# addtt/ladder-vae-pytorch

Measured on AMD Instinct MI355X. Metric: training images/sec (ELBO step: fwd+bwd+Adamax), higher is better.
Workload: dtype f32; 1 GPU; CIFAR10-shaped 15-layer LVAE (BASELINE configs[2]): 32x32x3, zdims 32x15, 4 blocks/layer, 64 filters, gated+skip, DMoL-10, dropout 0.2, free bits 1.0; batch_per_gpu=256, global_batch=256, parallelism=dp1, hip_graph=True

## Files before the change

include/lvae_hip.h:

```cpp
#ifndef LVAE_HIP_H
#define LVAE_HIP_H

#include <stddef.h>
#include <stdint.h>

#ifdef __cplusplus
extern "C" {
#endif

#define LVAE_ABI_VERSION 17

#define LVAE_EINVAL (-1)
#define LVAE_EALIGN (-2)
#define LVAE_EWORKSPACE (-3)

enum { LVAE_STATS_BN_FWD = 0, LVAE_STATS_BN_BWD = 1 };
enum { LVAE_PREC_F32 = 0, LVAE_PREC_BF16 = 1 };
enum { LVAE_DT_F32 = 0, LVAE_DT_BF16 = 1 };
enum {
  LVAE_FORM_AUTO = 0,
  LVAE_FORM_F32_MFMA = 1,
  LVAE_FORM_SIX_PRODUCT = 2,
  LVAE_FORM_SIX_PRODUCT_DIRECT = 3
};
enum { LVAE_ACT_NONE = 0, LVAE_ACT_ELU = 1, LVAE_ACT_RELU = 2, LVAE_ACT_LEAKYRELU = 3, LVAE_ACT_SELU = 4 };

enum {
  LVAE_GATHER_CONV = 0,
  LVAE_GATHER_TRANSPOSED = 1
};

int lvae_abi_version(void);
const char* lvae_last_error(void);

typedef struct lvae_bn_fold {
  const float* parts;
  int32_t rows;
  int64_t M;
  const float* gamma;
  const float* beta;
  float eps, momentum;
  float* running_mean;
  float* running_var;
  float* coef_out;
} lvae_bn_fold;

typedef struct lvae_conv_desc {
  const float* x;
  const float* x2;
  int32_t C1, C2;
  const float* w;
  int64_t w_stap, w_sk, w_sn;
  const float* bias;
  const float* in_scale;
  const float* in_shift;
  int32_t in_act;
  const float* out_scale;
  int32_t out_act;
  float* y;
  int32_t N, H, W, OH, OW, Cout;
  int32_t KH, KW, stride, pad;
  int32_t gather;
  int32_t precision;
  void* workspace;
  int64_t workspace_bytes;
  int32_t workspace_ready;
  float* stats_out;
  const float* stats_pivot;
  int32_t stats_mode;
  int32_t stats_act;
  const float* stats_x;
  const struct lvae_bn_fold* in_fold;
  int32_t form;
  uint8_t x_dtype;
  uint8_t y_dtype;
  uint8_t stats_x_dtype;
  uint8_t reserved_;
} lvae_conv_desc;

size_t lvae_conv2d_workspace(const lvae_conv_desc* d);
int lvae_conv2d_f32(const lvae_conv_desc* d, void* stream);
int lvae_conv1x1_dgrad_cat_f32(const lvae_conv_desc* d, float* dx2, int32_t split, void* stream);
int32_t lvae_conv1x1_dgrad_cat_ok(const lvae_conv_desc* d, int32_t split);
enum {
  LVAE_VARIANT_DIRECT = 0,
  LVAE_VARIANT_POS = 2,
  LVAE_VARIANT_WINO_F32 = 3,
  LVAE_VARIANT_WINO_SIX = 4,
  LVAE_VARIANT_BF16_DIRECT = 5,
  LVAE_VARIANT_SIX_DIRECT = 6
};
int32_t lvae_conv2d_variant(const lvae_conv_desc* d);
int32_t lvae_conv2d_position_major(const lvae_conv_desc* d);
int32_t lvae_resblock_bf16_storage(const lvae_conv_desc* d);
int lvae_conv2d_bf16(const lvae_conv_desc* d, void* stream);
int32_t lvae_conv2d_stats_rows(const lvae_conv_desc* d);
int32_t lvae_conv2d_folds_bn_finalize(const lvae_conv_desc* d);
int32_t lvae_conv2d_stats_buffer_rows(const lvae_conv_desc* d);

size_t lvae_conv2d_prepare_entry_bytes(void);
int lvae_conv2d_prepare_entry(const lvae_conv_desc* d, void* entry);
int lvae_conv2d_prepare_weights(const void* entries, int32_t n, int32_t max_cout, void* stream);

int lvae_conv1x1_gate_f32(const lvae_conv_desc* d, const float* res, int32_t act, float* out, void* stream);
int32_t lvae_conv1x1_gate_stats_rows(const lvae_conv_desc* d);
enum {
  LVAE_GATE_PERSISTENT = 1,
  LVAE_GATE_SINGLE_SHOT = 2
};
int32_t lvae_conv1x1_gate_variant(const lvae_conv_desc* d);
int lvae_conv1x1_gate_bwd_f32(const lvae_conv_desc* d, const float* dout, const float* ab, int32_t act, float* dab,
                              void* stream);
int32_t lvae_conv1x1_gate_bwd_ok(const lvae_conv_desc* d);

typedef struct lvae_bn_apply {
  const float* parts;
  int32_t rows;
  int32_t act;
  int64_t M;
  const float* coef;
  const float* dh;
  const float* x;
  const float* add;
  float* dgamma;
  float* dbeta;
  float* out;
  int32_t dh_bf16;
  int32_t reserved_;
  const float* drop;
} lvae_bn_apply;
size_t lvae_conv1x1_gate_bwd_wgrad_workspace(const lvae_conv_desc* d);
int32_t lvae_conv1x1_gate_bwd_wgrad_apply_ok(const lvae_conv_desc* d);
int lvae_conv1x1_gate_bwd_wgrad_f32(const lvae_conv_desc* d, const float* dout, const float* ab, const float* y, int32_t act,
                                    float* dw, int64_t dw_sk, int64_t dw_sn, float* db, void* workspace, size_t workspace_bytes,
                                    const lvae_bn_apply* ap, void* stream);
int32_t lvae_conv1x1_gate_bwd_wgrad_recompute_ok(const lvae_conv_desc* d);
int lvae_conv1x1_gate_bwd_wgrad_recompute_f32(const lvae_conv_desc* d, const float* dout, const float* y, int32_t act, void* gate_ws,
                                              int64_t gate_ws_bytes, int32_t gate_ws_ready, const float* gate_w, int64_t gate_w_sk,
                                              int64_t gate_w_sn, const float* gate_bias, float* dw, int64_t dw_sk, int64_t dw_sn,
                                              float* db, void* workspace, size_t workspace_bytes, const lvae_bn_apply* ap, void* stream);

size_t lvae_conv1x1_cat_bwd_workspace(const lvae_conv_desc* d, int32_t split);
int32_t lvae_conv1x1_cat_bwd_apply_ok(const lvae_conv_desc* d, int32_t split);
int lvae_conv1x1_cat_bwd_f32(const lvae_conv_desc* d, const float* x1, const float* x2, float* dx1, float* dx2, float* dweight, float* dbias,
                             const lvae_bn_apply* ap, void* workspace, size_t workspace_bytes, int32_t max_workgroups, void* stream);

enum { LVAE_RB_PRO_AFFINE = 0, LVAE_RB_PRO_BN_APPLY = 1, LVAE_RB_PRO_GATE_BWD = 2 };
enum { LVAE_RB_EPI_PLAIN = 0, LVAE_RB_EPI_GATE = 1 };
typedef struct lvae_rb_ext {
  int32_t prologue, epilogue;
  const float* gate_w;
  int64_t gate_w_sk, gate_w_sn;
  void* gate_ws;
  int64_t gate_ws_bytes;
  int32_t gate_ws_ready;
  const float* gate_bias;
  int32_t act;
  const float* res;
  float* ab;
  float* out;
  float* out_stats;
  const float* out_stats_pivot;
  const float* dout;
  const float* ab_in;
  float* dab;
  const float* bwd_parts;
  int32_t bwd_rows;
  int32_t bwd_act;
  int64_t bwd_M;
  const float* bwd_coef;
  const float* bwd_x;
  float* dgamma;
  float* dbeta;
  const float* pro_drop;
  float* xt_out;
  const void* pf_ptr[2];
  int64_t pf_bytes[2];
  const float* ap_parts;
  int32_t ap_rows;
  int32_t ap_act;
  int64_t ap_M;
  const float* ap_coef;
  const float* ap_dh;
  const float* ap_x;
  const float* ap_add;
  float* ap_dgamma;
  float* ap_dbeta;
  float* ap_out;
} lvae_rb_ext;
size_t lvae_resblock_gate_workspace(const lvae_conv_desc* g);
int lvae_resblock_gate_prepare_entry(const lvae_conv_desc* g, void* entry);
int32_t lvae_resblock_conv_rows(const lvae_conv_desc* d);
int32_t lvae_resblock_conv_gate_rows(const lvae_conv_desc* d);
size_t lvae_resblock_conv_workspace(const lvae_conv_desc* d);
int lvae_resblock_conv_prepare_entry(const lvae_conv_desc* d, void* entry);
int lvae_resblock_conv_f32(const lvae_conv_desc* d, const lvae_rb_ext* ext, void* stream);

size_t lvae_conv2d_wgrad_workspace(const lvae_conv_desc* d);
int lvae_conv2d_wgrad_f32(const lvae_conv_desc* d, const float* dy, float* dw, float* db, void* workspace,
                          size_t workspace_bytes, void* stream);
int lvae_conv2d_wgrad_bf16(const lvae_conv_desc* d, const float* dy, float* dw, float* db, void* workspace, size_t workspace_bytes,
                           void* stream);
int32_t lvae_conv2d_wgrad_apply_ok(const lvae_conv_desc* d);
int lvae_conv2d_wgrad_apply_f32(const lvae_conv_desc* d, const lvae_bn_apply* ap, float* dw, float* db, void* workspace,
                                size_t workspace_bytes, void* stream);
int32_t lvae_conv2d_wgrad_pair_ok(const lvae_conv_desc* a, const lvae_conv_desc* b);
size_t lvae_conv2d_wgrad_pair_workspace(const lvae_conv_desc* a, const lvae_conv_desc* b);
int32_t lvae_conv2d_wgrad_pair_schedule(const lvae_conv_desc* a, const lvae_conv_desc* b, int32_t* sched);
int lvae_conv2d_wgrad_pair_f32(const lvae_conv_desc* a, const lvae_bn_apply* ap, const lvae_conv_desc* b, const float* dy_b, float* dw_a,
                               float* db_a, float* dw_b, float* db_b, void* workspace, size_t workspace_bytes, void* stream);
int32_t lvae_conv2d_wgrad_shared_ok(const lvae_conv_desc* descs, const lvae_bn_apply* const* aps, int32_t n);
size_t lvae_conv2d_wgrad_shared_workspace(const lvae_conv_desc* descs, int32_t n);
int32_t lvae_conv2d_wgrad_shared_schedule(const lvae_conv_desc* descs, const lvae_bn_apply* const* aps, int32_t n, int32_t* sched);
int lvae_conv2d_wgrad_shared_f32(const lvae_conv_desc* descs, const float* const* dy, float* const* dw, float* const* db, int32_t n,
                                 void* workspace, size_t workspace_bytes, void* stream);
enum {
  LVAE_WGRAD_VARIANT_GENERIC = 0,
  LVAE_WGRAD_VARIANT_IMG = 1,
  LVAE_WGRAD_VARIANT_BF16 = 2,
  LVAE_WGRAD_VARIANT_WINO = 3,
  LVAE_WGRAD_VARIANT_DIRECT_1X1 = 4,
  LVAE_WGRAD_VARIANT_TILE = 5,
  LVAE_WGRAD_VARIANT_THIN = 6
};
int32_t lvae_conv2d_wgrad_variant(const lvae_conv_desc* d);
size_t lvae_conv2d_wgrad_grouped_workspace(const lvae_conv_desc* descs, int32_t n);
int lvae_conv2d_wgrad_grouped_f32(const lvae_conv_desc* descs, const float* const* dy, float* const* dw, float* const* db,
                                  int32_t n, void* workspace, size_t workspace_bytes, void* stream);
int32_t lvae_conv2d_wgrad_grouped_schedule(const lvae_conv_desc* descs, int32_t n, int32_t* launch_of);

size_t lvae_bn_stats_workspace(int64_t M, int32_t C);
int lvae_bn_stats_f32(const float* x, int64_t M, int32_t C, const float* gamma, const float* beta, float eps,
                      float momentum, float* running_mean, float* running_var, float* scale, float* shift,
                      float* mean, float* rstd, void* workspace, size_t workspace_bytes, void* stream);
int lvae_bn_finalize_parts_f32(const float* parts, int32_t rows, int64_t M, int32_t C, const float* pivot, const float* gamma,
                               const float* beta, float eps, float momentum, float* running_mean, float* running_var,
                               float* scale, float* shift, float* mean, float* rstd, void* stream);
int lvae_bn_eval_coeffs_f32(int32_t C, const float* gamma, const float* beta, const float* running_mean,
                            const float* running_var, float eps, float* scale, float* shift, void* stream);

int lvae_affine_act_f32(const float* x, int64_t M, int32_t C, const float* scale, const float* shift, int32_t act,
                        const float* row_scale, int64_t rows_per_n, float* y, void* stream);

int lvae_affine_act_bwd_f32(const float* dh, const float* x, int64_t M, int32_t C, const float* scale,
                            const float* shift, int32_t act, int32_t bn_train, const float* mean, const float* rstd,
                            float* dgamma, float* dbeta, const float* drop, int64_t rows_per_n, const float* add,
                            float* dx, void* workspace, size_t workspace_bytes, void* stream);
int lvae_affine_act_bwd_parts_f32(const float* parts, int32_t rows, const float* dh, const float* x, int64_t M, int32_t C,
                                  const float* scale, const float* shift, int32_t act, const float* mean, const float* rstd,
                                  float* dgamma, float* dbeta, const float* drop, int64_t rows_per_n, const float* add,
                                  float* dx, void* workspace, size_t workspace_bytes, int32_t dtypes, void* stream);

int lvae_gate_fwd_f32(const float* ab, const float* res, int64_t M, int32_t C, int32_t act, float* out, void* stream);
int lvae_gate_bwd_f32(const float* dout, const float* ab, int64_t M, int32_t C, int32_t act, float* dab, void* stream);

int lvae_act_bwd_from_out_f32(const float* dy, const float* y, int64_t n, int32_t act, float* dx, void* stream);
int lvae_add_f32(const float* a, const float* b, int64_t n, float* out, void* stream);
int lvae_add3_f32(const float* a, const float* b, const float* c, int64_t n, float* out, void* stream);
int lvae_sum_of_row_means_f32(const float* x, int32_t L, int32_t N, float* out, void* stream);
int lvae_scale_rows_add_f32(const float* a, const float* row_scale, int64_t rows_per_n, int32_t C, const float* b,
                            int64_t M, float* out, void* stream);
int lvae_colsum_f32(const float* x, int64_t R, int64_t P, float* out, int32_t accumulate, void* stream);

int lvae_normal_stochastic_fwd_f32(const float* p, int32_t p_bcast, const float* q, const float* eps, int32_t N,
                                   int32_t HW, int32_t Z, int32_t mode, int32_t analytical_kl, float* z,
                                   float* logprob_p, float* logprob_q, float* kl_samplewise, float* kl_spatial,
                                   void* stream);
int lvae_normal_stochastic_bwd_f32(const float* p, int32_t p_bcast, const float* q, const float* eps, const float* z,
                                   const float* dz, const float* g_lp, const float* g_lq, const float* g_kl,
                                   const float* g_ks, int32_t N, int32_t HW, int32_t Z, int32_t mode,
                                   int32_t analytical_kl, float* dp, float* dq, void* stream);

typedef struct lvae_stoch_block {
  lvae_conv_desc conv_p, conv_q, conv_out;
  const float* p_given;
  int32_t p_bcast;
  int32_t mode, analytical_kl;
  const float* eps;
  float *logprob_p, *logprob_q, *kl_samplewise, *kl_spatial;
} lvae_stoch_block;
int32_t lvae_stoch_block_ok(const lvae_stoch_block* b);
size_t lvae_stoch_block_workspace(const lvae_conv_desc* d);
int lvae_stoch_block_prepare_entry(const lvae_conv_desc* d, void* entry);
int lvae_stoch_block_fwd_f32(const lvae_stoch_block* b, void* stream);
typedef struct lvae_stoch_block_bwd {
  lvae_conv_desc dgrad_out, dgrad_q, dgrad_p;
  const float* p;
  int32_t p_bcast;
  int32_t mode, analytical_kl;
  const float *q, *z, *eps, *dz, *g_lp, *g_lq, *g_kl, *g_ks;
} lvae_stoch_block_bwd;
int32_t lvae_stoch_block_bwd_ok(const lvae_stoch_block_bwd* b);
int lvae_stoch_block_bwd_f32(const lvae_stoch_block_bwd* b, void* stream);

int lvae_normal_prior_sample_f32(const float* p, int32_t p_bcast, const float* eps, float temperature,
                                 const float* row_temperature, int32_t N, int32_t HW, int32_t Z, float* z, float* logprob_p,
                                 void* stream);

size_t lvae_latent_interp_workspace(int32_t B, int32_t T);
int lvae_latent_interp_f32(const float* za, const float* zb, const float* t, int32_t B, int64_t n, int32_t T, int32_t mode, float* out,
                           void* workspace, size_t workspace_bytes, void* stream);

int lvae_kl_elementwise_fwd_f32(const float* p, int32_t p_bcast, const float* q, int32_t q_bcast, const float* z, int32_t N,
                                int32_t HW, int32_t Z, int32_t analytical_kl, float* out, void* stream);
int lvae_kl_elementwise_bwd_f32(const float* p, int32_t p_bcast, const float* q, int32_t q_bcast, const float* z, const float* g,
                                int32_t N, int32_t HW, int32_t Z, int32_t analytical_kl, float* dp, float* dq, float* dz,
                                void* stream);

int lvae_bernoulli_fwd_f32(const float* logits, const float* x, const float* u, int32_t N, int64_t P, float* mean,
                           float* mode, float* sample, float* ll, float* dll_dlogits, void* stream);
size_t lvae_dmol_workspace(int32_t N, int32_t HW);
int lvae_dmol_ll_fwd_f32(const float* l, const float* x, int32_t N, int32_t HW, int32_t nmix, float* ll, float* dll_dl,
                         void* workspace, size_t workspace_bytes, void* stream);
int lvae_dmol_sample_f32(const float* l, const float* u_mix, const float* u_log, int32_t N, int32_t HW, int32_t nmix,
                         float* sample, void* stream);
int lvae_gaussian_fwd_f32(const float* params, const float* x, const float* eps, int32_t N, int64_t P, int32_t C,
                          float* sample, float* ll, float* dll_dparams, void* stream);
int lvae_discr_logistic_fwd_f32(const float* raw, const float* x, const float* u, int32_t N, int64_t P, int32_t C, float* mean,
                                float* logscale, float* sample, float* ll, float* dll_draw, void* stream);
int lvae_bernoulli_masked_fwd_f32(const float* logits, const float* x, const float* u, int32_t N, int64_t P, int32_t C, float* mean,
                                  float* mode, float* sample, float* ll, float* dll_dlogits, const uint8_t* mask, float* filled,
                                  void* stream);
int lvae_dmol_ll_masked_fwd_f32(const float* l, const float* x, int32_t N, int32_t HW, int32_t nmix, float* ll, float* dll_dl,
                                void* workspace, size_t workspace_bytes, const uint8_t* mask, const float* sample, float* filled,
                                void* stream);
int lvae_gaussian_masked_fwd_f32(const float* params, const float* x, const float* eps, int32_t N, int64_t P, int32_t C, float* sample,
                                 float* ll, float* dll_dparams, const uint8_t* mask, float* filled, void* stream);
int lvae_discr_logistic_masked_fwd_f32(const float* raw, const float* x, const float* u, int32_t N, int64_t P, int32_t C, float* mean,
                                       float* logscale, float* sample, float* ll, float* dll_draw, const uint8_t* mask, float* filled,
                                       void* stream);
int lvae_mask_select_f32(const float* a, const float* b, float b_value, const uint8_t* mask, int32_t N, int32_t C, int64_t HW,
                         int32_t nchw, float* out, void* stream);
int lvae_scale_per_sample_f32(const float* a, const float* g, int32_t N, int64_t P, float* out, void* stream);

int lvae_upsample2x_fwd_f32(const float* x, int32_t N, int32_t H, int32_t W, int32_t C, float* y, void* stream);
int lvae_upsample2x_bwd_f32(const float* dy, int32_t N, int32_t H, int32_t W, int32_t C, float* dx, void* stream);
int lvae_pad_crop_f32(const float* x, int32_t N, int32_t C, int32_t H, int32_t W, int32_t src_nchw, float* y, int32_t OH,
                      int32_t OW, int32_t dst_nchw, void* stream);

int lvae_kl_bookkeeping_fwd_f32(const float* kl, int32_t L, int32_t N, float free_bits, float* kl_sep,
                                float* kl_avg_layerwise, float* scalars, void* stream);
int lvae_kl_bookkeeping_bwd_f32(const float* kl, int32_t L, int32_t N, float free_bits, const float* g_sep,
                                const float* g_avg, const float* g_scalars, float* dkl, void* stream);
int lvae_elbo_loss_fwd_f32(const float* ll, const float* kl_sep, const float* kl_loss, float beta, int32_t N,
                           float* elbo_sep, float* scalars, void* stream);
int lvae_elbo_loss_bwd_f32(const float* g_loss, float beta, int32_t N, float* d_ll, float* d_kl_loss, void* stream);
int lvae_elbo_loss_fwd_anneal_f32(const float* ll, const float* kl_sep, const float* kl_loss, const int64_t* step, int64_t anneal_steps,
                                  int32_t N, float* elbo_sep, float* scalars, void* stream);
int lvae_elbo_loss_bwd_anneal_f32(const float* g_loss, const int64_t* step, int64_t anneal_steps, int32_t N, float* d_ll,
                                  float* d_kl_loss, void* stream);

int lvae_iw_loss_fwd_f32(const float* ll, const float* kl_sep, float beta, int32_t K, int32_t B, float* elbo_sep, float* w, float* bound,
                         float* scalars, void* stream);
int lvae_iw_loss_bwd_f32(const float* g_loss, const float* w, float beta, int32_t K, int32_t B, float* d_ll, float* d_kl_sep,
                         void* stream);
int lvae_iw_loss_fwd_anneal_f32(const float* ll, const float* kl_sep, const int64_t* step, int64_t anneal_steps, int32_t K, int32_t B,
                                float* elbo_sep, float* w, float* bound, float* scalars, void* stream);
int lvae_iw_loss_bwd_anneal_f32(const float* g_loss, const float* w, const int64_t* step, int64_t anneal_steps, int32_t K, int32_t B,
                                float* d_ll, float* d_kl_sep, void* stream);
int lvae_repeat_samples_fwd_f32(const float* in, int64_t n, int32_t K, float* out, void* stream);
int lvae_repeat_samples_bwd_f32(const float* dout, int64_t n, int32_t K, float* din, void* stream);

int lvae_iw_logmeanexp_f32(const float* elbo, int32_t S, int32_t N, float* out, void* stream);
int lvae_iw_online_f32(const float* elbo, float* state, int32_t N, int32_t mode, int32_t S, float* iw, float* mean, void* stream);
int lvae_eval_online_f32(const float* elbo_sep, const float* ll, const float* kl_sep, const float* kl_avg_layerwise, double* state,
                         int32_t N, int32_t L, int32_t mode, void* stream);
int lvae_eval_totals_f64(const double* state, int32_t N, int32_t L, int32_t S, double* totals, void* stream);
size_t lvae_latent_stats_workspace(int32_t N, int32_t HW, int32_t Z);
int lvae_latent_stats_fold_f32(const float* p, int32_t p_bcast, const float* q, int32_t N, int32_t HW, int32_t Z, double* sums,
                               void* workspace, size_t workspace_bytes, void* stream);
int lvae_latent_stats_finalize_f64(const double* sums, int64_t U, int64_t n_images, double kl_threshold, double var_threshold,
                                   double* unit_out, double* layer_out, void* stream);
int lvae_summary_fold_f64(const float* loss, const float* elbo, const float* recons, const float* kl, const float* l2,
                          const float* grad_norm, const float* gscale, const float* kl_layers, int32_t L, double* acc, void* stream);
int lvae_summary_take_f64(double* acc, int32_t n, double* out, void* stream);
int lvae_micro_fold_f64(const float* loss, const float* elbo, const float* recons, const float* kl, const float* l2, const float* iw,
                        const float* ess, const float* kl_layers, int32_t L, int32_t M, double* acc, int64_t* count, float* out,
                        void* stream);

int lvae_image_border_count_f32(const float* a, int32_t a_nhwc, const float* b, int32_t b_nhwc, int32_t N, int32_t C, int32_t H,
                                int32_t W, float threshold, int32_t* count, void* stream);
int lvae_image_grid_u8(const float* a, int32_t a_nhwc, const float* b, int32_t b_nhwc, int32_t N, int32_t C, int32_t H, int32_t W,
                       int32_t nrow, const int32_t* border_count, float pad_value, uint8_t* grid, int64_t grid_bytes, void* stream);

#define LVAE_FEED_U8 0
#define LVAE_FEED_F32 1
int lvae_batch_gather_f32(const void* src, int32_t src_kind, int32_t src_hwc, int32_t N, int32_t C, int32_t H, int32_t W,
                          const int32_t* index, const int64_t* cursor, int32_t steps_per_epoch, int32_t B_global, int32_t lo,
                          int64_t base, int32_t n_rows, float* out, void* stream);

size_t lvae_nn_l2_workspace(int32_t Q, int64_t N, int32_t k);
int lvae_nn_l2_f32(const float* queries, int32_t Q, const void* table, int32_t table_kind, int64_t N, int64_t D, const int32_t* exclude,
                   int32_t k, int32_t* index_out, float* dist_out, void* workspace, size_t workspace_bytes, void* stream);

int lvae_adamax_step_f32(float* p, const float* g, float* exp_avg, float* exp_inf, const float* mask, int64_t n,
                         float lr, float beta1, float beta2, float eps, float weight_decay, const float* gscale,
                         const uint64_t* step_count, void* stream);
int lvae_adamax_ema_step_f32(float* p, const float* g, float* exp_avg, float* exp_inf, const float* mask, int64_t n,
                             float lr, float beta1, float beta2, float eps, float weight_decay, const float* gscale,
                             const uint64_t* step_count, float* ema, float decay, void* stream);
enum { LVAE_LR_CONSTANT = 0, LVAE_LR_COSINE = 1, LVAE_LR_LINEAR = 2, LVAE_LR_STEP = 3, LVAE_LR_EXP = 4 };
typedef struct lvae_lr_schedule {
  float base_lr;
  float min_lr;
  float gamma;
  int32_t kind;
  int64_t warmup_steps;
  int64_t decay_steps;
} lvae_lr_schedule;
int lvae_lr_schedule_at(const lvae_lr_schedule* schedule, uint64_t n, float* lr);
int lvae_adamax_sched_step_f32(float* p, const float* g, float* exp_avg, float* exp_inf, const float* mask, int64_t n,
                               const lvae_lr_schedule* schedule, float beta1, float beta2, float eps, float weight_decay,
                               const float* gscale, const uint64_t* step_count, float* ema, float decay, float* lr_out, void* stream);
typedef struct lvae_grad_guard_state {
  float norm;
  float scale;
  int32_t skip;
  int32_t reserved_;
  uint64_t clipped;
  uint64_t skipped;
} lvae_grad_guard_state;
int lvae_grad_guard_f32(const float* g, int64_t n, const float* gscale_in, float max_norm, float skip_threshold,
                        lvae_grad_guard_state* state, void* workspace, size_t workspace_bytes, void* stream);
int lvae_adamax_guarded_step_f32(float* p, const float* g, float* exp_avg, float* exp_inf, const float* mask, int64_t n, float lr,
                                 const lvae_lr_schedule* schedule, float beta1, float beta2, float eps, float weight_decay,
                                 const uint64_t* step_count, float* ema, float decay, float* lr_out,
                                 const lvae_grad_guard_state* guard, void* stream);
int lvae_adam_step_f32(float* p, const float* g, float* exp_avg, float* exp_avg_sq, const float* mask, int64_t n, float lr,
                       const lvae_lr_schedule* schedule , double beta1, double beta2, float eps, float weight_decay,
                       int32_t decoupled, const float* gscale , const uint64_t* step_count, float* ema ,
                       float decay, float* lr_out , const lvae_grad_guard_state* guard , void* stream);
typedef struct lvae_copy_entry {
  float* dst;
  const float* src;
  int64_t n;
} lvae_copy_entry;
int lvae_multi_copy_f32(const lvae_copy_entry* table, int32_t n_entries, const int32_t* flag, int32_t want, void* stream);
int lvae_swap_f32(float* a, float* b, int64_t n, void* stream);
size_t lvae_sumsq_workspace(int64_t n);
int lvae_l2norm_f32(const float* x, int64_t n, float* out, void* workspace, size_t workspace_bytes, void* stream);

int lvae_rng_fill_f32(float* out, int64_t n, int32_t kind, float lo, float hi, uint64_t seed, const uint64_t* offset,
                      uint64_t stream_id, void* stream);
int lvae_counter_advance(uint64_t* counter, uint64_t by, void* stream);
int lvae_counter_advance_unless(uint64_t* counter, uint64_t by, const int32_t* flag, void* stream);
int lvae_fill_f32(float* out, int64_t n, float value, void* stream);

int lvae_allreduce_unique_id(const char* librccl_path, void* id128);
int lvae_allreduce_init(const char* librccl_path, const void* id128, int32_t world, int32_t rank, void** handle);
int lvae_allreduce_enqueue(void* handle, float* buf, int64_t n, float* scratch, void* launch_stream, void* side_stream);
int lvae_allreduce_wait(void* handle, void* launch_stream, void* side_stream);
int lvae_allreduce_destroy(void* handle);

#ifdef __cplusplus
}
#endif
#endif
```

ladder-vae-pytorch_amd/_C.py:

```python
import ctypes as C
import os

import torch

_HERE = os.path.dirname(os.path.abspath(__file__))
LIB_PATH = os.path.join(_HERE, 'liblvae_hip.so')

ACT = {None: 0, 'none': 0, 'elu': 1, 'relu': 2, 'leakyrelu': 3, 'selu': 4}
GATHER_CONV, GATHER_TRANSPOSED = 0, 1
PREC_F32, PREC_BF16 = 0, 1
DT_F32, DT_BF16 = 0, 1
VARIANT_DIRECT, VARIANT_POS, VARIANT_WINO_F32, VARIANT_WINO_SIX, VARIANT_BF16_DIRECT, VARIANT_SIX_DIRECT = 0, 2, 3, 4, 5, 6
GATE_PERSISTENT, GATE_SINGLE_SHOT = 1, 2
WGRAD_VARIANT_GENERIC, WGRAD_VARIANT_IMG, WGRAD_VARIANT_BF16, WGRAD_VARIANT_WINO, WGRAD_VARIANT_DIRECT_1X1, WGRAD_VARIANT_TILE, WGRAD_VARIANT_THIN = range(7)
FEED_U8, FEED_F32 = 0, 1
FORM_AUTO, FORM_F32_MFMA, FORM_SIX_PRODUCT, FORM_SIX_PRODUCT_DIRECT = 0, 1, 2, 3


class LvaeHipError(RuntimeError):
    pass


class ConvDesc(C.Structure):
    _fields_ = [
        ('x', C.c_void_p), ('x2', C.c_void_p), ('C1', C.c_int32), ('C2', C.c_int32),
        ('w', C.c_void_p), ('w_stap', C.c_int64), ('w_sk', C.c_int64), ('w_sn', C.c_int64),
        ('bias', C.c_void_p), ('in_scale', C.c_void_p), ('in_shift', C.c_void_p), ('in_act', C.c_int32),
        ('out_scale', C.c_void_p), ('out_act', C.c_int32), ('y', C.c_void_p),
        ('N', C.c_int32), ('H', C.c_int32), ('W', C.c_int32), ('OH', C.c_int32), ('OW', C.c_int32),
        ('Cout', C.c_int32), ('KH', C.c_int32), ('KW', C.c_int32), ('stride', C.c_int32), ('pad', C.c_int32),
        ('gather', C.c_int32), ('precision', C.c_int32), ('workspace', C.c_void_p), ('workspace_bytes', C.c_int64), ('workspace_ready', C.c_int32), ('stats_out', C.c_void_p), ('stats_pivot', C.c_void_p), ('stats_mode', C.c_int32), ('stats_act', C.c_int32),
        ('stats_x', C.c_void_p),
        ('in_fold', C.c_void_p),
        ('form', C.c_int32), ('x_dtype', C.c_uint8), ('y_dtype', C.c_uint8), ('stats_x_dtype', C.c_uint8), ('reserved_', C.c_uint8),
    ]


class BnFold(C.Structure):
    _fields_ = [('parts', C.c_void_p), ('rows', C.c_int32), ('M', C.c_int64), ('gamma', C.c_void_p), ('beta', C.c_void_p),
                ('eps', C.c_float), ('momentum', C.c_float), ('running_mean', C.c_void_p), ('running_var', C.c_void_p),
                ('coef_out', C.c_void_p)]


class BnApply(C.Structure):
    _fields_ = [('parts', C.c_void_p), ('rows', C.c_int32), ('act', C.c_int32), ('M', C.c_int64), ('coef', C.c_void_p), ('dh', C.c_void_p),
                ('x', C.c_void_p), ('add', C.c_void_p), ('dgamma', C.c_void_p), ('dbeta', C.c_void_p), ('out', C.c_void_p),
                ('dh_bf16', C.c_int32), ('reserved_', C.c_int32), ('drop', C.c_void_p)]


class RbExt(C.Structure):
    _fields_ = [('prologue', C.c_int32), ('epilogue', C.c_int32), ('gate_w', C.c_void_p), ('gate_w_sk', C.c_int64), ('gate_w_sn', C.c_int64),
                ('gate_ws', C.c_void_p), ('gate_ws_bytes', C.c_int64), ('gate_ws_ready', C.c_int32), ('gate_bias', C.c_void_p), ('act', C.c_int32), ('res', C.c_void_p), ('ab', C.c_void_p), ('out', C.c_void_p),
                ('out_stats', C.c_void_p), ('out_stats_pivot', C.c_void_p), ('dout', C.c_void_p), ('ab_in', C.c_void_p), ('dab', C.c_void_p),
                ('bwd_parts', C.c_void_p), ('bwd_rows', C.c_int32), ('bwd_act', C.c_int32), ('bwd_M', C.c_int64), ('bwd_coef', C.c_void_p),
                ('bwd_x', C.c_void_p), ('dgamma', C.c_void_p), ('dbeta', C.c_void_p), ('pro_drop', C.c_void_p), ('xt_out', C.c_void_p),
                ('pf_ptr', C.c_void_p * 2), ('pf_bytes', C.c_int64 * 2),
                ('ap_parts', C.c_void_p), ('ap_rows', C.c_int32), ('ap_act', C.c_int32), ('ap_M', C.c_int64), ('ap_coef', C.c_void_p),
                ('ap_dh', C.c_void_p), ('ap_x', C.c_void_p), ('ap_add', C.c_void_p), ('ap_dgamma', C.c_void_p), ('ap_dbeta', C.c_void_p),
                ('ap_out', C.c_void_p)]


class StochBlock(C.Structure):
    _fields_ = [('conv_p', ConvDesc), ('conv_q', ConvDesc), ('conv_out', ConvDesc), ('p_given', C.c_void_p), ('p_bcast', C.c_int32),
                ('mode', C.c_int32), ('analytical_kl', C.c_int32), ('eps', C.c_void_p), ('logprob_p', C.c_void_p), ('logprob_q', C.c_void_p),
                ('kl_samplewise', C.c_void_p), ('kl_spatial', C.c_void_p)]


class StochBlockBwd(C.Structure):
    _fields_ = [('dgrad_out', ConvDesc), ('dgrad_q', ConvDesc), ('dgrad_p', ConvDesc), ('p', C.c_void_p), ('p_bcast', C.c_int32),
                ('mode', C.c_int32), ('analytical_kl', C.c_int32), ('q', C.c_void_p), ('z', C.c_void_p), ('eps', C.c_void_p), ('dz', C.c_void_p),
                ('g_lp', C.c_void_p), ('g_lq', C.c_void_p), ('g_kl', C.c_void_p), ('g_ks', C.c_void_p)]


class LrScheduleStruct(C.Structure):
    _fields_ = [('base_lr', C.c_float), ('min_lr', C.c_float), ('gamma', C.c_float), ('kind', C.c_int32),
                ('warmup_steps', C.c_int64), ('decay_steps', C.c_int64)]


class GradGuardState(C.Structure):
    _fields_ = [('norm', C.c_float), ('scale', C.c_float), ('skip', C.c_int32), ('reserved_', C.c_int32), ('clipped', C.c_uint64),
                ('skipped', C.c_uint64)]


class CopyEntry(C.Structure):
    _fields_ = [('dst', C.c_void_p), ('src', C.c_void_p), ('n', C.c_int64)]


LR_KINDS = {'constant': 0, 'cosine': 1, 'linear': 2, 'step': 3, 'exp': 4}

RB_PRO_AFFINE, RB_PRO_BN_APPLY, RB_PRO_GATE_BWD = 0, 1, 2
RB_EPI_PLAIN, RB_EPI_GATE = 0, 1

ABI_VERSION = 17

_P, _I, _L, _F, _Z, _U = C.c_void_p, C.c_int32, C.c_int64, C.c_float, C.c_size_t, C.c_uint64

SIGNATURES = {
    'lvae_abi_version': (C.c_int, []),
    'lvae_last_error': (C.c_char_p, []),
    'lvae_conv2d_workspace': (_Z, [C.POINTER(ConvDesc)]),
    'lvae_conv2d_f32': (C.c_int, [C.POINTER(ConvDesc), _P]),
    'lvae_conv2d_bf16': (C.c_int, [C.POINTER(ConvDesc), _P]),
    'lvae_conv1x1_dgrad_cat_f32': (C.c_int, [C.POINTER(ConvDesc), _P, _I, _P]),
    'lvae_conv1x1_dgrad_cat_ok': (_I, [C.POINTER(ConvDesc), _I]),
    'lvae_conv2d_stats_rows': (_I, [C.POINTER(ConvDesc)]),
    'lvae_conv2d_variant': (_I, [C.POINTER(ConvDesc)]),
    'lvae_conv2d_position_major': (_I, [C.POINTER(ConvDesc)]),
    'lvae_resblock_bf16_storage': (_I, [C.POINTER(ConvDesc)]),
    'lvae_conv2d_folds_bn_finalize': (_I, [C.POINTER(ConvDesc)]),
    'lvae_conv2d_stats_buffer_rows': (_I, [C.POINTER(ConvDesc)]),
    'lvae_conv2d_prepare_entry_bytes': (_Z, []),
    'lvae_conv2d_prepare_entry': (C.c_int, [C.POINTER(ConvDesc), _P]),
    'lvae_conv2d_prepare_weights': (C.c_int, [_P, _I, _I, _P]),
    'lvae_conv1x1_gate_f32': (C.c_int, [C.POINTER(ConvDesc), _P, _I, _P, _P]),
    'lvae_conv1x1_gate_stats_rows': (_I, [C.POINTER(ConvDesc)]),
    'lvae_conv1x1_gate_variant': (_I, [C.POINTER(ConvDesc)]),
    'lvae_conv1x1_gate_bwd_f32': (C.c_int, [C.POINTER(ConvDesc), _P, _P, _I, _P, _P]),
    'lvae_conv1x1_gate_bwd_ok': (_I, [C.POINTER(ConvDesc)]),
    'lvae_conv1x1_gate_bwd_wgrad_workspace': (_Z, [C.POINTER(ConvDesc)]),
    'lvae_conv1x1_gate_bwd_wgrad_apply_ok': (_I, [C.POINTER(ConvDesc)]),
    'lvae_conv1x1_gate_bwd_wgrad_f32': (C.c_int, [C.POINTER(ConvDesc), _P, _P, _P, _I, _P, _L, _L, _P, _P, _Z, C.POINTER(BnApply), _P]),
    'lvae_conv1x1_gate_bwd_wgrad_recompute_ok': (_I, [C.POINTER(ConvDesc)]),
    'lvae_conv1x1_gate_bwd_wgrad_recompute_f32': (C.c_int, [C.POINTER(ConvDesc), _P, _P, _I, _P, _L, _I, _P, _L, _L, _P, _P, _L, _L, _P, _P, _Z,
                                                            C.POINTER(BnApply), _P]),
    'lvae_conv1x1_cat_bwd_workspace': (_Z, [C.POINTER(ConvDesc), _I]),
    'lvae_conv1x1_cat_bwd_apply_ok': (_I, [C.POINTER(ConvDesc), _I]),
    'lvae_conv1x1_cat_bwd_f32': (C.c_int, [C.POINTER(ConvDesc), _P, _P, _P, _P, _P, _P, C.POINTER(BnApply), _P, _Z, _I, _P]),
    'lvae_resblock_gate_workspace': (_Z, [C.POINTER(ConvDesc)]),
    'lvae_resblock_gate_prepare_entry': (C.c_int, [C.POINTER(ConvDesc), _P]),
    'lvae_resblock_conv_rows': (_I, [C.POINTER(ConvDesc)]),
    'lvae_resblock_conv_gate_rows': (_I, [C.POINTER(ConvDesc)]),
    'lvae_resblock_conv_workspace': (_Z, [C.POINTER(ConvDesc)]),
    'lvae_resblock_conv_prepare_entry': (C.c_int, [C.POINTER(ConvDesc), _P]),
    'lvae_resblock_conv_f32': (C.c_int, [C.POINTER(ConvDesc), C.POINTER(RbExt), _P]),
    'lvae_conv2d_wgrad_workspace': (_Z, [C.POINTER(ConvDesc)]),
    'lvae_conv2d_wgrad_f32': (C.c_int, [C.POINTER(ConvDesc), _P, _P, _P, _P, _Z, _P]),
    'lvae_conv2d_wgrad_bf16': (C.c_int, [C.POINTER(ConvDesc), _P, _P, _P, _P, _Z, _P]),
    'lvae_conv2d_wgrad_variant': (_I, [C.POINTER(ConvDesc)]),
    'lvae_conv2d_wgrad_apply_ok': (_I, [C.POINTER(ConvDesc)]),
    'lvae_conv2d_wgrad_apply_f32': (C.c_int, [C.POINTER(ConvDesc), C.POINTER(BnApply), _P, _P, _P, _Z, _P]),
    'lvae_conv2d_wgrad_pair_ok': (_I, [C.POINTER(ConvDesc), C.POINTER(ConvDesc)]),
    'lvae_conv2d_wgrad_pair_workspace': (_Z, [C.POINTER(ConvDesc), C.POINTER(ConvDesc)]),
    'lvae_conv2d_wgrad_pair_schedule': (_I, [C.POINTER(ConvDesc), C.POINTER(ConvDesc), C.POINTER(_I)]),
    'lvae_conv2d_wgrad_pair_f32': (C.c_int, [C.POINTER(ConvDesc), C.POINTER(BnApply), C.POINTER(ConvDesc), _P, _P, _P, _P, _P, _P, _Z, _P]),
    'lvae_conv2d_wgrad_shared_ok': (_I, [C.POINTER(ConvDesc), _P, _I]),
    'lvae_conv2d_wgrad_shared_workspace': (_Z, [C.POINTER(ConvDesc), _I]),
    'lvae_conv2d_wgrad_shared_schedule': (_I, [C.POINTER(ConvDesc), _P, _I, C.POINTER(_I)]),
    'lvae_conv2d_wgrad_shared_f32': (C.c_int, [C.POINTER(ConvDesc), _P, _P, _P, _I, _P, _Z, _P]),
    'lvae_conv2d_wgrad_grouped_workspace': (_Z, [C.POINTER(ConvDesc), _I]),
    'lvae_conv2d_wgrad_grouped_f32': (C.c_int, [C.POINTER(ConvDesc), _P, _P, _P, _I, _P, _Z, _P]),
    'lvae_conv2d_wgrad_grouped_schedule': (_I, [C.POINTER(ConvDesc), _I, C.POINTER(_I)]),
    'lvae_bn_stats_workspace': (_Z, [_L, _I]),
    'lvae_bn_stats_f32': (C.c_int, [_P, _L, _I, _P, _P, _F, _F, _P, _P, _P, _P, _P, _P, _P, _Z, _P]),
    'lvae_bn_finalize_parts_f32': (C.c_int, [_P, _I, _L, _I, _P, _P, _P, _F, _F, _P, _P, _P, _P, _P, _P, _P]),
    'lvae_bn_eval_coeffs_f32': (C.c_int, [_I, _P, _P, _P, _P, _F, _P, _P, _P]),
    'lvae_affine_act_f32': (C.c_int, [_P, _L, _I, _P, _P, _I, _P, _L, _P, _P]),
    'lvae_affine_act_bwd_f32': (C.c_int, [_P, _P, _L, _I, _P, _P, _I, _I, _P, _P, _P, _P, _P, _L, _P, _P, _P, _Z, _P]),
    'lvae_affine_act_bwd_parts_f32': (C.c_int, [_P, _I, _P, _P, _L, _I, _P, _P, _I, _P, _P, _P, _P, _P, _L, _P, _P, _P, _Z, _I, _P]),
    'lvae_gate_fwd_f32': (C.c_int, [_P, _P, _L, _I, _I, _P, _P]),
    'lvae_gate_bwd_f32': (C.c_int, [_P, _P, _L, _I, _I, _P, _P]),
    'lvae_act_bwd_from_out_f32': (C.c_int, [_P, _P, _L, _I, _P, _P]),
    'lvae_add_f32': (C.c_int, [_P, _P, _L, _P, _P]),
    'lvae_add3_f32': (C.c_int, [_P, _P, _P, _L, _P, _P]),
    'lvae_sum_of_row_means_f32': (C.c_int, [_P, _I, _I, _P, _P]),
    'lvae_scale_rows_add_f32': (C.c_int, [_P, _P, _L, _I, _P, _L, _P, _P]),
    'lvae_colsum_f32': (C.c_int, [_P, _L, _L, _P, _I, _P]),
    'lvae_normal_stochastic_fwd_f32': (C.c_int, [_P, _I, _P, _P, _I, _I, _I, _I, _I, _P, _P, _P, _P, _P, _P]),
    'lvae_normal_stochastic_bwd_f32': (C.c_int, [_P, _I, _P, _P, _P, _P, _P, _P, _P, _P, _I, _I, _I, _I, _I, _P, _P, _P]),
    'lvae_stoch_block_ok': (_I, [C.POINTER(StochBlock)]),
    'lvae_stoch_block_workspace': (_Z, [C.POINTER(ConvDesc)]),
    'lvae_stoch_block_prepare_entry': (C.c_int, [C.POINTER(ConvDesc), _P]),
    'lvae_stoch_block_fwd_f32': (C.c_int, [C.POINTER(StochBlock), _P]),
    'lvae_stoch_block_bwd_ok': (_I, [C.POINTER(StochBlockBwd)]),
    'lvae_stoch_block_bwd_f32': (C.c_int, [C.POINTER(StochBlockBwd), _P]),
    'lvae_normal_prior_sample_f32': (C.c_int, [_P, _I, _P, _F, _P, _I, _I, _I, _P, _P, _P]),
    'lvae_latent_interp_workspace': (_Z, [_I, _I]),
    'lvae_latent_interp_f32': (C.c_int, [_P, _P, _P, _I, _L, _I, _I, _P, _P, _Z, _P]),
    'lvae_kl_elementwise_fwd_f32': (C.c_int, [_P, _I, _P, _I, _P, _I, _I, _I, _I, _P, _P]),
    'lvae_kl_elementwise_bwd_f32': (C.c_int, [_P, _I, _P, _I, _P, _P, _I, _I, _I, _I, _P, _P, _P, _P]),
    'lvae_bernoulli_fwd_f32': (C.c_int, [_P, _P, _P, _I, _L, _P, _P, _P, _P, _P, _P]),
    'lvae_dmol_workspace': (_Z, [_I, _I]),
    'lvae_dmol_ll_fwd_f32': (C.c_int, [_P, _P, _I, _I, _I, _P, _P, _P, _Z, _P]),
    'lvae_dmol_sample_f32': (C.c_int, [_P, _P, _P, _I, _I, _I, _P, _P]),
    'lvae_gaussian_fwd_f32': (C.c_int, [_P, _P, _P, _I, _L, _I, _P, _P, _P, _P]),
    'lvae_discr_logistic_fwd_f32': (C.c_int, [_P, _P, _P, _I, _L, _I, _P, _P, _P, _P, _P, _P]),
    'lvae_bernoulli_masked_fwd_f32': (C.c_int, [_P, _P, _P, _I, _L, _I, _P, _P, _P, _P, _P, _P, _P, _P]),
    'lvae_dmol_ll_masked_fwd_f32': (C.c_int, [_P, _P, _I, _I, _I, _P, _P, _P, _Z, _P, _P, _P, _P]),
    'lvae_gaussian_masked_fwd_f32': (C.c_int, [_P, _P, _P, _I, _L, _I, _P, _P, _P, _P, _P, _P]),
    'lvae_discr_logistic_masked_fwd_f32': (C.c_int, [_P, _P, _P, _I, _L, _I, _P, _P, _P, _P, _P, _P, _P, _P]),
    'lvae_mask_select_f32': (C.c_int, [_P, _P, _F, _P, _I, _I, _L, _I, _P, _P]),
    'lvae_scale_per_sample_f32': (C.c_int, [_P, _P, _I, _L, _P, _P]),
    'lvae_upsample2x_fwd_f32': (C.c_int, [_P, _I, _I, _I, _I, _P, _P]),
    'lvae_upsample2x_bwd_f32': (C.c_int, [_P, _I, _I, _I, _I, _P, _P]),
    'lvae_pad_crop_f32': (C.c_int, [_P, _I, _I, _I, _I, _I, _P, _I, _I, _I, _P]),
    'lvae_kl_bookkeeping_fwd_f32': (C.c_int, [_P, _I, _I, _F, _P, _P, _P, _P]),
    'lvae_kl_bookkeeping_bwd_f32': (C.c_int, [_P, _I, _I, _F, _P, _P, _P, _P, _P]),
    'lvae_elbo_loss_fwd_f32': (C.c_int, [_P, _P, _P, _F, _I, _P, _P, _P]),
    'lvae_elbo_loss_bwd_f32': (C.c_int, [_P, _F, _I, _P, _P, _P]),
    'lvae_elbo_loss_fwd_anneal_f32': (C.c_int, [_P, _P, _P, _P, _L, _I, _P, _P, _P]),
    'lvae_elbo_loss_bwd_anneal_f32': (C.c_int, [_P, _P, _L, _I, _P, _P, _P]),
    'lvae_iw_loss_fwd_f32': (C.c_int, [_P, _P, _F, _I, _I, _P, _P, _P, _P, _P]),
    'lvae_iw_loss_bwd_f32': (C.c_int, [_P, _P, _F, _I, _I, _P, _P, _P]),
    'lvae_iw_loss_fwd_anneal_f32': (C.c_int, [_P, _P, _P, _L, _I, _I, _P, _P, _P, _P, _P]),
    'lvae_iw_loss_bwd_anneal_f32': (C.c_int, [_P, _P, _P, _L, _I, _I, _P, _P, _P]),
    'lvae_repeat_samples_fwd_f32': (C.c_int, [_P, _L, _I, _P, _P]),
    'lvae_repeat_samples_bwd_f32': (C.c_int, [_P, _L, _I, _P, _P]),
    'lvae_iw_online_f32': (C.c_int, [_P, _P, _I, _I, _I, _P, _P, _P]),
    'lvae_eval_online_f32': (C.c_int, [_P, _P, _P, _P, _P, _I, _I, _I, _P]),
    'lvae_eval_totals_f64': (C.c_int, [_P, _I, _I, _I, _P, _P]),
    'lvae_latent_stats_workspace': (_Z, [_I, _I, _I]),
    'lvae_latent_stats_fold_f32': (C.c_int, [_P, _I, _P, _I, _I, _I, _P, _P, _Z, _P]),
    'lvae_latent_stats_finalize_f64': (C.c_int, [_P, _L, _L, C.c_double, C.c_double, _P, _P, _P]),
    'lvae_summary_fold_f64': (C.c_int, [_P, _P, _P, _P, _P, _P, _P, _P, _I, _P, _P]),
    'lvae_summary_take_f64': (C.c_int, [_P, _I, _P, _P]),
    'lvae_micro_fold_f64': (C.c_int, [_P, _P, _P, _P, _P, _P, _P, _P, _I, _I, _P, _P, _P, _P]),
    'lvae_image_border_count_f32': (C.c_int, [_P, _I, _P, _I, _I, _I, _I, _I, _F, _P, _P]),
    'lvae_image_grid_u8': (C.c_int, [_P, _I, _P, _I, _I, _I, _I, _I, _I, _P, _F, _P, _L, _P]),
    'lvae_batch_gather_f32': (C.c_int, [_P, _I, _I, _I, _I, _I, _I, _P, _P, _I, _I, _I, _L, _I, _P, _P]),
    'lvae_nn_l2_workspace': (_Z, [_I, _L, _I]),
    'lvae_nn_l2_f32': (C.c_int, [_P, _I, _P, _I, _L, _L, _P, _I, _P, _P, _P, _Z, _P]),
    'lvae_iw_logmeanexp_f32': (C.c_int, [_P, _I, _I, _P, _P]),
    'lvae_adamax_step_f32': (C.c_int, [_P, _P, _P, _P, _P, _L, _F, _F, _F, _F, _F, _P, _P, _P]),
    'lvae_adamax_ema_step_f32': (C.c_int, [_P, _P, _P, _P, _P, _L, _F, _F, _F, _F, _F, _P, _P, _P, _F, _P]),
    'lvae_lr_schedule_at': (C.c_int, [C.POINTER(LrScheduleStruct), _U, C.POINTER(C.c_float)]),
    'lvae_adamax_sched_step_f32': (C.c_int, [_P, _P, _P, _P, _P, _L, C.POINTER(LrScheduleStruct), _F, _F, _F, _F, _P, _P, _P, _F, _P, _P]),
    'lvae_grad_guard_f32': (C.c_int, [_P, _L, _P, _F, _F, _P, _P, _Z, _P]),
    'lvae_adamax_guarded_step_f32': (C.c_int, [_P, _P, _P, _P, _P, _L, _F, C.POINTER(LrScheduleStruct), _F, _F, _F, _F, _P, _P, _F, _P, _P, _P]),
    'lvae_adam_step_f32': (C.c_int, [_P, _P, _P, _P, _P, _L, _F, C.POINTER(LrScheduleStruct), C.c_double, C.c_double, _F, _F, _I, _P, _P, _P,
                                     _F, _P, _P, _P]),
    'lvae_multi_copy_f32': (C.c_int, [_P, _I, _P, _I, _P]),
    'lvae_swap_f32': (C.c_int, [_P, _P, _L, _P]),
    'lvae_sumsq_workspace': (_Z, [_L]),
    'lvae_l2norm_f32': (C.c_int, [_P, _L, _P, _P, _Z, _P]),
    'lvae_rng_fill_f32': (C.c_int, [_P, _L, _I, _F, _F, _U, _P, _U, _P]),
    'lvae_counter_advance': (C.c_int, [_P, _U, _P]),
    'lvae_counter_advance_unless': (C.c_int, [_P, _U, _P, _P]),
    'lvae_fill_f32': (C.c_int, [_P, _L, _F, _P]),
    'lvae_allreduce_unique_id': (C.c_int, [C.c_char_p, _P]),
    'lvae_allreduce_init': (C.c_int, [C.c_char_p, _P, _I, _I, C.POINTER(C.c_void_p)]),
    'lvae_allreduce_enqueue': (C.c_int, [_P, _P, _L, _P, _P, _P]),
    'lvae_allreduce_wait': (C.c_int, [_P, _P, _P]),
    'lvae_allreduce_destroy': (C.c_int, [_P]),
}

_lib = None


def load():
    global _lib
    if _lib is not None:
        return _lib
    if not os.path.exists(LIB_PATH):
        raise LvaeHipError("%s is missing: build it with `python -c 'import __graft_entry__ as g; g.build()'` or "
                           "`make -C ladder-vae-pytorch_amd/csrc`. There is no CPU / PyTorch fallback." % LIB_PATH)
    lib = C.CDLL(LIB_PATH)
    for name, (res, args) in SIGNATURES.items():
        fn = getattr(lib, name)
        fn.restype, fn.argtypes = res, args
    if lib.lvae_abi_version() != ABI_VERSION:
        raise LvaeHipError("liblvae_hip.so ABI version %d, expected %d" % (lib.lvae_abi_version(), ABI_VERSION))
    _lib = lib
    return lib


def stream_ptr():
    return torch.cuda.current_stream().cuda_stream


def ptr(t, dtypes=(torch.float32, torch.int64, torch.uint8)):
    if t is None:
        return None
    if not t.is_cuda:
        raise LvaeHipError("lvae_hip kernels need CUDA/HIP tensors; got a %s tensor (no CPU fallback exists)" % t.device)
    if t.dtype not in dtypes:
        raise LvaeHipError("unexpected dtype %s for this entry point (it has no storage-type argument for this tensor)" % t.dtype)
    return t.data_ptr()


def ptr_dt(t):
    return ptr(t, (torch.float32, torch.bfloat16))


def check(rc, name):
    if rc != 0:
        raise LvaeHipError("%s failed (%d): %s" % (name, rc, load().lvae_last_error().decode()))


def call(name, *args):
    check(getattr(load(), name)(*args), name)
```

ladder-vae-pytorch_amd/csrc/resblock_img.hip:

```cpp
#include <string.h>

#include "bf16_frag.h"
#include "bn_stats.h"
#include "lvae_host.h"

namespace lvae {

struct RbArgs {
  lvae_conv_desc d;
  lvae_bn_fold f;
  lvae_rb_ext e;
  const __bf16* Wp;
  int NI, HW, halo_w, halo_h, halo_px, flip, nwg;
  uint32_t m_hw, m_w, m_per_img, m_halo_w;
};

constexpr int RB_LDK = 72;
constexpr int RB_LDD = 136;
constexpr int RB_LDO = 68;
constexpr int RB_LDG = 132;
constexpr int RB_SCR_BYTES = 9216;

#ifdef LVAE_RB_DBG
__device__ unsigned long long g_rb_stamps[1024 * 4 * 12];
#define RB_STAMP_DECL unsigned long long rb_ts[12] = {0, 0, 0, 0, 0, 0, 0, 0, 0, 0, 0, 0}
#define RB_STAMP(i) rb_ts[i] = __builtin_amdgcn_s_memtime()
#define RB_STAMP_FLUSH                                                                                             \
  do {                                                                                                             \
    if ((threadIdx.x & 63) == 0 && blockIdx.x < 1024)                                                              \
      for (int i_ = 0; i_ < 12; ++i_) g_rb_stamps[(blockIdx.x * 4 + (threadIdx.x >> 6)) * 12 + i_] = rb_ts[i_];    \
  } while (0)
#else
#define RB_STAMP_DECL do {} while (0)
#define RB_STAMP(i) do {} while (0)
#define RB_STAMP_FLUSH do {} while (0)
#endif

constexpr int RB_PF = 32;
__device__ __forceinline__ void rb_parts_issue(const float* __restrict__ parts, int rows, f32x4 (&v)[RB_PF]) {
  const int t = threadIdx.x, q = t & 31, rg = t >> 5;
#pragma unroll
  for (int u = 0; u < RB_PF; ++u) {
    const int rr = rg + 8 * u;
    v[u] = *reinterpret_cast<const f32x4*>(parts + (size_t)(rr < rows ? rr : 0) * 128 + q * 4);
  }
}
template <typename F>
__device__ __forceinline__ void rb_parts_finish(const float* __restrict__ parts, int rows, const f32x4 (&v0)[RB_PF], float* scr, F&& finish,
                                                unsigned long long* ts = nullptr) {
  const int t = threadIdx.x, q = t & 31, rg = t >> 5;
  f32x4 acc = {0.f, 0.f, 0.f, 0.f};
#pragma unroll
  for (int u = 0; u < RB_PF; ++u)
    if (rg + 8 * u < rows) acc += v0[u];
#ifdef LVAE_RB_DBG
  if (ts) { asm volatile("" :: "v"(acc[0])); ts[8] = __builtin_amdgcn_s_memtime(); }
#endif
  for (int r = rg + 8 * RB_PF; r < rows; r += 8 * 16) {
    f32x4 v[16];
#pragma unroll
    for (int u = 0; u < 16; ++u) {
      const int rr = r + 8 * u;
      v[u] = *reinterpret_cast<const f32x4*>(parts + (size_t)(rr < rows ? rr : 0) * 128 + q * 4);
    }
#pragma unroll
    for (int u = 0; u < 16; ++u)
      if (r + 8 * u < rows) acc += v[u];
  }
  *reinterpret_cast<f32x4*>(scr + rg * 128 + q * 4) = acc;
  lds_barrier();
#ifdef LVAE_RB_DBG
  if (ts) ts[9] = __builtin_amdgcn_s_memtime();
#endif
  if (t < 64) {
    double sa = 0.0, sb = 0.0;
#pragma unroll
    for (int g = 0; g < 8; ++g) {
      sa += (double)scr[g * 128 + t];
      sb += (double)scr[g * 128 + 64 + t];
    }
    finish(t, sa, sb);
  }
  lds_barrier();
}

template <int SPLIT, int MI, int PRO, int EPI, bool ELU, bool AP = false>
__global__ __launch_bounds__(256) void rb_conv_kernel(RbArgs a) {
  static_assert(MI == 1 || MI == 2, "32- or 64-pixel tiles (MI 32-row blocks)");
  static_assert(!AP || PRO == LVAE_RB_PRO_GATE_BWD, "the deferred apply feeds the gate-backward prologue");
  constexpr int BM = 32 * MI, LDK = RB_LDK, LDO = RB_LDO, NQ = BM / 16;
  constexpr int OS_BYTES = BM * LDO * 4;
  extern __shared__ __attribute__((aligned(16))) unsigned char smem_raw[];
  kernarg_warmup<sizeof(RbArgs)>();
  float* scr = reinterpret_cast<float*>(smem_raw);
  unsigned char* mainr = smem_raw + RB_SCR_BYTES;
  __bf16* As = reinterpret_cast<__bf16*>(mainr + (PRO == LVAE_RB_PRO_GATE_BWD ? OS_BYTES : 0));
  const int a_plane = a.halo_px * LDK;

  const lvae_conv_desc& d = a.d;
  const lvae_rb_ext& e = a.e;
  const int in_act = ELU ? LVAE_ACT_ELU : d.in_act, stats_act = ELU ? LVAE_ACT_ELU : d.stats_act;
  const int gate_act = ELU ? LVAE_ACT_ELU : e.act, bwd_act = ELU ? LVAE_ACT_ELU : e.bwd_act, ap_act = ELU ? LVAE_ACT_ELU : e.ap_act;
  const int t = threadIdx.x, lane = t & 63, wave = t >> 6;
  const int wm = MI == 2 ? wave >> 1 : 0, wn = wave & 1, li = lane & 31, lh = lane >> 5;
  const bool g1_on = MI == 2 || wave < 2;
  const int bid = blockIdx.x;
  const int n0 = bid * a.NI, HW = a.HW;
  const int nvalid = min(BM, (d.N - n0) * HW);
  const size_t row0 = (size_t)n0 * HW;
  const int c4 = (t & 15) * 4, p0 = t >> 4;
  const f32x4 zero4 = {0.f, 0.f, 0.f, 0.f};
  const f32x4 one4 = {1.f, 1.f, 1.f, 1.f};

  constexpr int RING = SPLIT == 1 ? 9 : 3;
  bf16x8 bq[RING][2][SPLIT];
  const __bf16* wp_lane = a.Wp + (size_t)wave * SPLIT * 1024 + (size_t)lane * 8;
  auto load_b = [&](int tap, bf16x8 (&r)[2][SPLIT]) {
    const __bf16* src = wp_lane + (size_t)tap * 4 * SPLIT * 1024;
#pragma unroll
    for (int p = 0; p < SPLIT; ++p) {
      r[0][p] = *reinterpret_cast<const bf16x8*>(src + p * 1024);
      r[1][p] = *reinterpret_cast<const bf16x8*>(src + p * 1024 + 512);
    }
  };
  RB_STAMP_DECL;
#ifdef LVAE_RB_DBG_REPS
  const int rb_reps = a.flip >= 0 ? LVAE_RB_DBG_REPS : 1;
#pragma unroll 1
  for (int rb_rep = 0; rb_rep < rb_reps; ++rb_rep) {
  lds_barrier();
#endif
  RB_STAMP(0);
  constexpr int PFN = 6;
  unsigned pf_dump[2][PFN];
  auto pf_issue = [&]() {
#pragma unroll
    for (int k = 0; k < 2; ++k) {
      const int per_xcd = (a.nwg + 7) >> 3, part = bid >> 3;
      const int lines = e.pf_ptr[k] != nullptr ? (int)((e.pf_bytes[k] + 127) >> 7) : 0, per = (lines + per_xcd - 1) / per_xcd;
      const int lo = part * per, hi = min(lo + per, lines);
      const char* base = static_cast<const char*>(e.pf_ptr[k]) + (size_t)(lo + t) * 128;
#pragma unroll
      for (int i = 0; i < PFN; ++i) {
        pf_dump[k][i] = 0;
        if (lo + t + 256 * i < hi) pf_dump[k][i] = *reinterpret_cast<const unsigned*>(base + i * 256 * 128);
      }
    }
  };
  auto pf_drain = [&]() {
#pragma unroll
    for (int k = 0; k < 2; ++k)
#pragma unroll
      for (int i = 0; i < PFN; ++i) asm volatile("" ::"v"(pf_dump[k][i]));
  };

  int hp[NQ], img_n[NQ];
  size_t grow[NQ];
  bool ok[NQ];
#pragma unroll
  for (int q = 0; q < NQ; ++q) {
    const int p = p0 + 16 * q;
    const int img = fastdiv(p, a.m_hw), r = p - img * HW;
    const int y = fastdiv(r, a.m_w), x = r - y * d.W;
    hp[q] = ((img * a.halo_h + y + 1) * a.halo_w + x + 1) * LDK + c4;
    ok[q] = p < nvalid;
    img_n[q] = ok[q] ? n0 + img : n0;
    grow[q] = row0 + (ok[q] ? p : 0);
  }
  auto put_interior = [&](int q, f32x4 v) {
    bf16x4 pl[SPLIT];
    split4_packed<SPLIT>(v, pl);
#pragma unroll
    for (int k = 0; k < SPLIT; ++k) *reinterpret_cast<bf16x4*>(As + k * a_plane + hp[q]) = pl[k];
  };
  auto zero_ring = [&]() {
    const int per_img = a.halo_h * a.halo_w;
    const bf16x8 z = {0, 0, 0, 0, 0, 0, 0, 0};
    for (int idx = t; idx < a.halo_px * 8; idx += 256) {
      const int px = idx >> 3, c8 = (idx & 7) * 8;
      const int img = fastdiv(px, a.m_per_img), r = px - img * per_img;
      const int hy = fastdiv(r, a.m_halo_w), hx = r - hy * a.halo_w;
      if (hy == 0 || hy == a.halo_h - 1 || hx == 0 || hx == a.halo_w - 1) {
#pragma unroll
        for (int k = 0; k < SPLIT; ++k) *reinterpret_cast<bf16x8*>(As + k * a_plane + px * LDK + c8) = z;
      }
    }
  };

  if (PRO == LVAE_RB_PRO_AFFINE) {
    const lvae_bn_fold& f = a.f;
    const bool has_tf = f.parts != nullptr || d.in_scale != nullptr;
    f32x4 pv[RB_PF];
    if (f.parts != nullptr) rb_parts_issue(f.parts, f.rows, pv);
    pf_issue();
    const bool lead = t < 64 && f.parts != nullptr;
    const float pivot = lead ? f.parts[((size_t)f.rows * 2) * 64 + t] : 0.f;
    const float gam = lead && f.gamma ? f.gamma[t] : 1.f, bet = lead && f.beta ? f.beta[t] : 0.f;
    const bool upd = lead && bid == 0 && f.running_mean != nullptr;
    const float rm0 = upd ? f.running_mean[t] : 0.f, rv0 = upd ? f.running_var[t] : 0.f;
    f32x4 xv[NQ];
#pragma unroll
    for (int q = 0; q < NQ; ++q) xv[q] = *reinterpret_cast<const f32x4*>(d.x + grow[q] * 64 + c4);
    zero_ring();
    f32x4 sc = one4, sh = zero4;
    if (f.parts != nullptr) {
      rb_parts_finish(f.parts, f.rows, pv, scr, [&](int c, double sa, double sb) {
        const BnChannel r = bn_finalize_channel(sa, sb, pivot, f.M, f.eps, gam, bet);
        scr[1024 + c] = r.scale;
        scr[1024 + 64 + c] = r.shift;
        if (bid == 0) {
          if (f.coef_out) bn_store_coef(f.coef_out, 64, c, r);
          if (upd) bn_update_running(f.running_mean, f.running_var, c, rm0, rv0, f.momentum, r, f.M);
        }
      });
      sc = *reinterpret_cast<const f32x4*>(scr + 1024 + c4);
      sh = *reinterpret_cast<const f32x4*>(scr + 1024 + 64 + c4);
    } else if (d.in_scale != nullptr) {
      sc = *reinterpret_cast<const f32x4*>(d.in_scale + c4);
      sh = *reinterpret_cast<const f32x4*>(d.in_shift + c4);
    }
    RB_STAMP(1);
#pragma unroll
    for (int q = 0; q < NQ; ++q) {
      f32x4 v = xv[q];
      if (has_tf) v = act_fwd4(v * sc + sh, in_act);
      put_interior(q, ok[q] ? v : zero4);
    }
    RB_STAMP(10);
    RB_STAMP(11);
  }

  if (PRO == LVAE_RB_PRO_BN_APPLY) {
    f32x4 pv[RB_PF];
    rb_parts_issue(e.bwd_parts, e.bwd_rows, pv);
    pf_issue();
    const f32x4 sc = *reinterpret_cast<const f32x4*>(e.bwd_coef + c4), sh = *reinterpret_cast<const f32x4*>(e.bwd_coef + 64 + c4);
    const f32x4 mu = *reinterpret_cast<const f32x4*>(e.bwd_coef + 128 + c4), rs = *reinterpret_cast<const f32x4*>(e.bwd_coef + 192 + c4);
    const bool acc_here = bid == 0 && t < 64;
    const float db0 = acc_here && e.dbeta ? e.dbeta[t] : 0.f, dg0 = acc_here && e.dgamma ? e.dgamma[t] : 0.f;
    f32x4 gv[NQ], xv[NQ], dm[NQ];
#pragma unroll
    for (int q = 0; q < NQ; ++q) {
      gv[q] = *reinterpret_cast<const f32x4*>(d.x + grow[q] * 64 + c4);
      xv[q] = *reinterpret_cast<const f32x4*>(e.bwd_x + grow[q] * 64 + c4);
      dm[q] = e.pro_drop ? *reinterpret_cast<const f32x4*>(e.pro_drop + (size_t)img_n[q] * 64 + c4) : one4;
    }
    zero_ring();
    rb_parts_finish(e.bwd_parts, e.bwd_rows, pv, scr, [&](int c, double sa, double sb) {
      const BnBwdChannel r = bn_bwd_finish(sa, sb, e.bwd_M);
      scr[1024 + c] = r.c1;
      scr[1024 + 64 + c] = r.c2;
      if (bid == 0) {
        if (e.dbeta) e.dbeta[c] = db0 + r.dbeta;
        if (e.dgamma) e.dgamma[c] = dg0 + r.dgamma;
      }
    }
#ifdef LVAE_RB_DBG
    , rb_ts
#endif
    );
    const f32x4 c1 = *reinterpret_cast<const f32x4*>(scr + 1024 + c4), c2 = *reinterpret_cast<const f32x4*>(scr + 1024 + 64 + c4);
    RB_STAMP(1);
#pragma unroll
    for (int q = 0; q < NQ; ++q) {
      const f32x4 g = gv[q] * act_grad4(xv[q] * sc + sh, bwd_act);
      f32x4 v = bn_bwd_apply(g, xv[q], c1, c2, mu, rs, sc) * dm[q];
      if (!ok[q]) v = zero4;
      if (ok[q] && e.xt_out) store_wt4(e.xt_out + grow[q] * 64 + c4, v);
      put_interior(q, v);
    }
  }

  if (PRO == LVAE_RB_PRO_GATE_BWD) {
    __bf16* Ds = reinterpret_cast<__bf16*>(mainr);
    constexpr int LDD = RB_LDD, d_plane = BM * LDD;
    f32x4 go[NQ], aa[NQ], bb[NQ], dm[NQ];
    if (AP) {
      f32x4 pv[RB_PF];
      rb_parts_issue(e.ap_parts, e.ap_rows, pv);
      pf_issue();
      const f32x4 sc = *reinterpret_cast<const f32x4*>(e.ap_coef + c4), sh = *reinterpret_cast<const f32x4*>(e.ap_coef + 64 + c4);
      const f32x4 mu = *reinterpret_cast<const f32x4*>(e.ap_coef + 128 + c4), rs = *reinterpret_cast<const f32x4*>(e.ap_coef + 192 + c4);
      const bool acc_here = bid == 0 && t < 64;
      const float db0 = acc_here && e.ap_dbeta ? e.ap_dbeta[t] : 0.f, dg0 = acc_here && e.ap_dgamma ? e.ap_dgamma[t] : 0.f;
      f32x4 xa[NQ], ad[NQ];
#pragma unroll
      for (int q = 0; q < NQ; ++q) {
        go[q] = *reinterpret_cast<const f32x4*>(e.ap_dh + grow[q] * 64 + c4);
        xa[q] = *reinterpret_cast<const f32x4*>(e.ap_x + grow[q] * 64 + c4);
        ad[q] = *reinterpret_cast<const f32x4*>(e.ap_add + grow[q] * 64 + c4);
      }
#pragma unroll
      for (int q = 0; q < NQ; ++q) {
        aa[q] = *reinterpret_cast<const f32x4*>(e.ab_in + grow[q] * 128 + c4);
        bb[q] = *reinterpret_cast<const f32x4*>(e.ab_in + grow[q] * 128 + 64 + c4);
      }
      rb_parts_finish(e.ap_parts, e.ap_rows, pv, scr, [&](int c, double sa, double sb) {
        const BnBwdChannel r = bn_bwd_finish(sa, sb, e.ap_M);
        scr[1024 + c] = r.c1;
        scr[1024 + 64 + c] = r.c2;
        if (bid == 0) {
          if (e.ap_dbeta) e.ap_dbeta[c] = db0 + r.dbeta;
          if (e.ap_dgamma) e.ap_dgamma[c] = dg0 + r.dgamma;
        }
      });
      const f32x4 c1 = *reinterpret_cast<const f32x4*>(scr + 1024 + c4), c2 = *reinterpret_cast<const f32x4*>(scr + 1024 + 64 + c4);
#pragma unroll
      for (int q = 0; q < NQ; ++q) {
        const f32x4 g = go[q] * act_grad4(xa[q] * sc + sh, ap_act);
        const f32x4 v = bn_bwd_apply(g, xa[q], c1, c2, mu, rs, sc) + ad[q];
        go[q] = v;
        if (ok[q]) store_wt4(e.ap_out + grow[q] * 64 + c4, v);
      }
    } else {
      pf_issue();
#pragma unroll
      for (int q = 0; q < NQ; ++q) {
        go[q] = *reinterpret_cast<const f32x4*>(e.dout + grow[q] * 64 + c4);
        aa[q] = *reinterpret_cast<const f32x4*>(e.ab_in + grow[q] * 128 + c4);
        bb[q] = *reinterpret_cast<const f32x4*>(e.ab_in + grow[q] * 128 + 64 + c4);
      }
    }
    bf16x8 gq[8][SPLIT];
    {
      const __bf16* gws = static_cast<const __bf16*>(e.gate_ws) + (size_t)wn * SPLIT * 512 + lane * 8;
#pragma unroll
      for (int s = 0; s < 8; ++s)
#pragma unroll
        for (int k = 0; k < SPLIT; ++k) gq[s][k] = *reinterpret_cast<const bf16x8*>(gws + ((size_t)s * 2 * SPLIT + k) * 512);
    }
#pragma unroll
    for (int q = 0; q < NQ; ++q) dm[q] = e.pro_drop ? *reinterpret_cast<const f32x4*>(e.pro_drop + (size_t)img_n[q] * 64 + c4) : one4;
#pragma unroll
    for (int q = 0; q < NQ; ++q) {
      const int p = p0 + 16 * q;
      f32x4 da, db;
#pragma unroll
      for (int j = 0; j < 4; ++j) {
        const float s = sigmoidf_(bb[q][j]);
        const float gs = go[q][j] * s;
        da[j] = gs;
        db[j] = gs * (1.f - s);
      }
      da = da * act_grad4(aa[q], gate_act);
      db = db * act_fwd4(aa[q], gate_act);
      if (!ok[q]) da = db = zero4;
      if (ok[q] && e.dab) {
        store_wt4(e.dab + grow[q] * 128 + c4, da);
        store_wt4(e.dab + grow[q] * 128 + 64 + c4, db);
      }
      bf16x4 pa[SPLIT], pb[SPLIT];
      split4_packed<SPLIT>(da, pa);
      split4_packed<SPLIT>(db, pb);
#pragma unroll
      for (int k = 0; k < SPLIT; ++k) {
        *reinterpret_cast<bf16x4*>(Ds + k * d_plane + p * LDD + c4) = pa[k];
        *reinterpret_cast<bf16x4*>(Ds + k * d_plane + p * LDD + 64 + c4) = pb[k];
      }
    }
    RB_STAMP(8);
    lds_barrier();
    f32x16 acc1;
#pragma unroll
    for (int r = 0; r < 16; ++r) acc1[r] = 0.f;
    if (g1_on) {
#pragma unroll
      for (int s = 0; s < 8; ++s) {
        bf16x8 af[SPLIT];
#pragma unroll
        for (int k = 0; k < SPLIT; ++k) af[k] = *reinterpret_cast<const bf16x8*>(Ds + k * d_plane + (wm * 32 + li) * LDD + 16 * s + 8 * lh);
        acc1 = mfma_pieces<SPLIT>(af, gq[s], acc1);
      }
    }
    RB_STAMP(9);
    lds_barrier();
    float* Os1 = reinterpret_cast<float*>(mainr);
    if (g1_on) {
#pragma unroll
      for (int r = 0; r < 16; ++r) Os1[(wm * 32 + (r & 3) + 8 * (r >> 2) + 4 * lh) * LDO + wn * 32 + li] = acc1[r];
    }
    lds_barrier();
#pragma unroll
    for (int q = 0; q < NQ; ++q) {
      const int p = p0 + 16 * q;
      f32x4 v = *reinterpret_cast<const f32x4*>(Os1 + p * LDO + c4) * dm[q];
      if (!ok[q]) v = zero4;
      if (ok[q] && e.xt_out) store_wt4(e.xt_out + grow[q] * 64 + c4, v);
      put_interior(q, v);
    }
    zero_ring();
  }

  pf_drain();
  f32x4 ep_bias = zero4, ep_mask[NQ], ep_piv = zero4, ep_bsh = zero4, ep_bmu = zero4, ep_brs = zero4, ep_sx[NQ], ep_res[NQ], ep_ga = zero4, ep_gb = zero4;
  const bool plain_stats = EPI == LVAE_RB_EPI_PLAIN && d.stats_out != nullptr;
  const bool stats_bwd = plain_stats && d.stats_mode == LVAE_STATS_BN_BWD;
  {
    if (d.bias) ep_bias = *reinterpret_cast<const f32x4*>(d.bias + c4);
#pragma unroll
    for (int q = 0; q < NQ; ++q) {
      ep_mask[q] = d.out_scale ? *reinterpret_cast<const f32x4*>(d.out_scale + (size_t)img_n[q] * 64 + c4) : one4;
      ep_sx[q] = zero4;
      ep_res[q] = zero4;
    }
    if (plain_stats) {
      ep_piv = *reinterpret_cast<const f32x4*>(d.stats_pivot + c4);
      if (stats_bwd) {
        ep_bsh = *reinterpret_cast<const f32x4*>(d.stats_pivot + 64 + c4);
        ep_bmu = *reinterpret_cast<const f32x4*>(d.stats_pivot + 128 + c4);
        ep_brs = *reinterpret_cast<const f32x4*>(d.stats_pivot + 192 + c4);
#pragma unroll
        for (int q = 0; q < NQ; ++q) ep_sx[q] = *reinterpret_cast<const f32x4*>(d.stats_x + grow[q] * 64 + c4);
      }
    }
    if (EPI == LVAE_RB_EPI_GATE) {
      if (e.out_stats) ep_piv = *reinterpret_cast<const f32x4*>(e.out_stats_pivot + c4);
      if (e.gate_bias) {
        ep_ga = *reinterpret_cast<const f32x4*>(e.gate_bias + c4);
        ep_gb = *reinterpret_cast<const f32x4*>(e.gate_bias + 64 + c4);
      }
      if (e.res) {
#pragma unroll
        for (int q = 0; q < NQ; ++q) ep_res[q] = *reinterpret_cast<const f32x4*>(e.res + grow[q] * 64 + c4);
      }
    }
  }
#pragma unroll
  for (int i = 0; i < RING; ++i) load_b(i, bq[i]);

  int hbase[MI];
#pragma unroll
  for (int mb = 0; mb < MI; ++mb) {
    const int p = mb * 32 + li;
    const int img = fastdiv(p, a.m_hw), r = p - img * HW;
    const int ty = fastdiv(r, a.m_w), tx = r - ty * d.W;
    hbase[mb] = ((img * a.halo_h + ty) * a.halo_w + tx) * LDK + wave * 16 + 8 * lh;
  }
  f32x16 acc[MI][2];
#pragma unroll
  for (int mb = 0; mb < MI; ++mb)
#pragma unroll
    for (int nh = 0; nh < 2; ++nh)
#pragma unroll
      for (int r = 0; r < 16; ++r) acc[mb][nh][r] = 0.f;

  RB_STAMP(2);
  lds_barrier();
  RB_STAMP(3);

  {
    bf16x8 af[2][MI][SPLIT];
    auto load_a = [&](int tap, bf16x8 (&fa)[MI][SPLIT]) {
      const int kh = tap / 3, kw = tap - kh * 3;
      const int dh = a.flip ? 2 - kh : kh, dw = a.flip ? 2 - kw : kw;
      const int off = (dh * a.halo_w + dw) * LDK;
#pragma unroll
      for (int p = 0; p < SPLIT; ++p)
#pragma unroll
        for (int mb = 0; mb < MI; ++mb) fa[mb][p] = *reinterpret_cast<const bf16x8*>(As + p * a_plane + hbase[mb] + off);
    };
    load_a(0, af[0]);
#pragma unroll
    for (int tap = 0; tap < 9; ++tap) {
      const int cur = tap & 1;
      if (tap + 1 < 9) load_a(tap + 1, af[cur ^ 1]);
#pragma unroll
      for (int mb = 0; mb < MI; ++mb)
#pragma unroll
        for (int nh = 0; nh < 2; ++nh) acc[mb][nh] = mfma_pieces<SPLIT>(af[cur][mb], bq[tap % RING][nh], acc[mb][nh]);
      if (tap + RING < 9) load_b(tap + RING, bq[tap % RING]);
    }
  }

  RB_STAMP(4);
  bf16x8 gqa[EPI == LVAE_RB_EPI_GATE ? 4 : 1][SPLIT], gqb[EPI == LVAE_RB_EPI_GATE ? 4 : 1][SPLIT];
  if (EPI == LVAE_RB_EPI_GATE) {
    const __bf16* gws = static_cast<const __bf16*>(e.gate_ws) + lane * 8;
#pragma unroll
    for (int s = 0; s < 4; ++s)
#pragma unroll
      for (int k = 0; k < SPLIT; ++k) {
        gqa[s][k] = *reinterpret_cast<const bf16x8*>(gws + ((size_t)(s * 4 + (MI == 2 ? wn : wave)) * SPLIT + k) * 512);
        if (MI == 2) gqb[s][k] = *reinterpret_cast<const bf16x8*>(gws + ((size_t)(s * 4 + 2 + wn) * SPLIT + k) * 512);
        else gqb[s][k] = gqa[s][k];
      }
  }

  lds_barrier();

  float* Os = reinterpret_cast<float*>(mainr);
  constexpr int OSW = BM * LDO;
#pragma unroll
  for (int mb = 0; mb < MI; ++mb)
#pragma unroll
    for (int nh = 0; nh < 2; ++nh)
#pragma unroll
      for (int r = 0; r < 16; ++r)
        Os[wave * OSW + (mb * 32 + (r & 3) + 8 * (r >> 2) + 4 * lh) * LDO + nh * 32 + li] = acc[mb][nh][r];
  lds_barrier();
  RB_STAMP(5);
  auto os_sum = [&](int p) {
    const float* o = Os + p * LDO + c4;
    return (*reinterpret_cast<const f32x4*>(o) + *reinterpret_cast<const f32x4*>(o + OSW)) +
           (*reinterpret_cast<const f32x4*>(o + 2 * OSW) + *reinterpret_cast<const f32x4*>(o + 3 * OSW));
  };

  f32x4 st1 = zero4, st2 = zero4;
  const float* stats_pivot = nullptr;
  float* stats_out = nullptr;
  bool stats_fwd = true;

  if (EPI == LVAE_RB_EPI_PLAIN) {
    stats_out = d.stats_out;
    stats_pivot = d.stats_pivot;
    stats_fwd = !stats_bwd;
#pragma unroll
    for (int q = 0; q < NQ; ++q) {
      const int p = p0 + 16 * q;
      const f32x4 v = (os_sum(p) + ep_bias) * ep_mask[q];
      if (ok[q]) {
        store_wt4(d.y + grow[q] * 64 + c4, v);
        if (stats_out) {
          if (stats_fwd) {
            stats_fwd_accum4(v, ep_piv, st1, st2);
          } else {
            stats_bwd_accum4(v, ep_sx[q], ep_piv, ep_bsh, ep_bmu, ep_brs, stats_act, st1, st2);
          }
        }
      }
    }
  }

  if (EPI == LVAE_RB_EPI_GATE) {
    __bf16* Gs = reinterpret_cast<__bf16*>(mainr + 4 * OS_BYTES);
    constexpr int g_plane = BM * LDK;
#pragma unroll
    for (int q = 0; q < NQ; ++q) {
      const int p = p0 + 16 * q;
      f32x4 v = (os_sum(p) + ep_bias) * ep_mask[q];
      if (!ok[q]) v = zero4;
      if (ok[q]) store_wt4(d.y + grow[q] * 64 + c4, v);
      bf16x4 pl[SPLIT];
      split4_packed<SPLIT>(v, pl);
#pragma unroll
      for (int k = 0; k < SPLIT; ++k) *reinterpret_cast<bf16x4*>(Gs + k * g_plane + p * LDK + c4) = pl[k];
    }
    lds_barrier();
    f32x16 acca, accb;
#pragma unroll
    for (int r = 0; r < 16; ++r) acca[r] = accb[r] = 0.f;
#pragma unroll
    for (int s = 0; s < 4; ++s) {
      bf16x8 af[SPLIT];
#pragma unroll
      for (int k = 0; k < SPLIT; ++k) af[k] = *reinterpret_cast<const bf16x8*>(Gs + k * g_plane + (wm * 32 + li) * LDK + 16 * s + 8 * lh);
      acca = mfma_pieces<SPLIT>(af, gqa[s], acca);
      if (MI == 2) accb = mfma_pieces<SPLIT>(af, gqb[s], accb);
    }
    lds_barrier();
    constexpr int LDG = RB_LDG;
    float* Qs = reinterpret_cast<float*>(mainr);
#pragma unroll
    for (int r = 0; r < 16; ++r) {
      const int row = wm * 32 + (r & 3) + 8 * (r >> 2) + 4 * lh;
      if (MI == 2) {
        Qs[row * LDG + wn * 32 + li] = acca[r];
        Qs[row * LDG + 64 + wn * 32 + li] = accb[r];
      } else {
        Qs[row * LDG + wave * 32 + li] = acca[r];
      }
    }
    lds_barrier();
    stats_out = e.out_stats;
    stats_pivot = e.out_stats_pivot;
#pragma unroll
    for (int q = 0; q < NQ; ++q) {
      const int p = p0 + 16 * q;
      if (ok[q]) {
        const f32x4 av = *reinterpret_cast<const f32x4*>(Qs + p * LDG + c4) + ep_ga;
        const f32x4 bv = *reinterpret_cast<const f32x4*>(Qs + p * LDG + 64 + c4) + ep_gb;
        if (e.ab) {
          store_wt4(e.ab + grow[q] * 128 + c4, av);
          store_wt4(e.ab + grow[q] * 128 + 64 + c4, bv);
        }
        f32x4 o = act_fwd4(av, gate_act);
#pragma unroll
        for (int j = 0; j < 4; ++j) o[j] *= sigmoidf_(bv[j]);
        o += ep_res[q];
        store_wt4(e.out + grow[q] * 64 + c4, o);
        if (stats_out) stats_fwd_accum4(o, ep_piv, st1, st2);
      }
    }
  }

  RB_STAMP(6);
  if (stats_out) {
    lds_barrier();
    float* red = reinterpret_cast<float*>(mainr);
    *reinterpret_cast<f32x4*>(red + (t >> 4) * 64 + c4) = st1;
    *reinterpret_cast<f32x4*>(red + 1024 + (t >> 4) * 64 + c4) = st2;
    lds_barrier();
    if (t < 128) {
      const int c = t & 63, which = t >> 6;
      float v = 0.f;
#pragma unroll
      for (int r = 0; r < 16; ++r) v += red[which * 1024 + r * 64 + c];
      stats_out[((size_t)bid * 2 + which) * 64 + c] = v;
      if (bid == 0 && which == 0 && stats_fwd) stats_out[((size_t)a.nwg * 2) * 64 + c] = stats_pivot[c];
    }
  }
  RB_STAMP(7);
#ifdef LVAE_RB_DBG_REPS
  }
#endif
  RB_STAMP_FLUSH;
}


static bool rb_gate_ok(const lvae_conv_desc* g) {
  return g != nullptr && g->w != nullptr && ((g->C1 == 64 && g->Cout == 128) || (g->C1 == 128 && g->Cout == 64));
}

static int rb_split(const lvae_conv_desc* d) { return d->precision == LVAE_PREC_BF16 ? 1 : 3; }

static int rb_mi(const lvae_conv_desc* d) {
  static const int force = (int)tune("LVAE_RB_MI", 0);
  if (force == 1 || force == 2) return force;
  const int HW = d->H * d->W;
  if (HW <= 16 && 32 % HW == 0 && ((int64_t)d->N * HW + 63) / 64 <= 128) return 1;
  return 2;
}

static size_t rb_lds_bytes(int split, int mi, int halo_px, int pro, int epi) {
  const size_t BM = 32 * mi, patch = (size_t)split * halo_px * RB_LDK * 2, os = BM * RB_LDO * 4;
  size_t m = patch > 4 * os ? patch : 4 * os;
  if (pro == LVAE_RB_PRO_GATE_BWD) {
    const size_t ds = (size_t)split * BM * RB_LDD * 2;
    if (os + patch > m) m = os + patch;
    if (ds > m) m = ds;
  }
  if (epi == LVAE_RB_EPI_GATE) {
    const size_t g = 4 * os + (size_t)split * BM * RB_LDK * 2, q = BM * RB_LDG * 4;
    if (g > m) m = g;
    if (q > m) m = q;
  }
  if (m < 2048 * 4) m = 2048 * 4;
  return RB_SCR_BYTES + m;
}

static bool rb_plan(const lvae_conv_desc* d, RbArgs& a, int& mi) {
  static const bool off = tune("LVAE_DISABLE_RB", 0) != 0;
  if (off || d == nullptr) return false;
  if (d->KH != 3 || d->KW != 3 || d->stride != 1 || d->pad != 1 || d->x2 != nullptr || d->OH != d->H || d->OW != d->W) return false;
  if (d->C1 != 64 || d->C2 != 0 || d->Cout != 64 || d->out_act != LVAE_ACT_NONE) return false;
  const int HW = d->H * d->W;
  if (HW > 64 || 64 % HW != 0 || d->N < 1) return false;
  if (d->x_dtype != LVAE_DT_F32 || d->y_dtype != LVAE_DT_F32 || d->stats_x_dtype != LVAE_DT_F32) return false;
  if ((int64_t)d->N * HW * 128 >= ((int64_t)1 << 31)) return false;
  mi = rb_mi(d);
  const int BM = 32 * mi;
  a.d = *d;
  a.d.in_fold = nullptr;
  a.f = lvae_bn_fold{};
  a.HW = HW;
  a.NI = BM / HW;
  a.halo_h = d->H + 2;
  a.halo_w = d->W + 2;
  a.halo_px = a.NI * a.halo_h * a.halo_w;
  a.flip = d->gather == LVAE_GATHER_TRANSPOSED ? 1 : 0;
  a.nwg = (d->N + a.NI - 1) / a.NI;
  a.m_hw = fastdiv_magic(HW);
  a.m_w = fastdiv_magic(d->W);
  a.m_per_img = fastdiv_magic(a.halo_h * a.halo_w);
  a.m_halo_w = fastdiv_magic(a.halo_w);
  return rb_lds_bytes(rb_split(d), mi, a.halo_px, LVAE_RB_PRO_GATE_BWD, LVAE_RB_EPI_GATE) <= 160 * 1024;
}

template <int SPLIT, int MI, int PRO, int EPI, bool ELU, bool AP = false>
static int rb_launch(const RbArgs& a, hipStream_t s) {
  return launch_lds<rb_conv_kernel<SPLIT, MI, PRO, EPI, ELU, AP>>("resblock_conv", dim3(a.nwg), dim3(256), rb_lds_bytes(SPLIT, MI, a.halo_px, PRO, EPI), 160 * 1024, s, a);
}

static bool rb_all_elu(const RbArgs& a) {
  const lvae_conv_desc& d = a.d;
  const lvae_rb_ext& e = a.e;
  const auto elu = [](int act) { return act == LVAE_ACT_ELU; };
  if (e.prologue == LVAE_RB_PRO_AFFINE && (d.in_scale != nullptr || a.f.parts != nullptr) && !elu(d.in_act)) return false;
  if (e.prologue == LVAE_RB_PRO_BN_APPLY && !elu(e.bwd_act)) return false;
  if (e.prologue == LVAE_RB_PRO_GATE_BWD && e.ap_parts != nullptr && !elu(e.ap_act)) return false;
  if ((e.prologue == LVAE_RB_PRO_GATE_BWD || e.epilogue == LVAE_RB_EPI_GATE) && !elu(e.act)) return false;
  if (d.stats_out != nullptr && d.stats_mode == LVAE_STATS_BN_BWD && !elu(d.stats_act)) return false;
  return true;
}

template <int SPLIT, int MI, bool ELU>
static int rb_dispatch2(const RbArgs& a, hipStream_t s) {
  const int pro = a.e.prologue, epi = a.e.epilogue;
  if (pro == LVAE_RB_PRO_AFFINE) return epi == LVAE_RB_EPI_GATE ? rb_launch<SPLIT, MI, LVAE_RB_PRO_AFFINE, LVAE_RB_EPI_GATE, ELU>(a, s)
                                                                  : rb_launch<SPLIT, MI, LVAE_RB_PRO_AFFINE, LVAE_RB_EPI_PLAIN, ELU>(a, s);
  if (pro == LVAE_RB_PRO_BN_APPLY) return rb_launch<SPLIT, MI, LVAE_RB_PRO_BN_APPLY, LVAE_RB_EPI_PLAIN, ELU>(a, s);
  if (a.e.ap_parts != nullptr) return rb_launch<SPLIT, MI, LVAE_RB_PRO_GATE_BWD, LVAE_RB_EPI_PLAIN, ELU, true>(a, s);
  return rb_launch<SPLIT, MI, LVAE_RB_PRO_GATE_BWD, LVAE_RB_EPI_PLAIN, ELU>(a, s);
}

template <int SPLIT, int MI>
static int rb_dispatch(const RbArgs& a, hipStream_t s) {
  return rb_all_elu(a) ? rb_dispatch2<SPLIT, MI, true>(a, s) : rb_dispatch2<SPLIT, MI, false>(a, s);
}

}

using namespace lvae;

extern "C" size_t lvae_resblock_gate_workspace(const lvae_conv_desc* g) { return rb_gate_ok(g) ? resblock_gate_ws_bytes(g, rb_split(g)) : 0; }

extern "C" int lvae_resblock_gate_prepare_entry(const lvae_conv_desc* g, void* entry) {
  LVAE_REQUIRE(rb_gate_ok(g) && entry, LVAE_EINVAL, "lvae_resblock_gate_prepare_entry: needs a 64 -> 128 or 128 -> 64 1x1 descriptor and an entry buffer");
  LVAE_REQUIRE(g->workspace && (size_t)g->workspace_bytes >= resblock_gate_ws_bytes(g, rb_split(g)) && al16_or_null(g->workspace), LVAE_EINVAL,
               "lvae_resblock_gate_prepare_entry: no scratch for the pre-split gate weights");
  resblock_gate_prep_entry(g, rb_split(g), entry);
  return 0;
}

extern "C" int32_t lvae_resblock_conv_gate_rows(const lvae_conv_desc* d) {
  RbArgs a;
  int mi;
  if (rb_plan(d, a, mi)) return a.nwg;
  return d != nullptr && d->precision == LVAE_PREC_F32 ? conv3x3_wino2_gate_rows(d) : 0;
}

extern "C" int32_t lvae_resblock_conv_rows(const lvae_conv_desc* d) {
  RbArgs a;
  int mi;
  return rb_plan(d, a, mi) ? a.nwg : 0;
}

extern "C" size_t lvae_resblock_conv_workspace(const lvae_conv_desc* d) {
  RbArgs a;
  int mi;
  return rb_plan(d, a, mi) ? conv3x3_bf16_workspace(d, rb_split(d)) : 0;
}

extern "C" int lvae_resblock_conv_prepare_entry(const lvae_conv_desc* d, void* entry) {
  LVAE_REQUIRE(d && entry, LVAE_EINVAL, "lvae_resblock_conv_prepare_entry: null pointer");
  RbArgs a;
  int mi;
  LVAE_REQUIRE(rb_plan(d, a, mi), LVAE_EINVAL, "lvae_resblock_conv_prepare_entry: shape not supported (lvae_resblock_conv_rows(d) == 0)");
  LVAE_REQUIRE(d->workspace && (size_t)d->workspace_bytes >= conv3x3_bf16_workspace(d, rb_split(d)) && al16_or_null(d->workspace), LVAE_EINVAL,
               "lvae_resblock_conv_prepare_entry: no scratch for the pre-split weights");
  conv3x3_bf16_prep_entry(d, rb_split(d), entry);
  return 0;
}

extern "C" int lvae_resblock_conv_f32(const lvae_conv_desc* d, const lvae_rb_ext* ext, void* stream) {
  LVAE_REQUIRE(d != nullptr && d->w != nullptr && d->y != nullptr, LVAE_EINVAL, "lvae_resblock_conv_f32: null descriptor / w / y");
  RbArgs a;
  int mi = 1;
  if (!rb_plan(d, a, mi)) {
    LVAE_REQUIRE(ext != nullptr && ext->prologue == LVAE_RB_PRO_AFFINE && ext->epilogue == LVAE_RB_EPI_GATE && d->precision == LVAE_PREC_F32 &&
                     conv3x3_wino2_gate_rows(d) > 0,
                 LVAE_EINVAL,
                 "lvae_resblock_conv_f32: shape not supported (whole-image kernels: 3x3 / stride 1 / pad 1, 64 -> 64 channels, H*W a divisor of 64, "
                 "fp32 tensors; conv + gate also for lvae_resblock_conv_gate_rows(d) > 0)");
    const lvae_rb_ext& e = *ext;
    LVAE_REQUIRE(e.out && al16_or_null(e.out) && al16_or_null(e.ab) && al16_or_null(e.res) && al16_or_null(e.gate_bias) && al16_or_null(e.out_stats) && al16_or_null(e.out_stats_pivot) &&
                     (e.out_stats == nullptr || e.out_stats_pivot != nullptr) && d->stats_out == nullptr && d->x != nullptr && d->y != nullptr,
                 LVAE_EINVAL, "lvae_resblock_conv_f32: gate epilogue needs x, y, out (16-byte aligned tensors); statistics of y are not available with it");
    lvae_conv_desc g = lvae_conv_desc{};
    g.w = e.gate_w; g.w_sk = e.gate_w_sk; g.w_sn = e.gate_w_sn; g.precision = d->precision; g.C1 = 64; g.Cout = 128;
    g.workspace = e.gate_ws; g.workspace_bytes = e.gate_ws_bytes;
    LVAE_REQUIRE(e.gate_ws != nullptr && al16_or_null(e.gate_ws) && (size_t)e.gate_ws_bytes >= resblock_gate_ws_bytes(&g, 3) && (e.gate_ws_ready || e.gate_w != nullptr),
                 LVAE_EWORKSPACE, "lvae_resblock_conv_f32: gate_ws missing or smaller than lvae_resblock_gate_workspace(), or not ready and no gate_w");
    if (!e.gate_ws_ready) {
      const int rc = resblock_gate_prepare_single(&g, 3, (hipStream_t)stream);
      if (rc) return rc;
    }
    return conv3x3_wino2_gate_launch(d, ext, (hipStream_t)stream);
  }
  const int split = rb_split(d);
  a.e = lvae_rb_ext{};
  if (ext != nullptr) a.e = *ext;
  const lvae_rb_ext& e = a.e;
  const int pro = e.prologue, epi = e.epilogue;
  LVAE_REQUIRE(pro >= LVAE_RB_PRO_AFFINE && pro <= LVAE_RB_PRO_GATE_BWD && (epi == LVAE_RB_EPI_PLAIN || epi == LVAE_RB_EPI_GATE), LVAE_EINVAL,
               "lvae_resblock_conv_f32: bad prologue / epilogue id");
  LVAE_REQUIRE(epi == LVAE_RB_EPI_PLAIN || pro == LVAE_RB_PRO_AFFINE, LVAE_EINVAL, "lvae_resblock_conv_f32: the gate epilogue goes with the forward prologue");
  LVAE_REQUIRE(d->workspace != nullptr && (size_t)d->workspace_bytes >= conv3x3_bf16_workspace(d, split) && al16_or_null(d->workspace), LVAE_EWORKSPACE,
               "lvae_resblock_conv_f32: workspace (pre-split weights) missing or smaller than lvae_resblock_conv_workspace(d)");
  LVAE_REQUIRE(al16_or_null(d->y) && al16_or_null(d->bias) && al16_or_null(d->out_scale) && al16_or_null(d->in_scale) && al16_or_null(d->in_shift) && al16_or_null(d->stats_pivot) &&
                   al16_or_null(d->stats_x) && al16_or_null(d->stats_out),
               LVAE_EALIGN, "lvae_resblock_conv_f32: pointers must be 16-byte aligned");
  LVAE_REQUIRE((d->in_scale == nullptr) || (d->in_shift != nullptr), LVAE_EINVAL, "lvae_resblock_conv_f32: in_scale without in_shift");
  LVAE_REQUIRE(d->stats_out == nullptr || (d->stats_pivot != nullptr && (d->stats_mode == LVAE_STATS_BN_FWD ||
                                                                           (d->stats_mode == LVAE_STATS_BN_BWD && d->stats_x != nullptr))),
               LVAE_EINVAL, "lvae_resblock_conv_f32: bad stats_pivot / stats_mode / stats_x");
  if (pro == LVAE_RB_PRO_AFFINE) {
    LVAE_REQUIRE(d->x != nullptr && al16_or_null(d->x), LVAE_EINVAL, "lvae_resblock_conv_f32: null or unaligned x");
    if (d->in_fold != nullptr) {
      a.f = *d->in_fold;
      LVAE_REQUIRE(a.f.parts != nullptr && al16_or_null(a.f.parts) && a.f.rows > 0 && a.f.M > 0 && d->in_scale == nullptr, LVAE_EINVAL,
                   "lvae_resblock_conv_f32: bad in_fold (parts / rows / M, or in_scale given too)");
    }
  } else {
    LVAE_REQUIRE(d->in_fold == nullptr && d->in_scale == nullptr, LVAE_EINVAL, "lvae_resblock_conv_f32: input transform with a backward prologue");
    LVAE_REQUIRE(al16_or_null(e.pro_drop) && al16_or_null(e.xt_out), LVAE_EALIGN, "lvae_resblock_conv_f32: pro_drop / xt_out must be 16-byte aligned");
  }
  if (pro == LVAE_RB_PRO_BN_APPLY) {
    LVAE_REQUIRE(d->x && e.bwd_x && e.bwd_parts && e.bwd_coef && e.bwd_rows > 0 && e.bwd_M > 0 && al16_or_null(d->x) && al16_or_null(e.bwd_x) &&
                     al16_or_null(e.bwd_parts) && al16_or_null(e.bwd_coef),
                 LVAE_EINVAL, "lvae_resblock_conv_f32: BatchNorm-apply prologue needs x (= dh), bwd_x, bwd_parts / rows / M and the coefficient block, 16-byte aligned");
  }
  if (pro == LVAE_RB_PRO_GATE_BWD) {
    LVAE_REQUIRE((e.dout || e.ap_parts) && e.ab_in && al16_or_null(e.dout) && al16_or_null(e.ab_in) && al16_or_null(e.dab), LVAE_EINVAL,
                 "lvae_resblock_conv_f32: gate-backward prologue needs dout (or the deferred apply that produces it) and ab_in (16-byte aligned tensors)");
    if (e.ap_parts != nullptr) {
      LVAE_REQUIRE(e.ap_rows > 0 && e.ap_M > 0 && e.ap_coef && e.ap_dh && e.ap_x && e.ap_add && e.ap_out && al16_or_null(e.ap_parts) && al16_or_null(e.ap_coef) &&
                       al16_or_null(e.ap_dh) && al16_or_null(e.ap_x) && al16_or_null(e.ap_add) && al16_or_null(e.ap_out),
                   LVAE_EINVAL, "lvae_resblock_conv_f32: deferred apply needs ap_parts / ap_rows / ap_M, the coefficient block, ap_dh, ap_x, ap_add and ap_out, 16-byte aligned");
    }
  } else {
    LVAE_REQUIRE(e.ap_parts == nullptr, LVAE_EINVAL, "lvae_resblock_conv_f32: the deferred apply goes with the gate-backward prologue");
  }
  if (pro == LVAE_RB_PRO_GATE_BWD || epi == LVAE_RB_EPI_GATE) {
    lvae_conv_desc g = lvae_conv_desc{};
    g.w = e.gate_w; g.w_sk = e.gate_w_sk; g.w_sn = e.gate_w_sn; g.precision = d->precision;
    g.C1 = epi == LVAE_RB_EPI_GATE ? 64 : 128; g.Cout = epi == LVAE_RB_EPI_GATE ? 128 : 64;
    g.workspace = e.gate_ws; g.workspace_bytes = e.gate_ws_bytes;
    LVAE_REQUIRE(e.gate_ws != nullptr && al16_or_null(e.gate_ws) && (size_t)e.gate_ws_bytes >= resblock_gate_ws_bytes(&g, split) &&
                     (e.gate_ws_ready || e.gate_w != nullptr),
                 LVAE_EWORKSPACE, "lvae_resblock_conv_f32: gate_ws missing or smaller than lvae_resblock_gate_workspace(), or not ready and no gate_w");
    if (!e.gate_ws_ready) {
      const int rc = resblock_gate_prepare_single(&g, split, (hipStream_t)stream);
      if (rc) return rc;
    }
  }
  if (epi == LVAE_RB_EPI_GATE) {
    LVAE_REQUIRE(e.out && al16_or_null(e.out) && al16_or_null(e.ab) && al16_or_null(e.res) && al16_or_null(e.gate_bias) && al16_or_null(e.out_stats) &&
                     al16_or_null(e.out_stats_pivot) && (e.out_stats == nullptr || e.out_stats_pivot != nullptr) && d->stats_out == nullptr,
                 LVAE_EINVAL, "lvae_resblock_conv_f32: gate epilogue needs out (16-byte aligned tensors); statistics of y are not available with it");
  }
  if (!d->workspace_ready) {
    const int rc = conv3x3_bf16_prepare_single(d, split, (hipStream_t)stream);
    if (rc) return rc;
  }
  a.Wp = static_cast<const __bf16*>(d->workspace);
  hipStream_t s = (hipStream_t)stream;
  if (mi == 1) return split == 1 ? rb_dispatch<1, 1>(a, s) : rb_dispatch<3, 1>(a, s);
  return split == 1 ? rb_dispatch<1, 2>(a, s) : rb_dispatch<3, 2>(a, s);
}

#ifdef LVAE_RB_DBG
extern "C" int lvae_debug_rb_stamps(void* host_out, size_t bytes) {
  return (int)hipMemcpyFromSymbol(host_out, HIP_SYMBOL(lvae::g_rb_stamps), bytes < sizeof(lvae::g_rb_stamps) ? bytes : sizeof(lvae::g_rb_stamps));
}
#endif
```

ladder-vae-pytorch_amd/kernels.py:

```python
import ctypes as C
import weakref

import torch

from . import _C
from ._C import ACT, BnFold, ConvDesc, RbExt, GATHER_CONV, GATHER_TRANSPOSED, PREC_BF16, PREC_F32, call, ptr, ptr_dt, stream_ptr

_ws_cache = {}

precision = PREC_F32


form = _C.FORM_AUTO


class use_form:
    def __init__(self, f):
        self.f = f

    def __enter__(self):
        global form
        self.prev, form = form, self.f

    def __exit__(self, *exc):
# ... 132 lines not shown
                blob = b''.join(e['entry'] for e in ents)
                t = torch.frombuffer(bytearray(blob), dtype=torch.uint8).to(torch.device('cuda', dev))
                self.table[dev] = (t, len(ents), max(e['cout'] for e in ents))
        for dev, ents in by_dev.items():
            t, n, max_cout = self.table[dev]
            with torch.cuda.device(dev):
                call('lvae_conv2d_prepare_weights', t.data_ptr(), n, max_cout, stream_ptr())
            for e in ents:
                w = e['weight']()
                e['stamp'] = self.stamp(w) if w is not None else None
        return len(self.entries)

    def pin_current(self):
        if self.table is None:
            return None
        return (self.table, [e for e in self.entries.values()])

    def invalidate(self):
        for e in self.entries.values():
            e['stamp'] = None

    def weights_written(self):
        self.epoch += 1


prepared = _PreparedWeights()


def _conv_ws(d, weight, device):
    need = _C.load().lvae_conv2d_workspace(C.byref(d))
    if need:
        prepared.attach(d, weight, device, need)


def resblock_bf16_storage(x, weight, g):
    if precision != PREC_BF16 or _ddi is not None or x.dtype != torch.float32:
        return False
    N, H, W, _ = x.shape
    d = _desc(g, weight, x, None, N, H, W, H, W, g.Cout, g.s_ci, g.s_co, GATHER_CONV)
    _conv_ws(d, weight, x.device)
    return bool(_C.load().lvae_resblock_bf16_storage(C.byref(d)))


_ddi = None


def _ddi_conv(state, x, weight, g, bias, x2, in_scale, in_shift, in_act, out_scale, out_act):
    global _ddi
    _ddi = None
    try:
        y = conv2d(x, weight, g, bias=bias, x2=x2, in_scale=in_scale, in_shift=in_shift, in_act=in_act)
        _, _, mean, rstd = bn_stats(y, None, None, None, None, eps=1e-20)
    finally:
        _ddi = state
    scale = 1.0 / (1.0 / rstd + 1e-5)
    weight.mul_(scale.view(1, -1, 1, 1) if g.transposed else scale.view(-1, 1, 1, 1))
    if bias is not None:
        bias.sub_(mean).mul_(scale)
        y = affine_act(y, scale, -mean * scale, None)
    else:
        y = affine_act(y, scale, torch.zeros_like(scale), None)
    if out_scale is not None or out_act is not None:
        ones, zeros = torch.ones_like(scale), torch.zeros_like(scale)
        y = affine_act(y, ones, zeros, out_act, row_scale=out_scale)
    state['done'].add(weight.data_ptr())
    state['count'] += 1
    return y


class StatParts:
    __slots__ = ('buf', 'rows', 'has_pivot')

    def __init__(self, buf, rows, has_pivot):
        self.buf, self.rows, self.has_pivot = buf, rows, has_pivot

    def rows_view(self):
        return self.buf[:self.rows]


def conv2d(x, weight, g, bias=None, x2=None, in_scale=None, in_shift=None, in_act=None, out_scale=None, out_act=None,
           stats_pivot=None, in_bn=None, out_bf16=False):
    if _ddi is not None and weight.data_ptr() not in _ddi['done']:
        assert in_bn is None
        y = _ddi_conv(_ddi, x, weight, g, bias, x2, in_scale, in_shift, in_act, out_scale, out_act)
        return y if stats_pivot is None else (y, None)
    _chk_nhwc(x, 'x')
    N, H, W, C1 = x.shape
    if x2 is not None:
        _chk_nhwc(x2, 'x2')
        assert x2.shape[:3] == x.shape[:3]
    if C1 + (x2.shape[3] if x2 is not None else 0) != g.Cin:
        raise _C.LvaeHipError("conv2d: input has %d channels, weight expects %d" % (C1 + (x2.shape[3] if x2 is not None else 0), g.Cin))
    OH, OW = g.out_size(H, W)
    y = torch.empty((N, OH, OW, g.Cout), dtype=torch.bfloat16 if out_bf16 else torch.float32, device=x.device)
    d = _desc(g, weight, x, x2, N, H, W, OH, OW, g.Cout, g.s_ci, g.s_co,
              GATHER_TRANSPOSED if g.transposed else GATHER_CONV, bias, in_scale, in_shift, in_act, out_scale, out_act, y)
    _conv_ws(d, weight, x.device)
    lib = _C.load()
    coef = fold = None
    if in_bn is not None:
        coef, fold = _in_bn(d, in_bn, x, in_bn[0].has_pivot and x2 is None and bool(lib.lvae_conv2d_folds_bn_finalize(C.byref(d))))
    parts = None
    if stats_pivot is not None:
        rows = lib.lvae_conv2d_stats_rows(C.byref(d))
        if rows > 0:
            buf_rows = lib.lvae_conv2d_stats_buffer_rows(C.byref(d))
            buf = torch.empty((buf_rows, 2, g.Cout), dtype=torch.float32, device=x.device)
            parts = StatParts(buf, rows, buf_rows > rows)
            d.stats_out, d.stats_pivot = ptr(buf), ptr(stats_pivot)
    call('lvae_conv2d_f32', C.byref(d), stream_ptr())
    del fold
    if in_bn is not None:
        return y, parts, coef
    return y if stats_pivot is None else (y, parts)


def conv1x1_gate(x, weight, g, bias, res, act, need_ab=True, stats_pivot=None):
    _chk_nhwc(x, 'x')
    N, H, W, _ = x.shape
    Cn = g.Cout // 2
    lib = _C.load()
    fused = _ddi is None or weight.data_ptr() in _ddi['done']
    if fused:
        ab = torch.empty((N, H, W, g.Cout), dtype=x.dtype, device=x.device) if need_ab else None
        d = _desc(g, weight, x, None, N, H, W, H, W, g.Cout, g.s_ci, g.s_co, GATHER_CONV, bias, y=ab)
        fused = bool(lib.lvae_conv1x1_gate_variant(C.byref(d)))
    if not fused:
        ab = conv2d(x, weight, g, bias=bias)
        out = gate_fwd(ab, res, act)
        return (ab, out) if stats_pivot is None else (ab, out, None)
    out = torch.empty((N, H, W, Cn), dtype=torch.float32, device=x.device)
    parts = None
    if stats_pivot is not None:
        rows = lib.lvae_conv1x1_gate_stats_rows(C.byref(d))
        if rows > 0:
            buf = torch.empty((rows + 1, 2, Cn), dtype=torch.float32, device=x.device)
            parts = StatParts(buf, rows, True)
            d.stats_out, d.stats_pivot = ptr(buf), ptr(stats_pivot)
    call('lvae_conv1x1_gate_f32', C.byref(d), ptr(res), ACT[act], ptr(out), stream_ptr())
    return (ab, out) if stats_pivot is None else (ab, out, parts)


def conv1x1_gate_bwd(dout, ab, weight, g, act, out_scale=None):
    _chk_nhwc(dout, 'dout')
    N, H, W, Cn = dout.shape
    dx = torch.empty((N, H, W, g.Cin), dtype=torch.float32, device=dout.device)
    d = _desc(g, weight, ab, None, N, H, W, H, W, g.Cin, g.s_co, g.s_ci, GATHER_TRANSPOSED, out_scale=out_scale, y=dx)
    if g.Cout != 2 * Cn or not _C.load().lvae_conv1x1_gate_bwd_ok(C.byref(d)):
        dab = gate_bwd(dout, ab, act)
        return dab, conv2d_dgrad(dab, weight, g, (H, W), out_scale=out_scale)
    dab = torch.empty_like(ab)
    call('lvae_conv1x1_gate_bwd_f32', C.byref(d), ptr(dout), ptr(ab), ACT[act], ptr(dab), stream_ptr())
    return dab, dx


def _gate_bwd_fused_desc(x_like, weight, g, dweight):
    N, H, W, Cn = x_like.shape
    if g.Cout != 2 * Cn or (dweight is not None and tuple(dweight.stride()) != tuple(weight.stride())):
        return None
    d = _desc(g, weight, x_like, None, N, H, W, H, W, g.Cin, g.s_co, g.s_ci, GATHER_TRANSPOSED)
    d.C1 = g.Cout
    return d


def gate_bwd_fused_ws(x_like, weight, g, dweight=None):
    d = _gate_bwd_fused_desc(x_like, weight, g, dweight)
    return int(_C.load().lvae_conv1x1_gate_bwd_wgrad_workspace(C.byref(d))) if d is not None else 0


def gate_bwd_apply_ok(x_like, weight, g, dweight=None):
    d = _gate_bwd_fused_desc(x_like, weight, g, dweight)
    return d is not None and bool(_C.load().lvae_conv1x1_gate_bwd_wgrad_apply_ok(C.byref(d)))


gate_bwd_fused_ok = gate_bwd_apply_ok


def conv1x1_gate_bwd_wgrad(dout, ab, y, weight, g, act, dweight, dbias, out_scale=None, out_bf16=False, apply=None):
    _chk_nhwc(dout, 'dout')
    N, H, W, Cn = dout.shape
    if g.Cout != 2 * Cn or tuple(dweight.stride()) != tuple(weight.stride()):
        return None
    if ab.dtype != y.dtype:
        raise _C.LvaeHipError("conv1x1_gate_bwd_wgrad: ab and y must have the same element type")
    dx = torch.empty((N, H, W, g.Cin), dtype=torch.bfloat16 if out_bf16 else torch.float32, device=dout.device)
    d = _desc(g, weight, ab, None, N, H, W, H, W, g.Cin, g.s_co, g.s_ci, GATHER_TRANSPOSED, out_scale=out_scale, y=dx)
    lib = _C.load()
    need = lib.lvae_conv1x1_gate_bwd_wgrad_workspace(C.byref(d))
    if not need or (apply is not None and not lib.lvae_conv1x1_gate_bwd_wgrad_apply_ok(C.byref(d))):
        return None
    ws = workspace(need, dout.device)
    ap = None
    if apply is not None:
        ap = _C.BnApply(ptr(apply.parts), apply.parts.shape[0], ACT[apply.act], N * H * W, ptr(apply.coef0), ptr_dt(apply.dh), ptr(apply.x),
                        ptr(apply.add), ptr(apply.dgamma), ptr(apply.dbeta), ptr(apply.out), int(apply.dh.dtype == torch.bfloat16), 0)
    call('lvae_conv1x1_gate_bwd_wgrad_f32', C.byref(d), ptr(dout), ptr_dt(ab), ptr_dt(y), ACT[act], ptr(dweight), g.s_ci, g.s_co, ptr(dbias),
         ws.data_ptr(), ws.numel(), C.byref(ap) if ap is not None else None, stream_ptr())
    return dx


def gate_bwd_recompute_ok(x_like, weight, g, dweight=None):
    d = _gate_bwd_fused_desc(x_like, weight, g, dweight)
    return d is not None and x_like.dtype == torch.float32 and bool(_C.load().lvae_conv1x1_gate_bwd_wgrad_recompute_ok(C.byref(d)))


def conv1x1_gate_bwd_wgrad_recompute(dout, y, weight, g, bias, act, dweight, dbias, out_scale=None, apply=None):
    _chk_nhwc(dout, 'dout')
    N, H, W, Cn = dout.shape
    if g.Cout != 2 * Cn or tuple(dweight.stride()) != tuple(weight.stride()) or y.dtype != torch.float32:
        return None
    dx = torch.empty((N, H, W, g.Cin), dtype=torch.float32, device=dout.device)
    d = _desc(g, weight, y, None, N, H, W, H, W, g.Cin, g.s_co, g.s_ci, GATHER_TRANSPOSED, out_scale=out_scale, y=dx)
    d.C1 = g.Cout
    lib = _C.load()
    need = lib.lvae_conv1x1_gate_bwd_wgrad_workspace(C.byref(d))
    if not need or not lib.lvae_conv1x1_gate_bwd_wgrad_recompute_ok(C.byref(d)):
        return None
    e = RbExt()
    _rb_gate_ws(e, weight, g, dout.device, False)
    ws = workspace(need, dout.device)
    ap = None
    if apply is not None:
        ap = _C.BnApply(ptr(apply.parts), apply.parts.shape[0], ACT[apply.act], N * H * W, ptr(apply.coef0), ptr_dt(apply.dh), ptr(apply.x),
                        ptr(apply.add), ptr(apply.dgamma), ptr(apply.dbeta), ptr(apply.out), int(apply.dh.dtype == torch.bfloat16), 0)
    call('lvae_conv1x1_gate_bwd_wgrad_recompute_f32', C.byref(d), ptr(dout), ptr(y), ACT[act], e.gate_ws, e.gate_ws_bytes, e.gate_ws_ready,
         e.gate_w, e.gate_w_sk, e.gate_w_sn, ptr(bias), ptr(dweight), g.s_ci, g.s_co, ptr(dbias), ws.data_ptr(), ws.numel(),
         C.byref(ap) if ap is not None else None, stream_ptr())
    return dx


def _rb_desc(x_like, weight, g, dgrad, y=None, bias=None, in_scale=None, in_shift=None, in_act=None, out_scale=None):
    N, H, W, _ = x_like.shape
    if dgrad:
        d = _desc(g, weight, x_like, None, N, H, W, H, W, g.Cin, g.s_co, g.s_ci, GATHER_TRANSPOSED, out_scale=out_scale, y=y)
    else:
        d = _desc(g, weight, x_like, None, N, H, W, H, W, g.Cout, g.s_ci, g.s_co, GATHER_CONV, bias, in_scale, in_shift, in_act, out_scale, None, y)
    need = _C.load().lvae_resblock_conv_workspace(C.byref(d))
    if need:
        prepared.attach(d, weight, x_like.device, need, 'lvae_resblock_conv_prepare_entry')
    return d, need


def _rb_gate_ws(e, gate_w, gate_g, device, bwd):
    gd = ConvDesc()
    gd.w, gd.precision = ptr(gate_w), precision
    if bwd:
        gd.C1, gd.Cout, gd.w_sk, gd.w_sn, gd.gather = gate_g.Cout, gate_g.Cin, gate_g.s_co, gate_g.s_ci, GATHER_TRANSPOSED
    else:
        gd.C1, gd.Cout, gd.w_sk, gd.w_sn, gd.gather = gate_g.Cin, gate_g.Cout, gate_g.s_ci, gate_g.s_co, GATHER_CONV
    need = _C.load().lvae_resblock_gate_workspace(C.byref(gd))
    if not need:
        raise _C.LvaeHipError("fused residual block: the gate convolution must be 1x1, 64 -> 128 channels")
    prepared.attach(gd, gate_w, device, need, 'lvae_resblock_gate_prepare_entry')
    e.gate_w, e.gate_w_sk, e.gate_w_sn = gd.w, gd.w_sk, gd.w_sn
    e.gate_ws, e.gate_ws_bytes, e.gate_ws_ready = gd.workspace, gd.workspace_bytes, gd.workspace_ready
    e._ws_tensor = gd._ws_tensor


def rb_rows(x, weight, g):
    d = _rb_query_desc(x, weight, g)
    return int(_C.load().lvae_resblock_conv_rows(C.byref(d))) if d is not None else 0


def _rb_query_desc(x, weight, g):
    if _ddi is not None or x.dtype != torch.float32 or x.dim() != 4 or g.transposed or g.KH != 3 or g.stride != 1 or g.pad != 1:
        return None
    N, H, W, _ = x.shape
    return _desc(g, weight, x, None, N, H, W, H, W, g.Cout, g.s_ci, g.s_co, GATHER_CONV)


def _in_bn(d, in_bn, x, can_fold=True, coef=None):
    if in_bn is None:
        d.in_scale, d.in_shift = ptr(coef[0]), ptr(coef[1])
        return coef, None
    sp, pivot, bn = in_bn
    N, H, W, C1 = x.shape
    M = N * H * W
    if sp.has_pivot and can_fold:
        coef = torch.empty((4, C1), dtype=torch.float32, device=x.device)
        fold = BnFold(ptr(sp.buf), sp.rows, M, ptr(bn.weight), ptr(bn.bias), bn.eps, bn.momentum, ptr(bn.running_mean),
                      ptr(bn.running_var), ptr(coef))
        d.in_fold = C.addressof(fold)
        return (coef[0], coef[1], coef[2], coef[3]), fold
    coef = bn_finalize_parts(sp.rows_view(), M, pivot, bn.weight, bn.bias, bn.running_mean, bn.running_var, bn.eps, bn.momentum)
    d.in_scale, d.in_shift = ptr(coef[0]), ptr(coef[1])
    return coef, None


def rb_weight_ranges(x_like, weight, g, dgrad, gate=None, gate_bwd=False):
    d, need = _rb_desc(x_like, weight, g, dgrad)
    out = [(int(d.workspace), int(need), d._ws_tensor)] if need else []
    if gate is not None:
        e = RbExt()
        _rb_gate_ws(e, gate[0], gate[1], x_like.device, gate_bwd)
        out.append((int(e.gate_ws), int(e.gate_ws_bytes), e._ws_tensor))
    return out


def _rb_prefetch(e, prefetch):
    for i, rng in enumerate((prefetch or [])[:2]):
        e.pf_ptr[i], e.pf_bytes[i] = rng[0], rng[1]


def rb_conv(x, weight, g, bias, in_act, out_scale, in_bn=None, coef=None, stats_pivot=None, prefetch=None):
    N, H, W, _ = x.shape
    y = torch.empty((N, H, W, g.Cout), dtype=torch.float32, device=x.device)
    d, _ = _rb_desc(x, weight, g, False, y, bias, None, None, in_act, out_scale)
    coef, keep = _in_bn(d, in_bn, x, coef=coef)
    parts = None
    if stats_pivot is not None:
        rows = _C.load().lvae_resblock_conv_rows(C.byref(d))
        buf = torch.empty((rows + 1, 2, g.Cout), dtype=torch.float32, device=x.device)
        parts = StatParts(buf, rows, True)
        d.stats_out, d.stats_pivot = ptr(buf), ptr(stats_pivot)
    e = RbExt()
    e.prologue, e.epilogue = _C.RB_PRO_AFFINE, _C.RB_EPI_PLAIN
    _rb_prefetch(e, prefetch)
    call('lvae_resblock_conv_f32', C.byref(d), C.byref(e), stream_ptr())
    del keep
    return y, parts, coef


def rb_gate_rows(x, weight, g, whole_image=True):
    d = _rb_query_desc(x, weight, g)
    if d is None:
        return 0
    rows = int(_C.load().lvae_resblock_conv_rows(C.byref(d)))
    if rows > 0:
        return rows if whole_image else 0
    _conv_ws(d, weight, x.device)
    return int(_C.load().lvae_resblock_conv_gate_rows(C.byref(d)))


def rb_conv_gate(x, weight, g, bias, in_act, out_scale, gate_w, gate_g, gate_bias, res, act, in_bn=None, coef=None, stats_pivot=None,
                 prefetch=None, want_ab=True):
    N, H, W, _ = x.shape
    dev = x.device
    y = torch.empty((N, H, W, g.Cout), dtype=torch.float32, device=dev)
    out = torch.empty((N, H, W, gate_g.Cout // 2), dtype=torch.float32, device=dev)
    d, need = _rb_desc(x, weight, g, False, y, bias, None, None, in_act, out_scale)
    if need and not want_ab:
        raise _C.LvaeHipError("rb_conv_gate: the whole-image kernels always store ab")
    ab = torch.empty((N, H, W, gate_g.Cout), dtype=torch.float32, device=dev) if want_ab else None
    can_fold = True
    if not need:
        _conv_ws(d, weight, dev)
        can_fold = bool(_C.load().lvae_conv2d_folds_bn_finalize(C.byref(d)))
    coef, keep = _in_bn(d, in_bn, x, can_fold, coef)
    e = RbExt()
    e.prologue, e.epilogue = _C.RB_PRO_AFFINE, _C.RB_EPI_GATE
    _rb_gate_ws(e, gate_w, gate_g, dev, False)
    e.gate_bias, e.act = ptr(gate_bias), ACT[act]
    e.res, e.ab, e.out = ptr(res), ptr(ab), ptr(out)
    parts = None
    if stats_pivot is not None:
        rows = _C.load().lvae_resblock_conv_gate_rows(C.byref(d))
        buf = torch.empty((rows + 1, 2, g.Cout), dtype=torch.float32, device=dev)
        parts = StatParts(buf, rows, True)
        e.out_stats, e.out_stats_pivot = ptr(buf), ptr(stats_pivot)
    _rb_prefetch(e, prefetch)
    call('lvae_resblock_conv_f32', C.byref(d), C.byref(e), stream_ptr())
    del keep
    return y, ab, out, parts, coef


def _rb_bn_bwd(d, bn_bwd, dx):
    xb, coef0, act = bn_bwd
    rows = _C.load().lvae_resblock_conv_rows(C.byref(d))
    parts = torch.empty((rows, 2, dx.shape[3]), dtype=torch.float32, device=dx.device)
    d.stats_out, d.stats_pivot, d.stats_x = ptr(parts), ptr(coef0), ptr(xb)
    d.stats_mode, d.stats_act = 1, ACT[act]
    return parts


class PendingApply:
    __slots__ = ('parts', 'dh', 'x', 'coef0', 'act', 'dgamma', 'dbeta', 'add', 'out')

    def __init__(self, parts, dh, x, coef0, act, dgamma, dbeta, add, out):
        self.parts, self.dh, self.x, self.coef0, self.act, self.dgamma, self.dbeta, self.add, self.out = parts, dh, x, coef0, act, dgamma, dbeta, add, out


def rb_gate_dgrad(dout, ab, gate_w, gate_g, act, drop, weight, g, bn_bwd, prefetch=None, apply=None):
    N, H, W, Cn = dout.shape
    dev = dout.device
    dab = torch.empty_like(ab)
    dy2 = torch.empty((N, H, W, Cn), dtype=torch.float32, device=dev)
    dh = torch.empty((N, H, W, g.Cin), dtype=torch.float32, device=dev)
    d, _ = _rb_desc(dout, weight, g, True, dh)
    e = RbExt()
    e.prologue, e.epilogue = _C.RB_PRO_GATE_BWD, _C.RB_EPI_PLAIN
    _rb_gate_ws(e, gate_w, gate_g, dev, True)
    e.act = ACT[act]
    e.dout, e.ab_in, e.dab, e.pro_drop, e.xt_out = ptr(dout), ptr(ab), ptr(dab), ptr(drop), ptr(dy2)
    if apply is not None:
        e.ap_parts, e.ap_rows, e.ap_act, e.ap_M = ptr(apply.parts), apply.parts.shape[0], ACT[apply.act], N * H * W
        e.ap_coef, e.ap_dh, e.ap_x, e.ap_add = ptr(apply.coef0), ptr(apply.dh), ptr(apply.x), ptr(apply.add)
        e.ap_dgamma, e.ap_dbeta, e.ap_out = ptr(apply.dgamma), ptr(apply.dbeta), ptr(apply.out)
    parts = _rb_bn_bwd(d, bn_bwd, dh)
    _rb_prefetch(e, prefetch)
    call('lvae_resblock_conv_f32', C.byref(d), C.byref(e), stream_ptr())
    return dab, dy2, dh, parts


def rb_apply_dgrad(parts_in, dh_in, x_bn, coef0, act, dgamma, dbeta, drop, weight, g, bn_bwd, prefetch=None):
    N, H, W, Cn = dh_in.shape
    dev = dh_in.device
    dy1 = torch.empty((N, H, W, Cn), dtype=torch.float32, device=dev)
    dh = torch.empty((N, H, W, g.Cin), dtype=torch.float32, device=dev)
    d, _ = _rb_desc(dh_in, weight, g, True, dh)
    e = RbExt()
    e.prologue, e.epilogue = _C.RB_PRO_BN_APPLY, _C.RB_EPI_PLAIN
    e.bwd_parts, e.bwd_rows, e.bwd_act, e.bwd_M = ptr(parts_in), parts_in.shape[0], ACT[act], N * H * W
    e.bwd_coef, e.bwd_x, e.dgamma, e.dbeta, e.pro_drop, e.xt_out = ptr(coef0), ptr(x_bn), ptr(dgamma), ptr(dbeta), ptr(drop), ptr(dy1)
    parts = _rb_bn_bwd(d, bn_bwd, dh)
    _rb_prefetch(e, prefetch)
    call('lvae_resblock_conv_f32', C.byref(d), C.byref(e), stream_ptr())
    return dy1, dh, parts


def bn_coef_block(scale, shift, mean, rstd):
    if scale is None or shift is None or mean is None or rstd is None:
        return False
    n = 4 * scale.numel()
    p0 = scale.data_ptr()
    return shift.data_ptr() == p0 + n and mean.data_ptr() == p0 + 2 * n and rstd.data_ptr() == p0 + 3 * n


def affine_act_bwd_parts(parts, dh, x, scale, shift, act, mean, rstd, dgamma, dbeta, drop=None, add=None, out_bf16=False, out=None):
    Cn = x.shape[-1]
    M = x.numel() // Cn
    dx = out if out is not None else torch.empty(x.shape, dtype=torch.bfloat16 if out_bf16 else torch.float32, device=x.device)
    ws = workspace(8 * Cn, x.device)
    rows_per_n = M // x.shape[0]
    dtypes = _dt(dh) | (_dt(x) << 1) | (_dt(dx) << 2)
    call('lvae_affine_act_bwd_parts_f32', ptr(parts), parts.shape[0], ptr_dt(dh), ptr_dt(x), M, Cn, ptr(scale), ptr(shift), ACT[act],
         ptr(mean), ptr(rstd), ptr(dgamma), ptr(dbeta), ptr(drop), rows_per_n, ptr(add), ptr_dt(dx), ws.data_ptr(), ws.numel(),
         dtypes, stream_ptr())
    return dx


def conv2d_dgrad(dy, weight, g, in_hw, out_scale=None, ci_range=None, bn_bwd=None, out_bf16=False):
    _chk_nhwc(dy, 'dy')
    N, OH, OW, Co = dy.shape
    H, W = in_hw
    a, b = ci_range if ci_range is not None else (0, g.Cin)
    dx = torch.empty((N, H, W, b - a), dtype=torch.bfloat16 if out_bf16 else torch.float32, device=dy.device)
    d = _desc(g, weight, dy, None, N, OH, OW, H, W, b - a, g.s_co, g.s_ci,
              GATHER_CONV if g.transposed else GATHER_TRANSPOSED, out_scale=out_scale, y=dx)
    d.w = ptr(weight) + 4 * a * g.s_ci
    _conv_ws(d, weight, dy.device)
    if bn_bwd is None:
        call('lvae_conv2d_f32', C.byref(d), stream_ptr())
        return dx
    xb, coef, act = bn_bwd
    parts = None
    rows = _C.load().lvae_conv2d_stats_rows(C.byref(d))
    if rows > 0 and out_scale is None and ci_range is None and tuple(xb.shape) == tuple(dx.shape):
        parts = torch.empty((rows, 2, b - a), dtype=torch.float32, device=dy.device)
        d.stats_out, d.stats_pivot, d.stats_x = ptr(parts), ptr(coef), ptr_dt(xb)
        d.stats_mode, d.stats_act, d.stats_x_dtype = 1, ACT[act], _dt(xb)
    call('lvae_conv2d_f32', C.byref(d), stream_ptr())
    return dx, parts


def conv2d_wgrad_apply_ok(x, weight, g):
    if precision != PREC_F32 or x.dtype != torch.float32 or x.dim() != 4 or g.transposed or _ddi is not None:
        return False
    N, H, W, _ = x.shape
    d = _desc(g, weight, x, None, N, H, W, H, W, g.Cout, g.s_ci, g.s_co, GATHER_CONV)
    return bool(_C.load().lvae_conv2d_wgrad_apply_ok(C.byref(d)))


def conv2d_wgrad_apply(x, weight, g, dweight, dbias, parts, dh, xbn, coef0, act, dgamma, dbeta, drop=None, in_scale=None, in_shift=None, in_act=None):
    _chk_nhwc(x, 'x')
    N, H, W, _ = x.shape
    if tuple(dweight.stride()) != tuple(weight.stride()):
        raise _C.LvaeHipError("conv2d_wgrad_apply: gradient strides differ from weight strides")
    d = _desc(g, weight, x, None, N, H, W, H, W, g.Cout, g.s_ci, g.s_co, GATHER_CONV, None, in_scale, in_shift, in_act)
    need = _C.load().lvae_conv2d_wgrad_workspace(C.byref(d))
    ws = workspace(need, x.device)
    dy = torch.empty((N, H, W, g.Cout), dtype=torch.float32, device=x.device)
    ap = _C.BnApply(ptr(parts), parts.shape[0], ACT[act], N * H * W, ptr(coef0), ptr(dh), ptr(xbn), None, ptr(dgamma), ptr(dbeta), ptr(dy), 0, 0, ptr(drop))
    call('lvae_conv2d_wgrad_apply_f32', C.byref(d), C.byref(ap), ptr(dweight), ptr(dbias), ws.data_ptr(), ws.numel(), stream_ptr())
    return dy


def _wgrad_pair_descs(x_a, w_a, g_a, x_b, w_b, g_b, in_a=(None, None, None), in_b=(None, None, None)):
    if precision != PREC_F32 or _ddi is not None or g_a.transposed or g_b.transposed:
        return None
    if x_a.dim() != 4 or x_b.dim() != 4:
        return None
    N, H, W, _ = x_a.shape
    d_a = _desc(g_a, w_a, x_a, None, N, H, W, H, W, g_a.Cout, g_a.s_ci, g_a.s_co, GATHER_CONV, None, *in_a)
    N, H, W, _ = x_b.shape
    d_b = _desc(g_b, w_b, x_b, None, N, H, W, H, W, g_b.Cout, g_b.s_ci, g_b.s_co, GATHER_CONV, None, *in_b)
    return d_a, d_b


def conv2d_wgrad_pair_ok(x_a, w_a, g_a, x_b, w_b, g_b):
    ds = _wgrad_pair_descs(x_a, w_a, g_a, x_b, w_b, g_b)
    return ds is not None and bool(_C.load().lvae_conv2d_wgrad_pair_ok(C.byref(ds[0]), C.byref(ds[1])))


def conv2d_wgrad_pair_schedule(x_a, w_a, g_a, x_b, w_b, g_b):
    ds = _wgrad_pair_descs(x_a, w_a, g_a, x_b, w_b, g_b)
    out = (C.c_int32 * 6)()
    if ds is None or not _C.load().lvae_conv2d_wgrad_pair_schedule(C.byref(ds[0]), C.byref(ds[1]), out):
        return None
    return tuple(out[:3]), tuple(out[3:])


def conv2d_wgrad_pair(x, weight, g, dweight, dbias, parts, dh, xbn, coef0, act, dgamma, dbeta, dy_b, weight_b, g_b, dweight_b, dbias_b,
                      drop=None, in_scale=None, in_shift=None, in_act=None, in_scale_b=None, in_shift_b=None, in_act_b=None, out=None):
    _chk_nhwc(x, 'x')
    _chk_nhwc(xbn, 'xbn')
    _chk_nhwc(dy_b, 'dy_b')
    N, H, W, _ = x.shape
    if tuple(dweight.stride()) != tuple(weight.stride()) or tuple(dweight_b.stride()) != tuple(weight_b.stride()):
        raise _C.LvaeHipError("conv2d_wgrad_pair: gradient strides differ from weight strides")
    ds = _wgrad_pair_descs(x, weight, g, xbn, weight_b, g_b, (in_scale, in_shift, in_act), (in_scale_b, in_shift_b, in_act_b))
    if ds is None:
        raise _C.LvaeHipError("conv2d_wgrad_pair: not a pair (fp32 precision, plain convolutions)")
    d_a, d_b = ds
    d_b.y_dtype = _dt(dy_b)
    need = _C.load().lvae_conv2d_wgrad_pair_workspace(C.byref(d_a), C.byref(d_b))
    ws = workspace(need, x.device)
    dy = out if out is not None else torch.empty((N, H, W, g.Cout), dtype=torch.float32, device=x.device)
    ap = _C.BnApply(ptr(parts), parts.shape[0], ACT[act], N * H * W, ptr(coef0), ptr(dh), ptr(xbn), None, ptr(dgamma), ptr(dbeta), ptr(dy), 0, 0, ptr(drop))
    call('lvae_conv2d_wgrad_pair_f32', C.byref(d_a), C.byref(ap), C.byref(d_b), ptr_dt(dy_b), ptr(dweight), ptr(dbias), ptr(dweight_b), ptr(dbias_b),
         ws.data_ptr(), ws.numel(), stream_ptr())
    return dy


def conv1x1_dgrad_cat(dy, weight, g, C1):
    _chk_nhwc(dy, 'dy')
    N, H, W, _ = dy.shape
    if not 0 < C1 < g.Cin:
        return None
    dx = torch.empty((N, H, W, C1), dtype=torch.float32, device=dy.device)
    dx2 = torch.empty((N, H, W, g.Cin - C1), dtype=torch.float32, device=dy.device)
    d = _desc(g, weight, dy, None, N, H, W, H, W, g.Cin, g.s_co, g.s_ci, GATHER_TRANSPOSED, y=dx)
    if not _C.load().lvae_conv1x1_dgrad_cat_ok(C.byref(d), C1):
        return None
    call('lvae_conv1x1_dgrad_cat_f32', C.byref(d), ptr(dx2), C1, stream_ptr())
    return dx, dx2


def _cat_bwd_desc(dy_like, weight, g, C1, dweight):
    if _ddi is not None or dy_like.dim() != 4 or g.transposed or dy_like.dtype != torch.float32 or not 0 < C1 < g.Cin:
        return None
    if dweight is not None and tuple(dweight.stride()) != tuple(weight.stride()):
        return None
    N, H, W, _ = dy_like.shape
    return _desc(g, weight, dy_like, None, N, H, W, H, W, g.Cin, g.s_co, g.s_ci, GATHER_TRANSPOSED)


def cat_bwd_ws(dy_like, weight, g, C1, dweight=None):
    d = _cat_bwd_desc(dy_like, weight, g, C1, dweight)
    return int(_C.load().lvae_conv1x1_cat_bwd_workspace(C.byref(d), C1)) if d is not None else 0


def cat_bwd_apply_ok(dy_like, weight, g, C1, dweight=None):
    d = _cat_bwd_desc(dy_like, weight, g, C1, dweight)
    return d is not None and bool(_C.load().lvae_conv1x1_cat_bwd_apply_ok(C.byref(d), C1))


def conv1x1_cat_bwd(dy, x, x2, weight, g, dweight, dbias, apply=None, store_dy=False, max_workgroups=0, scratch=None):
    _chk_nhwc(dy, 'dy')
    C1 = x.shape[3]
    d = _cat_bwd_desc(dy, weight, g, C1, dweight)
    if d is None or x.dtype != torch.float32 or x2 is None or x2.dtype != torch.float32 or tuple(x.shape[:3]) != tuple(dy.shape[:3]) or \
            tuple(x2.shape[:3]) != tuple(dy.shape[:3]) or x2.shape[3] != g.Cin - C1 or not (x.is_contiguous() and x2.is_contiguous()):
        return None
    lib = _C.load()
    need = lib.lvae_conv1x1_cat_bwd_workspace(C.byref(d), C1)
    if not need or (apply is not None and (not lib.lvae_conv1x1_cat_bwd_apply_ok(C.byref(d), C1) or apply.dh.dtype != torch.float32)):
        return None
    ws = scratch if scratch is not None else workspace(need, dy.device)
    if ws.numel() < need or ws.data_ptr() % 16 or any(t is not None and t.data_ptr() % 16 for t in (x, x2)):
        return None
    N, H, W, _ = dy.shape
    ap = None
    if apply is not None:
        d.x = None
        ap = _C.BnApply(ptr(apply.parts), apply.parts.shape[0], ACT[apply.act], N * H * W, ptr(apply.coef0), ptr(apply.dh), ptr(apply.x),
                        ptr(apply.add), ptr(apply.dgamma), ptr(apply.dbeta), ptr(apply.out) if store_dy else None, 0, 0)
    dx = torch.empty((N, H, W, C1), dtype=torch.float32, device=dy.device)
    dx2 = torch.empty((N, H, W, g.Cin - C1), dtype=torch.float32, device=dy.device)
    call('lvae_conv1x1_cat_bwd_f32', C.byref(d), ptr(x), ptr(x2), ptr(dx), ptr(dx2), ptr(dweight), ptr(dbias),
         C.byref(ap) if ap is not None else None, ws.data_ptr(), ws.numel(), int(max_workgroups), stream_ptr())
    return dx, dx2


def conv2d_wgrad(x, dy, weight, g, dweight, dbias=None, x2=None, in_scale=None, in_shift=None, in_act=None):
    _chk_nhwc(x, 'x')
    _chk_nhwc(dy, 'dy')
    N, H, W, _ = x.shape
    OH, OW = dy.shape[1], dy.shape[2]
    if tuple(dweight.stride()) != tuple(weight.stride()):
        raise _C.LvaeHipError("conv2d_wgrad: gradient strides %s differ from weight strides %s" %
                              (tuple(dweight.stride()), tuple(weight.stride())))
    d = _desc(g, weight, x, x2, N, H, W, OH, OW, g.Cout, g.s_ci, g.s_co,
              GATHER_TRANSPOSED if g.transposed else GATHER_CONV, None, in_scale, in_shift, in_act)
    d.y_dtype = _dt(dy)
    need = _C.load().lvae_conv2d_wgrad_workspace(C.byref(d))
    ws = workspace(need, x.device)
    call('lvae_conv2d_wgrad_f32', C.byref(d), ptr_dt(dy), ptr(dweight), ptr(dbias), ws.data_ptr(), ws.numel(), stream_ptr())


def _wgrad_item_arrays(items, who):
    n = len(items)
    descs = (ConvDesc * n)()
    dys, dws, dbs = (C.c_void_p * n)(), (C.c_void_p * n)(), (C.c_void_p * n)()
    for i, (x, dy, weight, g, dweight, dbias, kw) in enumerate(items):
        _chk_nhwc(x, 'x')
        _chk_nhwc(dy, 'dy')
        if tuple(dweight.stride()) != tuple(weight.stride()):
            raise _C.LvaeHipError("%s: gradient strides %s differ from weight strides %s" %
                                  (who, tuple(dweight.stride()), tuple(weight.stride())))
        N, H, W, _ = x.shape
        d = _desc(g, weight, x, kw.get('x2'), N, H, W, dy.shape[1], dy.shape[2], g.Cout, g.s_ci, g.s_co,
                  GATHER_TRANSPOSED if g.transposed else GATHER_CONV, None, kw.get('in_scale'), kw.get('in_shift'), kw.get('in_act'))
        d.y_dtype = _dt(dy)
        C.memmove(C.byref(descs, i * C.sizeof(ConvDesc)), C.byref(d), C.sizeof(ConvDesc))
        dys[i], dws[i], dbs[i] = ptr_dt(dy), ptr(dweight), ptr(dbias)
    return descs, dys, dws, dbs


def _wgrad_shared_descs(convs):
    if precision != PREC_F32 or _ddi is not None or not 1 <= len(convs) <= 3:
        return None
    descs = (ConvDesc * len(convs))()
    for i, (x, weight, g) in enumerate(convs):
        if x.dim() != 4 or x.dtype != torch.float32 or g.transposed:
            return None
        N, H, W, _ = x.shape
        d = _desc(g, weight, x, None, N, H, W, H, W, g.Cout, g.s_ci, g.s_co, GATHER_CONV)
        C.memmove(C.byref(descs, i * C.sizeof(ConvDesc)), C.byref(d), C.sizeof(ConvDesc))
    return descs


def conv2d_wgrad_shared_ok(convs, routed=False):
    descs = _wgrad_shared_descs(convs)
    if descs is None or not _C.load().lvae_conv2d_wgrad_shared_ok(descs, None, len(convs)):
        return False
    if not routed:
        return True
    wide = [i for i in range(len(convs)) if descs[i].C1 == 64]
    return bool(wide) and all(_C.load().lvae_conv2d_wgrad_variant(C.byref(descs[i])) == _C.WGRAD_VARIANT_WINO for i in wide)


def conv2d_wgrad_shared_schedule(convs):
    descs = _wgrad_shared_descs(convs)
    out = (C.c_int32 * (3 * len(convs)))()
    if descs is None or not _C.load().lvae_conv2d_wgrad_shared_schedule(descs, None, len(convs), out):
        return None
    return tuple(tuple(out[3 * i:3 * i + 3]) for i in range(len(convs)))


def conv2d_wgrad_shared(items):
    n = len(items)
    descs, dys, dws, dbs = _wgrad_item_arrays(items, 'conv2d_wgrad_shared')
    need = _C.load().lvae_conv2d_wgrad_shared_workspace(descs, n)
    ws = workspace(need, items[0][0].device)
    call('lvae_conv2d_wgrad_shared_f32', descs, C.cast(dys, C.c_void_p), C.cast(dws, C.c_void_p), C.cast(dbs, C.c_void_p), n,
         ws.data_ptr(), ws.numel(), stream_ptr())


def conv2d_wgrad_grouped(items):
    n = len(items)
    descs, dys, dws, dbs = _wgrad_item_arrays(items, 'conv2d_wgrad_grouped')
    need = _C.load().lvae_conv2d_wgrad_grouped_workspace(descs, n)
    ws = workspace(need, items[0][0].device)
    call('lvae_conv2d_wgrad_grouped_f32', descs, C.cast(dys, C.c_void_p), C.cast(dws, C.c_void_p), C.cast(dbs, C.c_void_p), n,
         ws.data_ptr(), ws.numel(), stream_ptr())


def bn_stats(x, gamma, beta, running_mean, running_var, eps=1e-5, momentum=0.1):
    Cn = x.shape[-1]
    M = x.numel() // Cn
    out = torch.empty((4, Cn), dtype=torch.float32, device=x.device)
    need = _C.load().lvae_bn_stats_workspace(M, Cn)
    ws = workspace(need, x.device)
    call('lvae_bn_stats_f32', ptr(x), M, Cn, ptr(gamma), ptr(beta), eps, momentum, ptr(running_mean), ptr(running_var),
         ptr(out[0]), ptr(out[1]), ptr(out[2]), ptr(out[3]), ws.data_ptr(), ws.numel(), stream_ptr())
    return out[0], out[1], out[2], out[3]


def bn_finalize_parts(parts, M, pivot, gamma, beta, running_mean, running_var, eps=1e-5, momentum=0.1):
    rows, _, Cn = parts.shape
    out = torch.empty((4, Cn), dtype=torch.float32, device=parts.device)
    call('lvae_bn_finalize_parts_f32', ptr(parts), rows, M, Cn, ptr(pivot), ptr(gamma), ptr(beta), eps, momentum,
         ptr(running_mean), ptr(running_var), ptr(out[0]), ptr(out[1]), ptr(out[2]), ptr(out[3]), stream_ptr())
    return out[0], out[1], out[2], out[3]


def bn_eval_coeffs(gamma, beta, running_mean, running_var, eps=1e-5):
    Cn = running_mean.numel()
    out = torch.empty((2, Cn), dtype=torch.float32, device=running_mean.device)
    call('lvae_bn_eval_coeffs_f32', Cn, ptr(gamma), ptr(beta), ptr(running_mean), ptr(running_var), eps, ptr(out[0]),
         ptr(out[1]), stream_ptr())
    return out[0], out[1]


def affine_act(x, scale, shift, act, row_scale=None):
    Cn = x.shape[-1]
    M = x.numel() // Cn
    y = torch.empty_like(x)
    rows_per_n = M // x.shape[0]
    call('lvae_affine_act_f32', ptr(x), M, Cn, ptr(scale), ptr(shift), ACT[act], ptr(row_scale), rows_per_n, ptr(y),
         stream_ptr())
    return y


# ... 826 lines not shown
```

ladder-vae-pytorch_amd/ops.py:

```python
from types import SimpleNamespace

import torch
from torch.autograd import Function

from . import kernels as K
from . import resblock as RB

_const_cache = {}


def _ones_zeros(C, device):
    key = (C, device)
    if key not in _const_cache:
        _const_cache[key] = (torch.ones(C, device=device), torch.zeros(C, device=device))
    return _const_cache[key]


def grad_buf(p):
    if not p.requires_grad:
        return None
    if p.grad is None:
        p.grad = torch.zeros_like(p)
    return p.grad


def _c(t):
    return t if t.is_contiguous() else t.contiguous()


_side = {'stream': None}


def set_wgrad_stream(streams):
    if streams is None:
        _side['stream'] = None
    else:
        _side['stream'] = list(streams) if isinstance(streams, (list, tuple)) else [streams]


def join_wgrad_stream():
    sts = _side['stream']
    if sts is not None:
        for st in sts:
            torch.cuda.current_stream().wait_stream(st)


def set_wgrad_grouping(max_rows, flush_at=None):
    flush_wgrad_group()
    _side['group_rows'] = max_rows
    _side['group_at'] = RB.switches.wgrad_flush if flush_at is None else flush_at


def flush_wgrad_group():
    q, _side['group_q'] = _side.get('group_q') or [], []
    if len(q) == 1:
        x, dy, w, g, dw, db, kw = q[0]
        K.conv2d_wgrad(x, dy, w, g, dw, db, **kw)
    elif q:
        K.conv2d_wgrad_grouped(q)


def drop_wgrad_group():
    _side['group_q'] = []


def wgrad(x, dy, w, g, dw, db, **kw):
    rows = _side.get('group_rows')
    if rows is not None and x.shape[0] * x.shape[1] * x.shape[2] <= rows:
        q = _side.setdefault('group_q', [])
        if any(e[4].data_ptr() == dw.data_ptr() for e in q):
            flush_wgrad_group()
            q = _side['group_q']
        q.append((x, dy, w, g, dw, db, kw))
        if len(q) >= _side.get('group_at', 1024):
            flush_wgrad_group()
        return
    sts = _side['stream']
    if sts is None:
        return K.conv2d_wgrad(x, dy, w, g, dw, db, **kw)
    st = sts[(dw.data_ptr() >> 8) % len(sts)]
    st.wait_stream(torch.cuda.current_stream())
    with torch.cuda.stream(st):
        K.conv2d_wgrad(x, dy, w, g, dw, db, **kw)
    for t in (x, dy, kw.get('x2'), kw.get('in_scale'), kw.get('in_shift')):
        if t is not None:
            t.record_stream(st)


class WgradShare:

    def __init__(self, n_in):
        self.items, self.wait = [], n_in

    @staticmethod
    def plan(convs):
        if not (RB.switches.wgrad_shared and torch.is_grad_enabled() and all(m.weight.requires_grad for _, m in convs)):
            return None
        if not K.conv2d_wgrad_shared_ok([(x, m.weight, m.geom()) for x, m in convs], routed=True):
            return None
        return WgradShare(len(convs) - 1)

    def add(self, item, is_input):
        self.items.append(item)
        self.wait -= int(is_input)
        if self.wait > 0:
            return
        items, self.items = self.items, []
        if (len(items) >= 2 and _side['stream'] is None and all(it[1].dtype == torch.float32 for it in items) and
                K.conv2d_wgrad_shared_ok([(it[0], it[2], it[3]) for it in items])):
            K.conv2d_wgrad_shared(items)
        else:
            for x, dy, w, g, dw, db, kw in items:
                wgrad(x, dy, w, g, dw, db, **kw)


class ConvFn(Function):

    @staticmethod
    def forward(ctx, x, x2, mod, out_act, weight, bias, share=None):
        g = mod.geom()
        y = K.conv2d(x, weight, g, bias=bias, x2=x2, out_act=out_act)
        ctx.mod, ctx.out_act, ctx.g, ctx.share = mod, out_act, g, share
        ctx.has_x2 = x2 is not None
        ctx.save_for_backward(x, x2, y if out_act else None)
        return y

    @staticmethod
    def backward(ctx, dy):
        x, x2, y = ctx.saved_tensors
        mod, g = ctx.mod, ctx.g
        dy = _c(dy)
        w = mod.weight
        if x2 is not None:
            st = getattr(mod, 'sched', None)
            pend = st.take_pending(dy) if st is not None else None
            if (RB.switches.merge_bwd_fused and not ctx.out_act and w.requires_grad and ctx.needs_input_grad[0] and ctx.needs_input_grad[1] and
                    _side['stream'] is None and dy.dtype == torch.float32 and
                    dy.shape[0] * dy.shape[1] * dy.shape[2] >= RB.switches.merge_bwd_min_rows):
                both = K.conv1x1_cat_bwd(dy, x, x2, w, g, grad_buf(w), grad_buf(mod.bias) if mod.bias is not None else None, apply=pend)
                if both is not None:
                    return both + (None,) * 5
            if pend is not None:
                C = pend.coef0.numel()
                sc, sh, mean, rstd = torch.as_strided(pend.coef0, (4, C), (C, 1)).unbind(0)
                K.affine_act_bwd_parts(pend.parts, pend.dh, pend.x, sc, sh, pend.act, mean, rstd, pend.dgamma, pend.dbeta, add=pend.add, out=pend.out)
        if ctx.out_act:
            dy = K.act_bwd_from_out(dy, y, ctx.out_act)
        if w.requires_grad:
            db = grad_buf(mod.bias) if mod.bias is not None else None
            if ctx.share is not None and x2 is None:
                ctx.share[0].add((x, dy, w, g, grad_buf(w), db, {}), ctx.share[1])
            else:
                wgrad(x, dy, w, g, grad_buf(w), db, x2=x2)
        dx = dx2 = None
        hw = (x.shape[1], x.shape[2])
        if x2 is None:
            if ctx.needs_input_grad[0]:
                dx = K.conv2d_dgrad(dy, w, g, hw)
        else:
            C1 = x.shape[3]
            both = K.conv1x1_dgrad_cat(dy, w, g, C1) if (RB.switches.dgrad_cat and ctx.needs_input_grad[0] and ctx.needs_input_grad[1]) else None
            if both is not None:
                dx, dx2 = both
            else:
                if ctx.needs_input_grad[0]:
                    dx = K.conv2d_dgrad(dy, w, g, hw, ci_range=(0, C1))
                if ctx.needs_input_grad[1]:
                    dx2 = K.conv2d_dgrad(dy, w, g, hw, ci_range=(C1, g.Cin))
        return dx, dx2, None, None, None, None, None


def merge_announces(x, x2, mod, y, out_act):
    sw = RB.switches
    if not (sw.merge_bwd_fused and x2 is not None and out_act is None and mod.training and torch.is_grad_enabled()):
        return False
    if not (mod.weight.requires_grad and x.requires_grad and x2.requires_grad and y.dtype == torch.float32):
        return False
    if y.shape[0] * y.shape[1] * y.shape[2] < sw.merge_bwd_min_rows:
        return False
    return K.cat_bwd_apply_ok(y, mod.weight, mod.geom(), x.shape[3], mod.weight.grad)


def conv(x, mod, x2=None, out_act=None, share=None):
    st = getattr(mod, 'sched', None)
    if st is not None:
        st.pending = None
    y = ConvFn.apply(x, x2, mod, out_act, mod.weight, mod.bias, share)
    if st is not None and merge_announces(x, x2, mod, y, out_act):
        y._lvae_handover = RB.Handover(None, None, st, 'any-dh')
    return y


def _bn_of_half(h, bn, training, parts, pivot):
    if bn is None:
        return None, _ones_zeros(h.shape[3], h.device) + (None, None)
    if not training:
        return None, K.bn_eval_coeffs(bn.weight, bn.bias, bn.running_mean, bn.running_var, bn.eps) + (None, None)
    if parts is not None:
        return (parts, pivot, bn), None
    return None, K.bn_stats(h, bn.weight, bn.bias, bn.running_mean, bn.running_var, bn.eps, bn.momentum)


def _conv_half(h, bn, cv, act, m, training, parts, pivot, stats_pivot, s16):
    in_bn, coef = _bn_of_half(h, bn, training, parts, pivot)
    if in_bn is not None:
        return K.conv2d(h, cv.weight, cv.geom(), bias=cv.bias, in_act=act, out_scale=m, in_bn=in_bn, stats_pivot=stats_pivot, out_bf16=s16)
    r = K.conv2d(h, cv.weight, cv.geom(), bias=cv.bias, in_scale=coef[0], in_shift=coef[1], in_act=act, out_scale=m, stats_pivot=stats_pivot,
                 out_bf16=s16)
    return (r if stats_pivot is not None else (r, None)) + (coef,)


def _fwd_fused_gate(call, x, blk, m1, m2, training):
    act, st, bn2, cv1, cv2, gate = blk.act, blk.sched, blk.bn2, blk.conv1, blk.conv2, blk.gate
    whole = call.plan.forward == 'whole-image'
    if whole:
        in_bn, coef1 = _bn_of_half(x, blk.bn1, True, call.parts, call.pivot)
        st.link('fwd', K.rb_weight_ranges(x, cv1.weight, cv1.geom(), False))
        y1, parts2, coef1 = K.rb_conv(x, cv1.weight, cv1.geom(), cv1.bias, act, m1, in_bn=in_bn, coef=coef1, stats_pivot=bn2.running_mean,
                                      prefetch=K.rb_weight_ranges(x, cv2.weight, cv2.geom(), False, gate=(gate.weight, gate.geom())))
    else:
        y1, parts2, coef1 = _conv_half(x, blk.bn1, cv1, act, m1, True, call.parts, call.pivot, bn2.running_mean, False)
    in_bn, coef2 = _bn_of_half(y1, bn2, True, parts2, bn2.running_mean)
    call.out_pivot = coef1[2].detach() if call.plan.gate_stats else None
    y2, ab, out, call.out_parts, coef2 = K.rb_conv_gate(y1, cv2.weight, cv2.geom(), cv2.bias, act, m2, gate.weight, gate.geom(), gate.bias, x, act,
                                                        in_bn=in_bn, coef=coef2, stats_pivot=call.out_pivot,
                                                        prefetch=st.next_ranges('fwd') if whole else None,
                                                        want_ab=not call.plan.recompute_ab)
    return y1, y2, ab, out, coef1, coef2


def _fwd_per_op(call, x, blk, m1, m2, training):
    act, bn2, gate, s16 = blk.act, blk.bn2, blk.gate, call.plan.bf16_internals
    want_stats = training and bn2 is not None and bn2.running_mean is not None
    y1, parts2, coef1 = _conv_half(x, blk.bn1, blk.conv1, act, m1, training, call.parts, call.pivot, bn2.running_mean if want_stats else None, s16)
    y2, _, coef2 = _conv_half(y1, bn2, blk.conv2, act, m2, training, parts2, bn2.running_mean if bn2 is not None else None, None, s16)
    if gate is None:
        return y1, y2, None, K.add(y2, x), coef1, coef2
    call.out_pivot = coef1[2].detach() if call.plan.gate_stats else None
    r = K.conv1x1_gate(y2, gate.weight, gate.geom(), gate.bias, x, act, stats_pivot=call.out_pivot)
    ab, out, call.out_parts = r if call.out_pivot is not None else r + (None,)
    return y1, y2, ab, out, coef1, coef2


class ResBlockFn(Function):

    @staticmethod
    def forward(ctx, x, blk, m1, m2, training, call, *params):
        plan, fwd = call.plan, _fwd_fused_gate if call.plan.forward in ('whole-image', 'wino-gate') else _fwd_per_op
        y1, y2, ab, out, coef1, coef2 = fwd(call, x, blk, m1, m2, training)
        if plan.backward == 'whole-image' and not (K.bn_coef_block(*coef1) and K.bn_coef_block(*coef2)):
            call.plan = plan = plan._replace(backward='composed', accepts=None)
        ctx.blk, ctx.plan, ctx.training, ctx.defer = blk, plan, training, call.defer
        ctx.save_for_backward(x, y1, y2, ab, *coef1, *coef2, m1, m2)
        return out

    @staticmethod
    def backward(ctx, dout):
        blk, plan, act = ctx.blk, ctx.plan, ctx.blk.act
        x, y1, y2, ab, sc1, sh1, mean1, rstd1, sc2, sh2, mean2, rstd2, m1, m2 = ctx.saved_tensors
        coef1, coef2 = (sc1, sh1, mean1, rstd1), (sc2, sh2, mean2, rstd2)
        dout = _c(dout)
        if plan.backward == 'whole-image':
            dh1, parts1 = _bwd_whole_image(blk, dout, x, y1, y2, ab, coef1, coef2, m1, m2)
        else:
            dy2 = _bwd_gate(blk, plan, dout, y2, ab, m2)
            cv1, bn2 = blk.conv1, blk.bn2
            cv2 = blk.conv2
            paired = (plan.wgrad_pair and _side['stream'] is None and dy2.dtype == torch.float32 and bn2 is not None and ctx.training and
                      K.bn_coef_block(*coef2))
            dh2, parts2 = _bwd_half(ctx, cv2, bn2, y1, dy2, coef2, wgrad_done=paired)
            absorbed = (plan.wgrad_absorbs_apply and parts2 is not None and _side['stream'] is None and dh2.dtype == torch.float32)
            if paired and absorbed:
                dy1 = K.conv2d_wgrad_pair(x, cv1.weight, cv1.geom(), grad_buf(cv1.weight), grad_buf(cv1.bias), parts2, dh2, y1, sc2, act,
                                          grad_buf(bn2.weight), grad_buf(bn2.bias), dy2, cv2.weight, cv2.geom(), grad_buf(cv2.weight),
                                          grad_buf(cv2.bias), drop=m1, in_scale=sc1, in_shift=sh1, in_act=act, in_scale_b=sc2, in_shift_b=sh2,
                                          in_act_b=act)
            elif absorbed:
                dy1 = K.conv2d_wgrad_apply(x, cv1.weight, cv1.geom(), grad_buf(cv1.weight), grad_buf(cv1.bias), parts2, dh2, y1, sc2, act,
                                           grad_buf(bn2.weight), grad_buf(bn2.bias), drop=m1, in_scale=sc1, in_shift=sh1, in_act=act)
            else:
                if paired:
                    wgrad(y1, dy2, cv2.weight, cv2.geom(), grad_buf(cv2.weight), grad_buf(cv2.bias), in_scale=sc2, in_shift=sh2, in_act=act)
                dy1 = _bwd_apply(ctx, bn2, parts2, dh2, y1, coef2, drop=m1, out_bf16=plan.bf16_internals)
            dh1, parts1 = _bwd_half(ctx, cv1, blk.bn1, x, dy1, coef1, wgrad_done=absorbed)
        if parts1 is not None and ctx.defer is not None and (dh1.dtype == torch.float32 or ctx.defer[1] == 'any-dh') and K.bn_coef_block(*coef1):
            dx = torch.empty_like(x)
            ctx.defer[0].pending = K.PendingApply(parts1, dh1, x, sc1, act, grad_buf(blk.bn1.weight), grad_buf(blk.bn1.bias), dout, dx)
        else:
            dx = _bwd_apply(ctx, blk.bn1, parts1, dh1, x, coef1, add=dout)
        return (dx, None, None, None, None, None) + (None,) * (len(ctx.needs_input_grad) - 6)


def _bwd_whole_image(blk, dout, x, y1, y2, ab, coef1, coef2, m1, m2):
    act, st, gate, cv2, cv1, bn2 = blk.act, blk.sched, blk.gate, blk.conv2, blk.conv1, blk.bn2
    gw, w2, w1 = gate.weight, cv2.weight, cv1.weight
    st.link('bwd', K.rb_weight_ranges(dout, w2, cv2.geom(), True, gate=(gw, gate.geom()), gate_bwd=True))
    dab, dy2, dh2, parts2 = K.rb_gate_dgrad(dout, ab, gw, gate.geom(), act, m2, w2, cv2.geom(), bn_bwd=(y1, coef2[0], act),
                                            prefetch=K.rb_weight_ranges(dout, w1, cv1.geom(), True), apply=st.take_pending(dout))
    if gw.requires_grad:
        wgrad(y2, dab, gw, gate.geom(), grad_buf(gw), grad_buf(gate.bias))
    wgrad(y1, dy2, w2, cv2.geom(), grad_buf(w2), grad_buf(cv2.bias), in_scale=coef2[0], in_shift=coef2[1], in_act=act)
    dy1, dh1, parts1 = K.rb_apply_dgrad(parts2, dh2, y1, coef2[0], act, grad_buf(bn2.weight), grad_buf(bn2.bias), m1, w1, cv1.geom(),
                                        bn_bwd=(x, coef1[0], act), prefetch=st.next_ranges('bwd'))
    wgrad(x, dy1, w1, cv1.geom(), grad_buf(w1), grad_buf(cv1.bias), in_scale=coef1[0], in_shift=coef1[1], in_act=act)
    return dh1, parts1


def _bwd_gate(blk, plan, dout, y2, ab, m2):
    gate, act, s16 = blk.gate, blk.act, plan.bf16_internals
    if gate is None:
        return K.scale_rows_add(dout, m2, None) if m2 is not None else dout
    gw = gate.weight
    if plan.backward == 'persistent-gate':
        if plan.recompute_ab:
            dy2 = K.conv1x1_gate_bwd_wgrad_recompute(dout, y2, gw, gate.geom(), gate.bias, act, grad_buf(gw), grad_buf(gate.bias), out_scale=m2,
                                                     apply=blk.sched.take_pending(dout))
        else:
            dy2 = K.conv1x1_gate_bwd_wgrad(dout, ab, y2, gw, gate.geom(), act, grad_buf(gw), grad_buf(gate.bias), out_scale=m2, out_bf16=s16,
                                           apply=blk.sched.take_pending(dout))
        if dy2 is None:
            raise K._C.LvaeHipError("residual block: the persistent gate backward the block was planned with did not take this shape")
        return dy2
    if s16:
        raise K._C.LvaeHipError("bf16-stored residual block: the fused gate backward did not take this shape")
    dab, dy2 = K.conv1x1_gate_bwd(dout, ab, gw, gate.geom(), act, out_scale=m2)
    wgrad(y2, dab, gw, gate.geom(), grad_buf(gw), grad_buf(gate.bias))
    return dy2


def _bwd_half(ctx, cv, bn, h, dy, coef, wgrad_done=False):
    w, g, act = cv.weight, cv.geom(), ctx.blk.act
    if not wgrad_done:
        wgrad(h, dy, w, g, grad_buf(w), grad_buf(cv.bias), in_scale=coef[0], in_shift=coef[1], in_act=act)
    if bn is not None and ctx.training and K.bn_coef_block(*coef):
        return K.conv2d_dgrad(dy, w, g, h.shape[1:3], bn_bwd=(h, coef[0], act), out_bf16=ctx.plan.bf16_internals)
    return K.conv2d_dgrad(dy, w, g, h.shape[1:3]), None


def _bwd_apply(ctx, bn, parts, dh, h, coef, drop=None, add=None, out_bf16=False):
    sc, sh, mean, rstd = coef
    train = bn is not None and ctx.training
    dgamma, dbeta = (grad_buf(bn.weight), grad_buf(bn.bias)) if train else (None, None)
    if parts is not None:
        return K.affine_act_bwd_parts(parts, dh, h, sc, sh, ctx.blk.act, mean, rstd, dgamma, dbeta, drop=drop, add=add, out_bf16=out_bf16)
    return K.affine_act_bwd(dh, h, sc, sh, ctx.blk.act, train, mean, rstd, dgamma, dbeta, drop=drop, add=add)


def residual_block(x, blk, m1, m2):
    training = blk.training
    blk.sched.pending = None
    parts, pivot, defer = RB.received(x, training)
    call = SimpleNamespace(plan=RB.plan_block(blk, x, training), parts=parts, pivot=pivot, defer=defer, out_parts=None, out_pivot=None)
    out = ResBlockFn.apply(x, blk, m1, m2, training, call, *blk.parameters())
    return RB.tagged(out, blk, call.plan, call.out_parts, call.out_pivot)


class BnDropFn(Function):

    @staticmethod
    def forward(ctx, x, bn, mask, training, *params):
        _, (sc, sh, mean, rstd) = _bn_of_half(x, bn, training, None, None)
        y = K.affine_act(x, sc, sh, None, row_scale=mask)
        ctx.bn, ctx.training = bn, training
        ctx.save_for_backward(x, sc, sh, mean, rstd, mask)
        return y

    @staticmethod
    def backward(ctx, dy):
        x, sc, sh, mean, rstd, mask = ctx.saved_tensors
        dy = _c(dy)
        if mask is not None:
            dy = K.scale_rows_add(dy, mask, None)
        bn = ctx.bn
        train = bn is not None and ctx.training
        dx = K.affine_act_bwd(dy, x, sc, sh, None, train, mean, rstd, grad_buf(bn.weight) if train else None,
                              grad_buf(bn.bias) if train else None)
        return (dx, None, None, None) + (None,) * (len(ctx.needs_input_grad) - 4)


class GateFn(Function):

    @staticmethod
    def forward(ctx, ab, res, act):
        ctx.act = act
        ctx.has_res = res is not None
        ctx.save_for_backward(ab)
        return K.gate_fwd(ab, res, act)

    @staticmethod
    def backward(ctx, dout):
        (ab,) = ctx.saved_tensors
        dout = _c(dout)
        return K.gate_bwd(dout, ab, ctx.act), (dout if ctx.has_res else None), None


class AddFn(Function):
    @staticmethod
    def forward(ctx, a, b):
        return K.add(a, b)

    @staticmethod
    def backward(ctx, d):
        return d, d


class NormalStochFn(Function):

    @staticmethod
    def forward(ctx, p, q, noise, mode, analytical, Z, N, rows=None):
        z, lp, lq, kl, ks = K.normal_stochastic_fwd(p, q, noise, mode, analytical, Z, N, rows=rows)
        ctx.set_materialize_grads(False)
        ctx.mode, ctx.analytical, ctx.Z = mode, analytical, Z
        ctx.has_q = q is not None
        ctx.p_bcast = p.shape[0] == 1 and N > 1
        ctx.save_for_backward(p, q, noise if mode == 0 else None, z)
        if q is None:
            return z, lp
        return z, lp, lq, kl, ks

    @staticmethod
    def backward(ctx, dz, g_lp, g_lq=None, g_kl=None, g_ks=None):
        p, q, eps, z = ctx.saved_tensors
        cc = lambda t: None if t is None else _c(t)
        if dz is None and g_lp is None and g_lq is None and g_kl is None and g_ks is None:
            return None, None, None, None, None, None, None, None
        dp, dq = K.normal_stochastic_bwd(p, q, eps, z, cc(dz), cc(g_lp), cc(g_lq), cc(g_kl), cc(g_ks), ctx.mode,
                                         ctx.analytical, ctx.Z)
        if ctx.p_bcast:
            red = torch.empty_like(p)
            K.colsum(dp.view(dp.shape[0], -1), red.view(-1), False)
            dp = red
        return dp, dq, None, None, None, None, None, None


class StochBlockFn(Function):

    @staticmethod
    def forward(ctx, x_p, p_given, x_q, noise, blk, mode, analytical, N, rows, *params):
        cv = lambda m: (m.weight, m.geom(), m.bias)
        has_p = x_p is not None
        out, z, p, q, lp, lq, kl, ks = K.stoch_block_fwd(x_p, cv(blk.conv_in_p) if has_p else None, p_given, x_q, cv(blk.conv_in_q), cv(blk.conv_out),
                                                         noise, mode, analytical, N, rows=rows)
        ctx.set_materialize_grads(False)
        ctx.blk, ctx.mode, ctx.analytical, ctx.has_p = blk, mode, analytical, has_p
        ctx.p_bcast = p.shape[0] == 1 and N > 1
        ctx.save_for_backward(x_p, p, x_q, q, noise if mode == 0 else None, z)
        return (out, z, q, lp, lq, kl, ks) + ((p,) if has_p else ())

    @staticmethod
    def backward(ctx, d_out, dz, dq_out, g_lp, g_lq, g_kl, g_ks, dp_out=None):
        x_p, p, x_q, q, eps, z = ctx.saved_tensors
        none = (None,) * len(ctx.needs_input_grad)
        if all(g is None for g in (d_out, dz, dq_out, g_lp, g_lq, g_kl, g_ks, dp_out)):
            return none
        cc = lambda t: None if t is None else _c(t)
        cv = lambda m: None if m is None else (m.weight, m.geom(), m.bias)
        co, cq, cp = ctx.blk.conv_out, ctx.blk.conv_in_q, ctx.blk.conv_in_p if ctx.has_p else None
        hw = (z.shape[1], z.shape[2])
        d_out, dz, g = cc(d_out), cc(dz), (cc(g_lp), cc(g_lq), cc(g_kl), cc(g_ks))
        one = None
        if d_out is not None and dq_out is None and dp_out is None and RB.switches.stoch_block_bwd:
            one = K.stoch_block_bwd(d_out, cv(cp), cv(cq), cv(co), p, q, z, eps, dz, *g, ctx.mode, ctx.analytical)
        if one is not None:
            dp, dq, dx_p, dx_q = one
        else:
            if d_out is not None:
                dzc = K.conv2d_dgrad(d_out, co.weight, co.geom(), hw)
                dz = dzc if dz is None else K.add(dzc, dz)
            dp, dq = K.normal_stochastic_bwd(p, q, eps, z, dz, *g, ctx.mode, ctx.analytical, z.shape[3])
            if dq_out is not None:
                dq = K.add(dq, _c(dq_out))
            if dp_out is not None:
                dp = K.add(dp, _c(dp_out))
            dx_q = K.conv2d_dgrad(dq, cq.weight, cq.geom(), hw) if ctx.needs_input_grad[2] else None
            dx_p = K.conv2d_dgrad(dp, cp.weight, cp.geom(), hw) if cp is not None and ctx.needs_input_grad[0] else None
        for m, x, dy in ((co, z, d_out), (cq, x_q, dq), (cp, x_p, dp)):
            if m is not None and dy is not None and m.weight.requires_grad:
                wgrad(x, dy, m.weight, m.geom(), grad_buf(m.weight), grad_buf(m.bias))
        dpg = None
        if cp is None and ctx.needs_input_grad[1]:
            dpg = dp
            if ctx.p_bcast:
                dpg = torch.empty_like(p)
                K.colsum(dp.view(dp.shape[0], -1), dpg.view(-1), False)
        return (dx_p, dpg, dx_q) + none[3:]


class KlElementwiseFn(Function):

    @staticmethod
    def forward(ctx, z, p, q, analytical):
        ctx.analytical = analytical
        ctx.save_for_backward(z, p, q)
        return K.kl_elementwise_fwd(p, q, z, analytical)

    @staticmethod
    def backward(ctx, g):
        z, p, q = ctx.saved_tensors
        dp, dq, dz = K.kl_elementwise_bwd(p, q, z, _c(g), ctx.analytical, need_dz=ctx.needs_input_grad[0])
        out = []
        for t, d in ((p, dp), (q, dq)):
            if t.shape[0] == 1 and d.shape[0] > 1:
                red = torch.empty_like(t)
                K.colsum(d.view(d.shape[0], -1), red.view(-1), False)
                d = red
            out.append(d)
        return dz, out[0], out[1], None


class BernoulliFn(Function):

    @staticmethod
    def forward(ctx, logits, x, u):
        mean, mode, sample, ll, dll = K.bernoulli_fwd(logits, x, u, True)
        ctx.save_for_backward(dll)
        ctx.mark_non_differentiable(mode, sample)
        ctx.has_ll = ll is not None
        if ll is None:
            ll = torch.zeros((logits.shape[0],), device=logits.device)
        return ll, mean, mode, sample

    @staticmethod
    def backward(ctx, g_ll, g_mean, g_mode, g_sample):
        (dll,) = ctx.saved_tensors
        if dll is None:
            return None, None, None
        return K.scale_per_sample(dll, _c(g_ll)), None, None


class GaussianFn(Function):

    @staticmethod
    def forward(ctx, params, x, eps):
        sample, ll, dll = K.gaussian_fwd(params, x, eps, True)
        ctx.save_for_backward(dll)
        ctx.mark_non_differentiable(sample)
        if ll is None:
            ll = torch.zeros((params.shape[0],), device=params.device)
        return ll, sample

    @staticmethod
    def backward(ctx, g_ll, g_sample):
        (dll,) = ctx.saved_tensors
        return (K.scale_per_sample(dll, _c(g_ll)) if dll is not None else None), None, None


class DiscrLogisticFn(Function):

    @staticmethod
    def forward(ctx, raw, x, u):
        mean, ls, sample, ll, dll = K.discr_logistic_fwd(raw, x, u, True)
        ctx.save_for_backward(dll)
        ctx.mark_non_differentiable(mean, ls, sample)
        if ll is None:
            ll = torch.zeros((raw.shape[0],), device=raw.device)
        return ll, mean, ls, sample

    @staticmethod
    def backward(ctx, g_ll, g_mean, g_ls, g_sample):
        (dll,) = ctx.saved_tensors
        return (K.scale_per_sample(dll, _c(g_ll)) if dll is not None else None), None, None


class DmolFn(Function):

    @staticmethod
    def forward(ctx, l, x):
        ll, dl = K.dmol_ll_fwd(l, x, True)
        ctx.save_for_backward(dl)
        return ll

    @staticmethod
    def backward(ctx, g_ll):
        (dl,) = ctx.saved_tensors
        return K.scale_per_sample(dl, _c(g_ll)), None


def _filled_out(ctx, filled_out):
    if filled_out is not None:
        ctx.mark_dirty(filled_out)


class BernoulliMaskedFn(Function):
    @staticmethod
    def forward(ctx, logits, x, u, mask, filled_out=None):
        _filled_out(ctx, filled_out)
        mean, mode, sample, ll, dll, filled = K.bernoulli_masked_fwd(logits, x, u, mask, True, filled_out)
        ctx.save_for_backward(dll)
        ctx.mark_non_differentiable(mode, sample, filled)
        return ll, mean, mode, sample, filled

    @staticmethod
    def backward(ctx, g_ll, g_mean, g_mode, g_sample, g_filled):
        (dll,) = ctx.saved_tensors
        return K.scale_per_sample(dll, _c(g_ll)), None, None, None, None


class GaussianMaskedFn(Function):
    @staticmethod
    def forward(ctx, params, x, eps, mask, filled_out=None):
        _filled_out(ctx, filled_out)
        sample, ll, dll, filled = K.gaussian_masked_fwd(params, x, eps, mask, True, filled_out)
        ctx.save_for_backward(dll)
        ctx.mark_non_differentiable(sample, filled)
        return ll, sample, filled

# ... 230 lines not shown
```

ladder-vae-pytorch_amd/resblock.py:

```python
import os
import weakref
from typing import NamedTuple, Optional

import torch

from . import kernels as K


class Switches:

    def __init__(self, env):
        on = lambda name: env.get(name, '1') != '0'
        self.wgrad_flush = int(env.get('LVAE_WGRAD_FLUSH', '1024'))
        self.dgrad_cat = on('LVAE_DGRAD_CAT')
        self.wgrad_apply = on('LVAE_WGRAD_APPLY')
        self.wgrad_apply_maxw = int(env.get('LVAE_WGRAD_APPLY_MAXW', '16'))
        self.wgrad_pair = on('LVAE_WGRAD_PAIR')
        self.wgrad_pair_maxw = int(env.get('LVAE_WGRAD_PAIR_MAXW', '16'))
        self.wgrad_shared = on('LVAE_WGRAD_SHARED')
        self.merge_bwd_fused = on('LVAE_MERGE_BWD_FUSED')
        self.merge_bwd_min_rows = int(env.get('LVAE_MERGE_BWD_MIN_ROWS', '65536'))
        self.gate_stats = env.get('LVAE_NO_GATE_STATS') is None
        self.defer_apply = on('LVAE_DEFER_APPLY')
        self.defer_apply_large = on('LVAE_DEFER_APPLY_LARGE')
        self.rb_fwd_min_hw, self.rb_bwd_min_hw = int(env.get('LVAE_RB_FWD_MIN_HW', '16')), int(env.get('LVAE_RB_BWD_MIN_HW', '1'))
        self.rb_gate_large = on('LVAE_RB_GATE_LARGE')
        self.stoch_block = on('LVAE_STOCH_BLOCK')
        self.stoch_block_bwd = on('LVAE_STOCH_BLOCK_BWD')
        self.gate_recompute = on('LVAE_GATE_RECOMPUTE')
        self.gate_recompute_maxw = int(env.get('LVAE_GATE_RECOMPUTE_MAXW', '16'))


switches = Switches(os.environ)


class BlockPlan(NamedTuple):
    forward: str
    bf16_internals: bool
    gate_stats: bool
    backward: Optional[str]
    wgrad_absorbs_apply: bool
    wgrad_pair: bool
    accepts: Optional[str]
    recompute_ab: bool = False


def plan_block(blk, x, training):
    sw, grad = switches, torch.is_grad_enabled()
    cv1, cv2, gate, bn1, bn2 = blk.conv1, blk.conv2, blk.gate, blk.bn1, blk.bn2
    gated_bn = gate is not None and bn1 is not None and bn2 is not None and gate.bias is not None
    full = (training and gated_bn and cv1.bias is not None and cv2.bias is not None and bn1.running_mean is not None and
            bn2.running_mean is not None and x.dtype == torch.float32)
    hw = x.shape[1] * x.shape[2]
    whole = full and K.rb_rows(x, cv1.weight, cv1.geom()) > 0
    whole_fwd, whole_bwd = whole and 0 < sw.rb_fwd_min_hw <= hw, whole and 0 < sw.rb_bwd_min_hw <= hw
    s16 = bool(not whole_fwd and not whole_bwd and gated_bn and K.resblock_bf16_storage(x, cv1.weight, cv1.geom()))
    if whole_fwd:
        forward = 'whole-image'
    elif full and not s16 and sw.rb_gate_large and K.rb_gate_rows(x, cv2.weight, cv2.geom(), whole_image=False) > 0:
        forward = 'wino-gate'
    else:
        forward = 'per-op' if gate is not None else 'ungated'
    gate_stats = gate is not None and training and bn1 is not None and bn1.running_mean is not None and sw.gate_stats
    backward, accepts, absorbs, pair = None, None, False, False
    if grad and whole_bwd:
        backward, accepts = 'whole-image', 'f32-dh'
    elif grad:
        backward = 'composed'
        if gate is not None and gate.bias is not None and gate.weight.requires_grad and \
                K.gate_bwd_fused_ws(x, gate.weight, gate.geom(), gate.weight.grad) > 0:
            backward = 'persistent-gate'
            if training and not whole_fwd and sw.defer_apply_large and K.gate_bwd_apply_ok(x, gate.weight, gate.geom(), gate.weight.grad):
                accepts = 'any-dh'
        absorbs = bool(training and bn2 is not None and sw.wgrad_apply and not s16 and cv1.weight.requires_grad and
                       x.shape[2] <= sw.wgrad_apply_maxw and K.conv2d_wgrad_apply_ok(x, cv1.weight, cv1.geom()))
        pair = bool(absorbs and sw.wgrad_pair and cv2.weight.requires_grad and x.shape[2] <= sw.wgrad_pair_maxw and
                    K.conv2d_wgrad_pair_ok(x, cv1.weight, cv1.geom(), x, cv2.weight, cv2.geom()))
    recompute = bool(forward == 'wino-gate' and backward == 'persistent-gate' and not s16 and sw.gate_recompute and
                     x.shape[2] <= sw.gate_recompute_maxw and K.gate_bwd_recompute_ok(x, gate.weight, gate.geom(), gate.weight.grad))
    return BlockPlan(forward, s16, gate_stats, backward, absorbs, pair, accepts, recompute)


class Handover(NamedTuple):
    parts: object
    pivot: object
    producer: object = None
    accepts: Optional[str] = None


def passed_on(src, aliases):
    h = getattr(src, '_lvae_handover', None)
    if h is not None and h.parts is not None:
        for a in aliases:
            a._lvae_handover = Handover(h.parts, h.pivot)


def received(x, training):
    h = getattr(x, '_lvae_handover', None) or Handover(None, None)
    defer = None
    if h.producer is not None:
        x._lvae_handover = h._replace(producer=None)
        if training and torch.is_grad_enabled() and switches.defer_apply and x.dtype == torch.float32:
            defer = (h.producer, h.accepts)
    return (h.parts, h.pivot, defer) if training else (None, None, defer)


def tagged(out, blk, plan, parts, pivot):
    producer = blk.sched if (plan.accepts and blk.training and torch.is_grad_enabled()) else None
    if parts is not None or producer is not None:
        out._lvae_handover = Handover(parts, pivot, producer, plan.accepts)
    return out


class BlockState:
    __slots__ = ('pending', 'first', 'next', '__weakref__')

    def __init__(self):
        self.pending, self.first, self.next = None, {}, weakref.WeakValueDictionary()

    def __reduce__(self):
        return BlockState, ()

    def take_pending(self, dout):
        pend, self.pending = self.pending, None
        if pend is not None and pend.out.data_ptr() != dout.data_ptr():
            raise K._C.LvaeHipError("deferred BatchNorm-backward apply: the gradient that reached the consuming block is not the tensor the "
                                    "producer left unwritten (the block output has another consumer?)")
        return pend

    _last = weakref.WeakValueDictionary()

    def link(self, direction, first_ranges):
        self.first[direction] = first_ranges
        prev = BlockState._last.get(direction)
        if prev is not None and prev is not self:
            prev.next[direction] = self
        BlockState._last[direction] = self

    def next_ranges(self, direction):
        nb = self.next.get(direction)
        return nb.first.get(direction) if nb is not None else None
```

Before: 9788 images/s.

## Split resblock conv tiles across two workgroups by output-channel half when grid is small

Adds an NS=2 variant of the resblock conv kernel in which two workgroups share each 32-pixel tile, each computing one 32-channel half of the output. Duplicate side outputs (xt_out, dab, ap_out) are written only by the first half, and stats and y stores are partitioned by channel half. The goal is to fill more of the GPU when the tile count is small (at most 128 tiles), at the cost of both workgroups redoing the prologue and halo loads. The auto heuristic turns this on by default for SPLIT=3, MI=1 and plain epilogues, and an env override is provided.

```diff
diff --git a/include/lvae_hip.h b/include/lvae_hip.h
--- a/include/lvae_hip.h
+++ b/include/lvae_hip.h
@@ -187,10 +187,12 @@
   float* ap_dgamma;
   float* ap_dbeta;
   float* ap_out;
+  int32_t nsplit;
 } lvae_rb_ext;
 size_t lvae_resblock_gate_workspace(const lvae_conv_desc* g);
 int lvae_resblock_gate_prepare_entry(const lvae_conv_desc* g, void* entry);
 int32_t lvae_resblock_conv_rows(const lvae_conv_desc* d);
+int32_t lvae_resblock_conv_nsplit(const lvae_conv_desc* d, const lvae_rb_ext* ext);
 int32_t lvae_resblock_conv_gate_rows(const lvae_conv_desc* d);
 size_t lvae_resblock_conv_workspace(const lvae_conv_desc* d);
 int lvae_resblock_conv_prepare_entry(const lvae_conv_desc* d, void* entry);
diff --git a/ladder-vae-pytorch_amd/_C.py b/ladder-vae-pytorch_amd/_C.py
--- a/ladder-vae-pytorch_amd/_C.py
+++ b/ladder-vae-pytorch_amd/_C.py
@@ -57,7 +57,7 @@
                 ('pf_ptr', C.c_void_p * 2), ('pf_bytes', C.c_int64 * 2),
                 ('ap_parts', C.c_void_p), ('ap_rows', C.c_int32), ('ap_act', C.c_int32), ('ap_M', C.c_int64), ('ap_coef', C.c_void_p),
                 ('ap_dh', C.c_void_p), ('ap_x', C.c_void_p), ('ap_add', C.c_void_p), ('ap_dgamma', C.c_void_p), ('ap_dbeta', C.c_void_p),
-                ('ap_out', C.c_void_p)]
+                ('ap_out', C.c_void_p), ('nsplit', C.c_int32)]
 
 
 class StochBlock(C.Structure):
@@ -129,6 +129,7 @@
     'lvae_resblock_gate_workspace': (_Z, [C.POINTER(ConvDesc)]),
     'lvae_resblock_gate_prepare_entry': (C.c_int, [C.POINTER(ConvDesc), _P]),
     'lvae_resblock_conv_rows': (_I, [C.POINTER(ConvDesc)]),
+    'lvae_resblock_conv_nsplit': (_I, [C.POINTER(ConvDesc), C.POINTER(RbExt)]),
     'lvae_resblock_conv_gate_rows': (_I, [C.POINTER(ConvDesc)]),
     'lvae_resblock_conv_workspace': (_Z, [C.POINTER(ConvDesc)]),
     'lvae_resblock_conv_prepare_entry': (C.c_int, [C.POINTER(ConvDesc), _P]),
diff --git a/ladder-vae-pytorch_amd/csrc/resblock_img.hip b/ladder-vae-pytorch_amd/csrc/resblock_img.hip
--- a/ladder-vae-pytorch_amd/csrc/resblock_img.hip
+++ b/ladder-vae-pytorch_amd/csrc/resblock_img.hip
@@ -84,9 +84,11 @@
   lds_barrier();
 }
 
-template <int SPLIT, int MI, int PRO, int EPI, bool ELU, bool AP = false>
+template <int SPLIT, int MI, int PRO, int EPI, bool ELU, bool AP = false, int NS = 1>
 __global__ __launch_bounds__(256) void rb_conv_kernel(RbArgs a) {
   static_assert(MI == 1 || MI == 2, "32- or 64-pixel tiles (MI 32-row blocks)");
+  static_assert(NS == 1 || (NS == 2 && MI == 1 && EPI == LVAE_RB_EPI_PLAIN), "two workgroups per tile: 32-pixel tiles with the plain epilogue");
+  constexpr int NH = 2 / NS;
   static_assert(!AP || PRO == LVAE_RB_PRO_GATE_BWD, "the deferred apply feeds the gate-backward prologue");
   constexpr int BM = 32 * MI, LDK = RB_LDK, LDO = RB_LDO, NQ = BM / 16;
   constexpr int OS_BYTES = BM * LDO * 4;
@@ -105,7 +107,10 @@
   const int wm = MI == 2 ? wave >> 1 : 0, wn = wave & 1, li = lane & 31, lh = lane >> 5;
   const bool g1_on = MI == 2 || wave < 2;
   const int bid = blockIdx.x;
-  const int n0 = bid * a.NI, HW = a.HW;
+  const int tile = NS == 2 ? bid >> 1 : bid, half = NS == 2 ? bid & 1 : 0;
+  const bool once = half == 0;
+  const bool mine = NS == 1 || ((t & 15) >> 3) == half;
+  const int n0 = tile * a.NI, HW = a.HW;
   const int nvalid = min(BM, (d.N - n0) * HW);
   const size_t row0 = (size_t)n0 * HW;
   const int c4 = (t & 15) * 4, p0 = t >> 4;
@@ -113,15 +118,14 @@
   const f32x4 one4 = {1.f, 1.f, 1.f, 1.f};
 
   constexpr int RING = SPLIT == 1 ? 9 : 3;
-  bf16x8 bq[RING][2][SPLIT];
-  const __bf16* wp_lane = a.Wp + (size_t)wave * SPLIT * 1024 + (size_t)lane * 8;
-  auto load_b = [&](int tap, bf16x8 (&r)[2][SPLIT]) {
+  bf16x8 bq[RING][NH][SPLIT];
+  const __bf16* wp_lane = a.Wp + (size_t)wave * SPLIT * 1024 + (size_t)lane * 8 + (NS == 2 ? half * 512 : 0);
+  auto load_b = [&](int tap, bf16x8 (&r)[NH][SPLIT]) {
     const __bf16* src = wp_lane + (size_t)tap * 4 * SPLIT * 1024;
 #pragma unroll
-    for (int p = 0; p < SPLIT; ++p) {
-      r[0][p] = *reinterpret_cast<const bf16x8*>(src + p * 1024);
-      r[1][p] = *reinterpret_cast<const bf16x8*>(src + p * 1024 + 512);
-    }
+    for (int p = 0; p < SPLIT; ++p)
+#pragma unroll
+      for (int nh = 0; nh < NH; ++nh) r[nh][p] = *reinterpret_cast<const bf16x8*>(src + p * 1024 + nh * 512);
   };
   RB_STAMP_DECL;
 #ifdef LVAE_RB_DBG_REPS
@@ -136,7 +140,7 @@
   auto pf_issue = [&]() {
 #pragma unroll
     for (int k = 0; k < 2; ++k) {
-      const int per_xcd = (a.nwg + 7) >> 3, part = bid >> 3;
+      const int per_xcd = (a.nwg * NS + 7) >> 3, part = bid >> 3;
       const int lines = e.pf_ptr[k] != nullptr ? (int)((e.pf_bytes[k] + 127) >> 7) : 0, per = (lines + per_xcd - 1) / per_xcd;
       const int lo = part * per, hi = min(lo + per, lines);
       const char* base = static_cast<const char*>(e.pf_ptr[k]) + (size_t)(lo + t) * 128;
@@ -266,7 +270,7 @@
       const f32x4 g = gv[q] * act_grad4(xv[q] * sc + sh, bwd_act);
       f32x4 v = bn_bwd_apply(g, xv[q], c1, c2, mu, rs, sc) * dm[q];
       if (!ok[q]) v = zero4;
-      if (ok[q] && e.xt_out) store_wt4(e.xt_out + grow[q] * 64 + c4, v);
+      if (ok[q] && once && e.xt_out) store_wt4(e.xt_out + grow[q] * 64 + c4, v);
       put_interior(q, v);
     }
   }
@@ -310,7 +314,7 @@
         const f32x4 g = go[q] * act_grad4(xa[q] * sc + sh, ap_act);
         const f32x4 v = bn_bwd_apply(g, xa[q], c1, c2, mu, rs, sc) + ad[q];
         go[q] = v;
-        if (ok[q]) store_wt4(e.ap_out + grow[q] * 64 + c4, v);
+        if (ok[q] && once) store_wt4(e.ap_out + grow[q] * 64 + c4, v);
       }
     } else {
       pf_issue();
@@ -345,7 +349,7 @@
       da = da * act_grad4(aa[q], gate_act);
       db = db * act_fwd4(aa[q], gate_act);
       if (!ok[q]) da = db = zero4;
-      if (ok[q] && e.dab) {
+      if (ok[q] && once && e.dab) {
         store_wt4(e.dab + grow[q] * 128 + c4, da);
         store_wt4(e.dab + grow[q] * 128 + 64 + c4, db);
       }
@@ -385,7 +389,7 @@
       const int p = p0 + 16 * q;
       f32x4 v = *reinterpret_cast<const f32x4*>(Os1 + p * LDO + c4) * dm[q];
       if (!ok[q]) v = zero4;
-      if (ok[q] && e.xt_out) store_wt4(e.xt_out + grow[q] * 64 + c4, v);
+      if (ok[q] && once && e.xt_out) store_wt4(e.xt_out + grow[q] * 64 + c4, v);
       put_interior(q, v);
     }
     zero_ring();
@@ -436,11 +440,11 @@
     const int ty = fastdiv(r, a.m_w), tx = r - ty * d.W;
     hbase[mb] = ((img * a.halo_h + ty) * a.halo_w + tx) * LDK + wave * 16 + 8 * lh;
   }
-  f32x16 acc[MI][2];
+  f32x16 acc[MI][NH];
 #pragma unroll
   for (int mb = 0; mb < MI; ++mb)
 #pragma unroll
-    for (int nh = 0; nh < 2; ++nh)
+    for (int nh = 0; nh < NH; ++nh)
 #pragma unroll
       for (int r = 0; r < 16; ++r) acc[mb][nh][r] = 0.f;
 
@@ -467,7 +471,7 @@
 #pragma unroll
       for (int mb = 0; mb < MI; ++mb)
 #pragma unroll
-        for (int nh = 0; nh < 2; ++nh) acc[mb][nh] = mfma_pieces<SPLIT>(af[cur][mb], bq[tap % RING][nh], acc[mb][nh]);
+        for (int nh = 0; nh < NH; ++nh) acc[mb][nh] = mfma_pieces<SPLIT>(af[cur][mb], bq[tap % RING][nh], acc[mb][nh]);
       if (tap + RING < 9) load_b(tap + RING, bq[tap % RING]);
     }
   }
@@ -493,10 +497,10 @@
 #pragma unroll
   for (int mb = 0; mb < MI; ++mb)
 #pragma unroll
-    for (int nh = 0; nh < 2; ++nh)
+    for (int nh = 0; nh < NH; ++nh)
 #pragma unroll
       for (int r = 0; r < 16; ++r)
-        Os[wave * OSW + (mb * 32 + (r & 3) + 8 * (r >> 2) + 4 * lh) * LDO + nh * 32 + li] = acc[mb][nh][r];
+        Os[wave * OSW + (mb * 32 + (r & 3) + 8 * (r >> 2) + 4 * lh) * LDO + (NS == 2 ? half : nh) * 32 + li] = acc[mb][nh][r];
   lds_barrier();
   RB_STAMP(5);
   auto os_sum = [&](int p) {
@@ -518,7 +522,7 @@
     for (int q = 0; q < NQ; ++q) {
       const int p = p0 + 16 * q;
       const f32x4 v = (os_sum(p) + ep_bias) * ep_mask[q];
-      if (ok[q]) {
+      if (ok[q] && mine) {
         store_wt4(d.y + grow[q] * 64 + c4, v);
         if (stats_out) {
           if (stats_fwd) {
@@ -605,8 +609,10 @@
       float v = 0.f;
 #pragma unroll
       for (int r = 0; r < 16; ++r) v += red[which * 1024 + r * 64 + c];
-      stats_out[((size_t)bid * 2 + which) * 64 + c] = v;
-      if (bid == 0 && which == 0 && stats_fwd) stats_out[((size_t)a.nwg * 2) * 64 + c] = stats_pivot[c];
+      if (NS == 1 || (c >> 5) == half) {
+        stats_out[((size_t)tile * 2 + which) * 64 + c] = v;
+        if (tile == 0 && which == 0 && stats_fwd) stats_out[((size_t)a.nwg * 2) * 64 + c] = stats_pivot[c];
+      }
     }
   }
   RB_STAMP(7);
@@ -629,6 +635,11 @@
   const int HW = d->H * d->W;
   if (HW <= 16 && 32 % HW == 0 && ((int64_t)d->N * HW + 63) / 64 <= 128) return 1;
   return 2;
+}
+
+static int rb_nsplit(const RbArgs& a, int split, int mi, int epi, int force) {
+  if (mi != 1 || epi != LVAE_RB_EPI_PLAIN || split != 3 || force == 1) return 1;
+  return force == 2 || 2 * (int64_t)a.nwg <= 256 ? 2 : 1;
 }
 
 static size_t rb_lds_bytes(int split, int mi, int halo_px, int pro, int epi) {
@@ -676,9 +687,9 @@
   return rb_lds_bytes(rb_split(d), mi, a.halo_px, LVAE_RB_PRO_GATE_BWD, LVAE_RB_EPI_GATE) <= 160 * 1024;
 }
 
-template <int SPLIT, int MI, int PRO, int EPI, bool ELU, bool AP = false>
+template <int SPLIT, int MI, int PRO, int EPI, bool ELU, bool AP = false, int NS = 1>
 static int rb_launch(const RbArgs& a, hipStream_t s) {
-  return launch_lds<rb_conv_kernel<SPLIT, MI, PRO, EPI, ELU, AP>>("resblock_conv", dim3(a.nwg), dim3(256), rb_lds_bytes(SPLIT, MI, a.halo_px, PRO, EPI), 160 * 1024, s, a);
+  return launch_lds<rb_conv_kernel<SPLIT, MI, PRO, EPI, ELU, AP, NS>>("resblock_conv", dim3(a.nwg * NS), dim3(256), rb_lds_bytes(SPLIT, MI, a.halo_px, PRO, EPI), 160 * 1024, s, a);
 }
 
 static bool rb_all_elu(const RbArgs& a) {
@@ -694,8 +705,16 @@
 }
 
 template <int SPLIT, int MI, bool ELU>
-static int rb_dispatch2(const RbArgs& a, hipStream_t s) {
+static int rb_dispatch2(const RbArgs& a, int nsplit, hipStream_t s) {
   const int pro = a.e.prologue, epi = a.e.epilogue;
+  if constexpr (SPLIT == 3 && MI == 1) {
+    if (nsplit == 2) {
+      if (pro == LVAE_RB_PRO_AFFINE) return rb_launch<SPLIT, MI, LVAE_RB_PRO_AFFINE, LVAE_RB_EPI_PLAIN, ELU, false, 2>(a, s);
+      if (pro == LVAE_RB_PRO_BN_APPLY) return rb_launch<SPLIT, MI, LVAE_RB_PRO_BN_APPLY, LVAE_RB_EPI_PLAIN, ELU, false, 2>(a, s);
+      if (a.e.ap_parts != nullptr) return rb_launch<SPLIT, MI, LVAE_RB_PRO_GATE_BWD, LVAE_RB_EPI_PLAIN, ELU, true, 2>(a, s);
+      return rb_launch<SPLIT, MI, LVAE_RB_PRO_GATE_BWD, LVAE_RB_EPI_PLAIN, ELU, false, 2>(a, s);
+    }
+  }
   if (pro == LVAE_RB_PRO_AFFINE) return epi == LVAE_RB_EPI_GATE ? rb_launch<SPLIT, MI, LVAE_RB_PRO_AFFINE, LVAE_RB_EPI_GATE, ELU>(a, s)
                                                                   : rb_launch<SPLIT, MI, LVAE_RB_PRO_AFFINE, LVAE_RB_EPI_PLAIN, ELU>(a, s);
   if (pro == LVAE_RB_PRO_BN_APPLY) return rb_launch<SPLIT, MI, LVAE_RB_PRO_BN_APPLY, LVAE_RB_EPI_PLAIN, ELU>(a, s);
@@ -704,8 +723,8 @@
 }
 
 template <int SPLIT, int MI>
-static int rb_dispatch(const RbArgs& a, hipStream_t s) {
-  return rb_all_elu(a) ? rb_dispatch2<SPLIT, MI, true>(a, s) : rb_dispatch2<SPLIT, MI, false>(a, s);
+static int rb_dispatch(const RbArgs& a, int nsplit, hipStream_t s) {
+  return rb_all_elu(a) ? rb_dispatch2<SPLIT, MI, true>(a, nsplit, s) : rb_dispatch2<SPLIT, MI, false>(a, nsplit, s);
 }
 
 }
@@ -733,6 +752,13 @@
   RbArgs a;
   int mi;
   return rb_plan(d, a, mi) ? a.nwg : 0;
+}
+
+extern "C" int32_t lvae_resblock_conv_nsplit(const lvae_conv_desc* d, const lvae_rb_ext* ext) {
+  RbArgs a;
+  int mi;
+  if (!rb_plan(d, a, mi)) return 0;
+  return rb_nsplit(a, rb_split(d), mi, ext != nullptr ? ext->epilogue : LVAE_RB_EPI_PLAIN, ext != nullptr ? ext->nsplit : 0);
 }
 
 extern "C" size_t lvae_resblock_conv_workspace(const lvae_conv_desc* d) {
@@ -845,8 +871,10 @@
   }
   a.Wp = static_cast<const __bf16*>(d->workspace);
   hipStream_t s = (hipStream_t)stream;
-  if (mi == 1) return split == 1 ? rb_dispatch<1, 1>(a, s) : rb_dispatch<3, 1>(a, s);
-  return split == 1 ? rb_dispatch<1, 2>(a, s) : rb_dispatch<3, 2>(a, s);
+  LVAE_REQUIRE(e.nsplit >= 0 && e.nsplit <= 2, LVAE_EINVAL, "lvae_resblock_conv_f32: nsplit must be 0 (the plan decides), 1 or 2");
+  const int nsplit = rb_nsplit(a, split, mi, epi, e.nsplit);
+  if (mi == 1) return split == 1 ? rb_dispatch<1, 1>(a, nsplit, s) : rb_dispatch<3, 1>(a, nsplit, s);
+  return split == 1 ? rb_dispatch<1, 2>(a, nsplit, s) : rb_dispatch<3, 2>(a, nsplit, s);
 }
 
 #ifdef LVAE_RB_DBG
diff --git a/ladder-vae-pytorch_amd/kernels.py b/ladder-vae-pytorch_amd/kernels.py
--- a/ladder-vae-pytorch_amd/kernels.py
+++ b/ladder-vae-pytorch_amd/kernels.py
@@ -458,7 +458,7 @@
         e.pf_ptr[i], e.pf_bytes[i] = rng[0], rng[1]
 
 
-def rb_conv(x, weight, g, bias, in_act, out_scale, in_bn=None, coef=None, stats_pivot=None, prefetch=None):
+def rb_conv(x, weight, g, bias, in_act, out_scale, in_bn=None, coef=None, stats_pivot=None, prefetch=None, nsplit=0):
     N, H, W, _ = x.shape
     y = torch.empty((N, H, W, g.Cout), dtype=torch.float32, device=x.device)
     d, _ = _rb_desc(x, weight, g, False, y, bias, None, None, in_act, out_scale)
@@ -470,7 +470,7 @@
         parts = StatParts(buf, rows, True)
         d.stats_out, d.stats_pivot = ptr(buf), ptr(stats_pivot)
     e = RbExt()
-    e.prologue, e.epilogue = _C.RB_PRO_AFFINE, _C.RB_EPI_PLAIN
+    e.prologue, e.epilogue, e.nsplit = _C.RB_PRO_AFFINE, _C.RB_EPI_PLAIN, nsplit
     _rb_prefetch(e, prefetch)
     call('lvae_resblock_conv_f32', C.byref(d), C.byref(e), stream_ptr())
     del keep
@@ -536,7 +536,7 @@
         self.parts, self.dh, self.x, self.coef0, self.act, self.dgamma, self.dbeta, self.add, self.out = parts, dh, x, coef0, act, dgamma, dbeta, add, out
 
 
-def rb_gate_dgrad(dout, ab, gate_w, gate_g, act, drop, weight, g, bn_bwd, prefetch=None, apply=None):
+def rb_gate_dgrad(dout, ab, gate_w, gate_g, act, drop, weight, g, bn_bwd, prefetch=None, apply=None, nsplit=0):
     N, H, W, Cn = dout.shape
     dev = dout.device
     dab = torch.empty_like(ab)
@@ -544,7 +544,7 @@
     dh = torch.empty((N, H, W, g.Cin), dtype=torch.float32, device=dev)
     d, _ = _rb_desc(dout, weight, g, True, dh)
     e = RbExt()
-    e.prologue, e.epilogue = _C.RB_PRO_GATE_BWD, _C.RB_EPI_PLAIN
+    e.prologue, e.epilogue, e.nsplit = _C.RB_PRO_GATE_BWD, _C.RB_EPI_PLAIN, nsplit
     _rb_gate_ws(e, gate_w, gate_g, dev, True)
     e.act = ACT[act]
     e.dout, e.ab_in, e.dab, e.pro_drop, e.xt_out = ptr(dout), ptr(ab), ptr(dab), ptr(drop), ptr(dy2)
@@ -558,14 +558,14 @@
     return dab, dy2, dh, parts
 
 
-def rb_apply_dgrad(parts_in, dh_in, x_bn, coef0, act, dgamma, dbeta, drop, weight, g, bn_bwd, prefetch=None):
+def rb_apply_dgrad(parts_in, dh_in, x_bn, coef0, act, dgamma, dbeta, drop, weight, g, bn_bwd, prefetch=None, nsplit=0):
     N, H, W, Cn = dh_in.shape
     dev = dh_in.device
     dy1 = torch.empty((N, H, W, Cn), dtype=torch.float32, device=dev)
     dh = torch.empty((N, H, W, g.Cin), dtype=torch.float32, device=dev)
     d, _ = _rb_desc(dh_in, weight, g, True, dh)
     e = RbExt()
-    e.prologue, e.epilogue = _C.RB_PRO_BN_APPLY, _C.RB_EPI_PLAIN
+    e.prologue, e.epilogue, e.nsplit = _C.RB_PRO_BN_APPLY, _C.RB_EPI_PLAIN, nsplit
     e.bwd_parts, e.bwd_rows, e.bwd_act, e.bwd_M = ptr(parts_in), parts_in.shape[0], ACT[act], N * H * W
     e.bwd_coef, e.bwd_x, e.dgamma, e.dbeta, e.pro_drop, e.xt_out = ptr(coef0), ptr(x_bn), ptr(dgamma), ptr(dbeta), ptr(drop), ptr(dy1)
     parts = _rb_bn_bwd(d, bn_bwd, dh)
diff --git a/ladder-vae-pytorch_amd/ops.py b/ladder-vae-pytorch_amd/ops.py
--- a/ladder-vae-pytorch_amd/ops.py
+++ b/ladder-vae-pytorch_amd/ops.py
@@ -217,7 +217,8 @@
         in_bn, coef1 = _bn_of_half(x, blk.bn1, True, call.parts, call.pivot)
         st.link('fwd', K.rb_weight_ranges(x, cv1.weight, cv1.geom(), False))
         y1, parts2, coef1 = K.rb_conv(x, cv1.weight, cv1.geom(), cv1.bias, act, m1, in_bn=in_bn, coef=coef1, stats_pivot=bn2.running_mean,
-                                      prefetch=K.rb_weight_ranges(x, cv2.weight, cv2.geom(), False, gate=(gate.weight, gate.geom())))
+                                      prefetch=K.rb_weight_ranges(x, cv2.weight, cv2.geom(), False, gate=(gate.weight, gate.geom())),
+                                      nsplit=RB.switches.rb_nsplit)
     else:
         y1, parts2, coef1 = _conv_half(x, blk.bn1, cv1, act, m1, True, call.parts, call.pivot, bn2.running_mean, False)
     in_bn, coef2 = _bn_of_half(y1, bn2, True, parts2, bn2.running_mean)
@@ -296,12 +297,13 @@
     gw, w2, w1 = gate.weight, cv2.weight, cv1.weight
     st.link('bwd', K.rb_weight_ranges(dout, w2, cv2.geom(), True, gate=(gw, gate.geom()), gate_bwd=True))
     dab, dy2, dh2, parts2 = K.rb_gate_dgrad(dout, ab, gw, gate.geom(), act, m2, w2, cv2.geom(), bn_bwd=(y1, coef2[0], act),
-                                            prefetch=K.rb_weight_ranges(dout, w1, cv1.geom(), True), apply=st.take_pending(dout))
+                                            prefetch=K.rb_weight_ranges(dout, w1, cv1.geom(), True), apply=st.take_pending(dout),
+                                            nsplit=RB.switches.rb_nsplit)
     if gw.requires_grad:
         wgrad(y2, dab, gw, gate.geom(), grad_buf(gw), grad_buf(gate.bias))
     wgrad(y1, dy2, w2, cv2.geom(), grad_buf(w2), grad_buf(cv2.bias), in_scale=coef2[0], in_shift=coef2[1], in_act=act)
     dy1, dh1, parts1 = K.rb_apply_dgrad(parts2, dh2, y1, coef2[0], act, grad_buf(bn2.weight), grad_buf(bn2.bias), m1, w1, cv1.geom(),
-                                        bn_bwd=(x, coef1[0], act), prefetch=st.next_ranges('bwd'))
+                                        bn_bwd=(x, coef1[0], act), prefetch=st.next_ranges('bwd'), nsplit=RB.switches.rb_nsplit)
     wgrad(x, dy1, w1, cv1.geom(), grad_buf(w1), grad_buf(cv1.bias), in_scale=coef1[0], in_shift=coef1[1], in_act=act)
     return dh1, parts1
 
diff --git a/ladder-vae-pytorch_amd/resblock.py b/ladder-vae-pytorch_amd/resblock.py
--- a/ladder-vae-pytorch_amd/resblock.py
+++ b/ladder-vae-pytorch_amd/resblock.py
@@ -24,6 +24,7 @@
         self.defer_apply = on('LVAE_DEFER_APPLY')
         self.defer_apply_large = on('LVAE_DEFER_APPLY_LARGE')
         self.rb_fwd_min_hw, self.rb_bwd_min_hw = int(env.get('LVAE_RB_FWD_MIN_HW', '16')), int(env.get('LVAE_RB_BWD_MIN_HW', '1'))
+        self.rb_nsplit = int(env.get('LVAE_RB_NSPLIT', '0'))
         self.rb_gate_large = on('LVAE_RB_GATE_LARGE')
         self.stoch_block = on('LVAE_STOCH_BLOCK')
         self.stoch_block_bwd = on('LVAE_STOCH_BLOCK_BWD')
```

Measured after the change: 9943 images/s, median of 6. 1.02x the previous value.
